# TIXhjq/ML_Function

Hardware: AMD Instinct MI355X
Metric: samples/sec fwd+bwd xDeepFM-CIN B=4096,F=39,K=16 (higher is better)
Workload: dtype f32

## Files before the change

ml_function_amd/csrc/cin.hip:

```cpp
#include "cin_kernels.h"
#include "cin_tail.h"
#include "cin_launch.h"
#include "cin_qtail.h"
#include "cin_qsplit.h"
#include "cin_qmerge.h"

#include <stdlib.h>

namespace fil {

struct CinShape {
  int B, F, K, L;
  int H[kCinMaxL];
  int Hp(int l) const { return l == 0 ? F : H[l - 1]; }
  int HS(int l) const { return 128 * cdiv(H[l], 128); }
  int xps(int l) const { return l == 0 ? F : HS(l - 1); }
  long M() const { return (long)B * K; }
  int JT() const { return cin_jt_of(F); }
  int HSmax() const {
    int h = 0;
    for (int l = 0; l < L; ++l) h = std::max(h, HS(l));
    return h;
  }
};
// ... 4 lines not shown
  if (F > kCinMaxFields) return fail(FIL_ERR_UNSUPPORTED, "%s: F=%d > %d fields", fn, F, kCinMaxFields);
  if ((long)B * K > (1L << 28)) return fail(FIL_ERR_UNSUPPORTED, "%s: B*K = %ld rows > 2^28 (row-split byte offsets of the dW kernel are 32-bit)", fn, (long)B * K);
  s.B = B; s.F = F; s.K = K; s.L = L;
  for (int l = 0; l < L; ++l) {
    if (H[l] < 1) return fail(FIL_ERR_ARG, "%s: H[%d]=%d", fn, l, H[l]);
    if (H[l] > kCinMaxH) return fail(FIL_ERR_UNSUPPORTED, "%s: H[%d]=%d > %d feature maps", fn, l, H[l], kCinMaxH);
    s.H[l] = H[l];
  }
  return FIL_OK;
}

static int chunks_of(int H) { return cdiv(H, 128); }
static int env_int(const char* name, int dflt) {
  const char* v = getenv(name);
  return v != nullptr && *v != 0 ? atoi(v) : dflt;
}
struct Knobs {
  int mb, sym, dw_mb, dw_splits, dz_mb, tail_splits, tail_settle, tail_dz_mode, ksplit, dzs_mb, qtail, qmerge, dz2, fwdq, headfold, packfold, dwfold4;
};
static const Knobs& knobs() {
  static const Knobs k = {env_int("FIL_CIN_MB", 0), env_int("FIL_CIN_SYM", 1), env_int("FIL_CIN_DW_MB", 1), env_int("FIL_CIN_DW_SPLITS", 0),
                          env_int("FIL_CIN_DZ_MB", 1), env_int("FIL_CIN_TAIL_SPLITS", 0), env_int("FIL_CIN_TAIL_SETTLE", 0), env_int("FIL_CIN_TAIL_DZ_MODE", 0), env_int("FIL_CIN_KSPLIT", -1), env_int("FIL_CIN_DZS_MB", 0), env_int("FIL_CIN_QTAIL", 1), env_int("FIL_CIN_QMERGE", 1), env_int("FIL_CIN_DZ2", 1), env_int("FIL_CIN_FWDQ", 1), env_int("FIL_CIN_HEADFOLD", 1), env_int("FIL_CIN_PACKFOLD", 1), env_int("FIL_CIN_DWFOLD4", 1)};
  return k;
}
struct CinTune {
  int mb_forced;
  bool sym, no_ksplit;
  explicit CinTune(int mode)
      : mb_forced((mode & FIL_CIN_MB2) ? 2 : knobs().mb), sym(knobs().sym != 0 && !(mode & FIL_CIN_NOSYM)), no_ksplit((mode & FIL_CIN_NOKSPLIT) != 0) {}
  int mb_rows(long M) const {
    if (mb_forced == 1 || mb_forced == 2) return mb_forced;
    return cdiv((int)std::min<long>(M, 1L << 30), 64) >= 768 ? 2 : 1;
  }
  int ksplit(long M) const {
    if (knobs().ksplit == 0 || no_ksplit) return 1;
    if (mb_rows(M) != 1) return 1;
    if (knobs().ksplit == 4) return 4;
    return cdiv((int)std::min<long>(M, 1L << 30), 32) <= 512 ? 4 : 1;
  }
};

static const char* kFwdNames[kCinMaxL] = {"cin_fwd_l1", "cin_fwd_l2", "cin_fwd_l3", "cin_fwd_l4", "cin_fwd_l5", "cin_fwd_l6", "cin_fwd_l7", "cin_fwd_l8"};
static const char* kDwNames[kCinMaxL] = {"cin_bwd_dw_l1", "cin_bwd_dw_l2", "cin_bwd_dw_l3", "cin_bwd_dw_l4", "cin_bwd_dw_l5", "cin_bwd_dw_l6", "cin_bwd_dw_l7", "cin_bwd_dw_l8"};
static const char* kDzNames[kCinMaxL] = {"cin_bwd_dz_l1", "cin_bwd_dz_l2", "cin_bwd_dz_l3", "cin_bwd_dz_l4", "cin_bwd_dz_l5", "cin_bwd_dz_l6", "cin_bwd_dz_l7", "cin_bwd_dz_l8"};
static double gemm_flops(long M, int Hp, int F, int H) { return 2.0 * (double)M * Hp * F * H; }

struct DwPlan {
  int MB, blocks_x, splits, rows_per_split, chunks;
};
static int cu_count() {
  static const int n = [] {
    int dev = 0, v = 0;
    if (hipGetDevice(&dev) != hipSuccess || hipDeviceGetAttribute(&v, hipDeviceAttributeMultiprocessorCount, dev) != hipSuccess || v <= 0) v = 256;
    return v;
  }();
  return n;
}

static DwPlan dw_plan(long M, int C, int H) {
  DwPlan p;
  p.chunks = chunks_of(H);
  p.MB = knobs().dw_mb == 2 ? 2 : 1;
  const int waves_c = cdiv(C, 32 * p.MB);
  p.blocks_x = cdiv(waves_c, 4);
  const long tiles = (long)p.blocks_x * p.chunks;
  const long ncu = cu_count();
  const long unit = 2 * kDwDepth;
  auto rows_of = [&](int splits) { return std::max<long>(unit, ((M + splits - 1) / splits + unit - 1) / unit * unit); };
  int best = knobs().dw_splits;
  if (best <= 0) {
    static const double t_of[4] = {0.0, 1.05e-4, 1.39e-4, 1.96e-4};
    double best_ms = -1.0;
    for (int sp = (int)std::max<long>(1, (M + (1L << 20) - 1) >> 20); sp <= 256; ++sp) {
      const long rps = rows_of(sp);
      const long real = (M + rps - 1) / rps;
      if (real != sp && sp > 1) continue;
      long wgs = tiles * real;
      double per_row = 0.0;
      while (wgs > 0) {
        const long round = std::min(wgs, 3 * ncu);
        per_row += t_of[std::min<long>(3, (round + ncu - 1) / ncu)];
        wgs -= round;
      }
      const double ms = (double)rps * per_row * p.MB + (double)real * C * H * 4.0 / 6e9;
      if (best_ms < 0 || ms < best_ms) best = sp, best_ms = ms;
      if (rps == unit) break;
    }
  }
  best = std::min(std::max(best, 1), 256);
  const long rps = rows_of(best);
  p.rows_per_split = (int)rps;
  p.splits = (int)std::max<long>(1, (M + rps - 1) / rps);
  return p;
}

static int launch_dw3(hipStream_t st, const DwPlan& p, const float* gT, int HS, const float* xT, const float* xpT, int xps, float* part,
                      long M, int F, int Hp, int H, int symD = 0, int xtra = 0) {
  const int items = p.blocks_x * p.splits * p.chunks;
  const dim3 grid((items + 7) / 8 * 8);
#define FIL_DW3(MBV, ONES) \
  hipLaunchKernelGGL((cin_dw3_kernel<MBV, ONES>), grid, dim3(kCinThreads), 0, st, gT, HS, xT, xpT, xps, part, (int)M, F, Hp, H, p.rows_per_split, \
                     p.blocks_x, p.chunks, items, symD, xtra)
  if (xT == nullptr) {
    if (p.MB == 2) FIL_DW3(2, true); else FIL_DW3(1, true);
  } else {
    if (p.MB == 2) FIL_DW3(2, false); else FIL_DW3(1, false);
  }
#undef FIL_DW3
  return p.splits;
}

struct TailGeom {
  bool on = false;
  int p = 0;
  int NCB = 0, JP = 0, JT4 = 0, NQ = 0, JHp = 0;
  int Hpp = 0, Hq = 0, HL = 0, Cp = 0, C1 = 0;
  int periods = 0, tiles = 0;
  size_t uf_floats = 0, uz_floats = 0;
};
static TailGeom tail_geom(const CinShape& s) {
  TailGeom g;
  if (s.L < 3 || !cin_tail_supported(s.F)) return g;
  g.on = true;
  g.p = s.L - 2;
  g.NCB = cin_tail_ncb(s.F);
  g.JP = 16 * g.NCB;
  g.JT4 = cin_tail_jt4(s.F);
  g.NQ = cin_tail_nq(s.F);
  g.JHp = 4 * g.NQ;
  g.Hpp = s.H[g.p - 1];
  g.Hq = s.H[g.p];
  g.HL = s.H[s.L - 1];
  g.Cp = g.Hpp * s.F;
  g.C1 = g.Cp + 1;
  const int JT = s.JT();
  g.periods = cdiv(g.Hpp, cin_dz_h_per_period(JT));
  g.tiles = g.periods * cin_dz_tiles_per_period(JT) + 1;
  g.uf_floats = (size_t)g.Hpp * g.JT4 * 64 * g.NCB + (size_t)align_up(g.JP + 1, 64);
  g.uz_floats = (size_t)g.tiles * 64 * g.JHp;
  return g;
}
constexpr int kCinRetiredBits = 0;
static bool tail_used(const CinShape& s, int mode) {
  if ((mode & (FIL_CIN_GENERAL | FIL_CIN_NOTAIL)) != 0) return false;
  const TailGeom g = tail_geom(s);
  if (!g.on) return false;
  return (mode & FIL_CIN_TAIL_ALWAYS) != 0 || 4 * g.JP <= 3 * g.Hq;
}
static bool qtail_used(const CinShape& s, int mode, const CinTune& tune) {
  if (s.M() <= 16384 && (mode & FIL_CIN_TAIL_ALWAYS) == 0) return false;
  return tail_used(s, mode) && s.L == 3 && tune.sym && s.F >= 2 && s.F + 2 <= kQtConst && s.H[0] <= 128 && 3 * s.F + 1 <= s.HSmax() && (mode & FIL_CIN_NOQTAIL) == 0 &&
         knobs().qtail != 0;
}
static bool qmerge_used(const CinShape& s, int mode, const CinTune& tune) {
  return qtail_used(s, mode, tune) && 3 * s.F + 3 <= s.HSmax() && (mode & FIL_CIN_NOQMERGE) == 0 && knobs().qmerge != 0;
}
constexpr int kCinPrecBf16 = 1 << 20;
static int qsplit_planes(int mode) { return (mode & kCinPrecBf16) != 0 ? 1 : 3; }
static bool qsplit_fwd_menu(int JT) { return JT >= 2 && JT <= 12 && JT % 2 == 0; }
static bool qsplit_used(const CinShape& s, int mode, const CinTune& tune) {
  return (mode & (FIL_CIN_BF16X3 | kCinPrecBf16)) != 0 && qmerge_used(s, mode, tune) && knobs().fwdq != 0 && knobs().dz2 != 0 && s.HS(0) == 128 &&
         qsplit_fwd_menu(cin_jt_sym(s.F));
}
static size_t qsplit_wb_bytes(const CinShape& s) { return (size_t)cin_qs_steps(s.F, cin_jt_sym(s.F)) * kQsStageBytes; }
static size_t qsplit_wzb_bytes(const CinShape& s) {
  const int jts = cin_jt_sym(s.F);
  return ((size_t)cdiv(s.F, cin_dz_h_per_period(jts)) * cin_dz_tiles_per_period(jts) + 1) * 8 * 3072;
}
static size_t qtail_wz_floats(const CinShape& s) {
  const int jts = cin_jt_sym(s.F);
  return ((size_t)cdiv(s.F, cin_dz_h_per_period(jts)) * cin_dz_tiles_per_period(jts) + 1) * 32 * s.HS(0);
}
static size_t qtail_wsn_floats(const CinShape& s) { return (size_t)chunks_of(s.H[0]) * 2 * s.JT() * 128; }
static size_t qtail_saved_floats(const CinShape& s) {
  return (size_t)s.M() * s.HS(0) + (size_t)s.F * s.F * s.H[0] + (size_t)s.H[1] * s.F + 128 + (size_t)s.H[0] * s.F + qtail_wsn_floats(s) +
         qtail_wz_floats(s);
}
struct TailDwPlan {
  int blocks_x, splits, rows_per_split;
};
static TailDwPlan tail_dw_plan(long M, int C1) {
  TailDwPlan p;
  p.blocks_x = cdiv(C1, 16 * kTailCbw);
  const long unit = 4L * 4 * kTailDwDepth;
  long want = knobs().tail_splits > 0 ? knobs().tail_splits : std::max<long>(1, 2L * cu_count() / p.blocks_x);
  want = std::max<long>(want, (M + (1L << 22) - 1) >> 22);
  const long rows = std::max(unit, ((M + want - 1) / want + unit - 1) / unit * unit);
  p.rows_per_split = (int)rows;
  p.splits = (int)std::max<long>(1, (M + rows - 1) / rows);
  return p;
}

constexpr int kHeadChunk = 16;
constexpr int kColRows = 128;

static size_t saved_bytes(const CinShape& s) {
  size_t t = align_up((size_t)s.M() * s.F * sizeof(float), 256);
  for (int l = 0; l + 1 < s.L; ++l) t += align_up((size_t)s.M() * s.HS(l) * sizeof(float), 256);
  const TailGeom g = tail_geom(s);
  if (g.on) {
    size_t u = align_up((size_t)s.M() * s.F * sizeof(float), 256);
    for (int l = 0; l < g.p; ++l) u += align_up((size_t)s.M() * s.HS(l) * sizeof(float), 256);
    u += align_up((size_t)s.M() * g.JP * sizeof(float), 256) + align_up((g.uz_floats + g.uf_floats) * sizeof(float), 256) +
         align_up((size_t)g.Hq * s.F * sizeof(float), 256);
    t = std::max(t, u);
  }
  if (g.on && s.L == 3) {
    const size_t u = align_up((size_t)s.M() * s.F * sizeof(float), 256) + align_up((size_t)s.M() * s.HS(0) * sizeof(float), 256) +
                     align_up(qtail_saved_floats(s) * sizeof(float), 256);
    t = std::max(t, u);
  }
  return t;
}
static size_t wf_floats(const CinShape& s) {
  size_t w = 0;
  for (int l = 0; l < s.L; ++l) {
    w = std::max(w, (size_t)chunks_of(s.H[l]) * s.Hp(l) * 2 * s.JT() * 128);
  }
  w = std::max(w, (size_t)chunks_of(s.H[0]) * s.F * 2 * cin_jt_sym(s.F) * 128);
  w += (size_t)2 * 2 * s.JT() * 128;
  return w;
}
static int dz_periods(const CinShape& s, int l) { return cdiv(s.Hp(l), cin_dz_h_per_period(s.JT())); }
static size_t wz_floats(const CinShape& s) {
  const int jts = cin_jt_sym(s.F);
  size_t w = ((size_t)cdiv(s.F, cin_dz_h_per_period(jts)) * cin_dz_tiles_per_period(jts) + 1) * 32 * s.HS(0);
  w = std::max(w, (size_t)s.F * (s.F / 2 + 1) * s.H[0]);
  for (int l = 0; l < s.L; ++l) w = std::max(w, ((size_t)dz_periods(s, l) * cin_dz_tiles_per_period(s.JT()) + 1) * 32 * s.HS(l));
  return w;
}
static int pool_chunks(const CinShape& s, int l) { return std::max(chunks_of(s.H[l]), l > 0 ? chunks_of(s.H[l - 1]) : 1); }
static size_t fwd_ws_bytes(const CinShape& s) {
  size_t t = 0;
  for (int l = 0; l < s.L; ++l) t += align_up((size_t)pool_chunks(s, l) * s.M() * sizeof(float), 256);
  t += align_up((size_t)s.Hp(s.L - 1) * s.F * sizeof(float), 256);
  t += align_up(wf_floats(s) * sizeof(float), 256);
  t += align_up((size_t)kCinMaxH * sizeof(float), 256);
  t += align_up(cin_x2_floats(s.M(), cin_x2_len(s.F)) * sizeof(float), 256);
  t += align_up((size_t)chunks_of(s.H[0]) * s.F * 2 * cin_jt_sym(s.F) * 128 * sizeof(float), 256);
  t += align_up(qsplit_wb_bytes(s), 256);
  return t;
}
static size_t dw_part_floats(const CinShape& s) {
  size_t pmax = 0;
  for (int l = 0; l < s.L; ++l) pmax = std::max(pmax, (size_t)dw_plan(s.M(), s.Hp(l) * s.F, s.H[l]).splits * s.Hp(l) * s.F * s.H[l]);
  const int csym = s.F * (s.F / 2 + 1);
  pmax = std::max(pmax, (size_t)dw_plan(s.M(), csym, s.H[0]).splits * csym * s.H[0]);
  pmax = std::max(pmax, (size_t)dw_plan(s.M(), csym + s.F, s.H[0]).splits * (csym + s.F) * s.H[0]);
  if (s.L == 3) pmax = std::max(pmax, (size_t)cin_dwq_plan(s.M(), csym + s.F, cu_count()).pairs * (csym + s.F) * 256);
  if (s.L == 3) pmax = std::max(pmax, (size_t)cin_dwqb_plan(s.M(), csym + s.F, cu_count()).splits * (csym + s.F) * 256);
  pmax = std::max(pmax, (size_t)dw_plan(s.M(), s.Hp(s.L - 1), s.F).splits * s.Hp(s.L - 1) * s.F);
  pmax = std::max(pmax, (size_t)dw_plan(s.M(), s.F, s.Hp(s.L - 1)).splits * s.Hp(s.L - 1) * s.F);
  const TailGeom g = tail_geom(s);
  if (g.on) {
    pmax = std::max(pmax, (size_t)tail_dw_plan(s.M(), g.C1).splits * g.C1 * g.JP + (size_t)cdiv(g.Cp, kTailPc) * g.Hq * s.F);
  }
  return pmax;
}
static size_t bwd_ws_bytes(const CinShape& s) {
  const size_t LK = (size_t)s.L * s.K;
  const size_t M = (size_t)s.M();
  size_t t = 0;
  t += align_up((size_t)s.B * LK * sizeof(float), 256);
  t += 2 * align_up(M * s.HSmax() * sizeof(float), 256);
  t += align_up(dw_part_floats(s) * sizeof(float), 256);
  const size_t nblk = (size_t)cdiv(std::max(1, s.B), kHeadChunk);
  const size_t ncol = (M + kColRows - 1) / kColRows;
  t += align_up(std::max(ncol * s.HSmax(), nblk * (LK + 1)) * sizeof(float), 256);
  const size_t cl = (size_t)std::max(s.Hp(s.L - 1), s.L == 3 ? s.H[0] : 0) * s.F;
  t += 2 * align_up(cl * sizeof(float), 256);
  t += align_up(wz_floats(s) * sizeof(float), 256);
  t += 2 * align_up(M * s.F * sizeof(float), 256);
  t += align_up((size_t)s.F * s.F * kCinMaxH * sizeof(float), 256);
  t += align_up(((M + 255) / 256 + 1) * kQtConst * sizeof(float), 256);
  t += align_up(((M + 255) / 256) * (LK + 1) * sizeof(float), 256);
  t += 2 * align_up(qsplit_wzb_bytes(s), 256);
  return t;
}

template <typename KernelT>
static void allow_lds(KernelT kernel, size_t sh) {
  if (sh > 48 * 1024) (void)hipFuncSetAttribute(reinterpret_cast<const void*>(kernel), hipFuncAttributeMaxDynamicSharedMemorySize, (int)sh);
}

}

using namespace fil;

extern "C" size_t fil_cin_saved_bytes(int B, int F, int K, int L, const int* H) {
  CinShape s;
  if (check_shape("fil_cin_saved_bytes", B, F, K, L, H, s) != FIL_OK || B == 0) return 0;
  return saved_bytes(s);
}

extern "C" size_t fil_cin_fwd_workspace_bytes(int B, int F, int K, int L, const int* H) {
  CinShape s;
  if (check_shape("fil_cin_fwd_workspace_bytes", B, F, K, L, H, s) != FIL_OK || B == 0) return 0;
  return fwd_ws_bytes(s);
}

extern "C" size_t fil_cin_bwd_workspace_bytes(int B, int F, int K, int L, const int* H) {
  CinShape s;
  if (check_shape("fil_cin_bwd_workspace_bytes", B, F, K, L, H, s) != FIL_OK || B == 0) return 0;
  return bwd_ws_bytes(s);
}

extern "C" int fil_cin_grad_ready_points(int B, int F, int K, int L, const int* H, int mode, int* point) {
  CinShape s;
  if (int rc = check_shape("fil_cin_grad_ready_points", B, F, K, L, H, s)) return rc;
  if (point == nullptr || mode < 0 || mode > 1023) return fail(FIL_ERR_ARG, "fil_cin_grad_ready_points: point == NULL or mode %d out of range", mode);
  if ((mode & kCinRetiredBits) != 0) return fail(FIL_ERR_UNSUPPORTED, "fil_cin_grad_ready_points: mode %d holds a retired bit (2: the split-bf16 experiment)", mode);
  if (B == 0) {
    for (int i = 0; i <= L; ++i) point[i] = 0;
    return 1;
  }
  int pt = 0, l = L - 1;
  point[L] = pt++;
  if (qmerge_used(s, mode, CinTune(mode))) {
    point[0] = point[L] = 0;
    pt = 1;
    point[1] = point[2] = pt++;
    return pt;
  }
  if (tail_used(s, mode)) {
    point[L - 1] = point[L - 2] = pt++;
    l = L - 3;
  }
  for (; l >= 0; --l) point[l] = pt++;
  return pt;
}

#define FIL_CIN_CHECK_ARG(cond)                                                        \
  do {                                                                                 \
    if (!(cond)) return ::fil::fail(FIL_ERR_ARG, "%s: bad argument: %s", who, #cond); \
  } while (0)

static int cin_precision_bits(const char* who, int mode, int precision, int* bits) {
  if (precision != FIL_CIN_PREC_DEFAULT && precision != FIL_CIN_PREC_BF16)
    return fail(FIL_ERR_ARG, "%s: precision %d (0 DEFAULT, 1 BF16)", who, precision);
  if (precision == FIL_CIN_PREC_BF16 && (mode & FIL_CIN_BF16X3) != 0)
    return fail(FIL_ERR_ARG, "%s: precision BF16 with mode bit BF16X3 (mode %d): two operand precisions", who, mode);
  *bits = precision == FIL_CIN_PREC_BF16 ? kCinPrecBf16 : 0;
  return FIL_OK;
}

extern "C" int fil_cin_precision_used(int B, int F, int K, int L, const int* H, int mode, int precision) {
  CinShape s;
  if (int rc = check_shape("fil_cin_precision_used", B, F, K, L, H, s)) return rc;
  if (mode < 0 || mode > 1023 || (mode & kCinRetiredBits) != 0) return fail(FIL_ERR_UNSUPPORTED, "fil_cin_precision_used: mode %d", mode);
  int bits = 0;
  if (int rc = cin_precision_bits("fil_cin_precision_used", mode, precision, &bits)) return rc;
  if (bits == 0 || B == 0) return FIL_CIN_PREC_DEFAULT;
  return qsplit_used(s, mode | bits, CinTune(mode)) ? FIL_CIN_PREC_BF16 : FIL_CIN_PREC_DEFAULT;
}

static int cin_fwd_impl(const char* who, const float* x, const float* const* W, const float* const* bias, const float* dense_w,
                        const float* dense_b, float* out, float* pooled, float* saved, int B, int F, int K, int L,
                        const int* H, int output_dim, int mode, int precision, void* workspace, size_t workspace_bytes, void* stream) {
  CinShape s;
  int rc = check_shape(who, B, F, K, L, H, s);
  if (rc != FIL_OK) return rc;
  if (mode < 0 || mode > 1023 || (mode & kCinRetiredBits) != 0)
    return fail(FIL_ERR_UNSUPPORTED, "%s: mode %d (bits: 1 general kernels, 2 BF16X3, 4 MB2, 8 NOSYM, 16 X_TRANSPOSED, 32 NOTAIL, 64 TAIL_ALWAYS, 128 NOKSPLIT, 256 NOQTAIL, 512 NOQMERGE)", who, mode);
  {
    int bits = 0;
    if ((rc = cin_precision_bits(who, mode, precision, &bits)) != FIL_OK) return rc;
    mode |= bits;
  }
  const bool xt_in = (mode & FIL_CIN_X_TRANSPOSED) != 0;
  const CinTune tune(mode);
  const bool tail = tail_used(s, mode);
  const bool qtail = qtail_used(s, mode, tune);
  const bool qmerge = qmerge_used(s, mode, tune);
  const bool qsplit = qsplit_used(s, mode, tune);
  const int qnp = qsplit_planes(mode);
  const TailGeom tg = tail_geom(s);
  mode &= 1;
  if (B == 0) return FIL_OK;
  FIL_CIN_CHECK_ARG(x && W && bias && pooled && saved);
  FIL_CIN_CHECK_ARG(output_dim != 1 || (dense_w && dense_b && out));
  if (workspace == nullptr || workspace_bytes < fwd_ws_bytes(s))
    return fail(FIL_ERR_WORKSPACE, "fil_cin_fwd: workspace %zu < %zu bytes", workspace_bytes, fwd_ws_bytes(s));
  hipStream_t st = (hipStream_t)stream;
  const long M = s.M();
  const int JT = s.JT(), MB = tune.mb_rows(M);
  Carver ws(workspace);
  PoolArgs pa;
  for (int l = 0; l < L; ++l) {
    pa.part[l] = ws.take<float>((size_t)pool_chunks(s, l) * M);
    pa.chunks[l] = chunks_of(H[l]);
  }
  float* wsum = ws.take<float>((size_t)s.Hp(L - 1) * F);
  float* Wf = ws.take<float>(wf_floats(s));
  float* qt_zbias = ws.take<float>((size_t)kCinMaxH);
  const int XL = cin_x2_len(F);
  float* x2T = ws.take<float>(cin_x2_floats(M, XL));
  const bool need_x2 = tune.sym;
  float* WfT = ws.take<float>((size_t)chunks_of(H[0]) * F * 2 * cin_jt_sym(F) * 128);
  u32x4* Wb = reinterpret_cast<u32x4*>(ws.take<unsigned char>(qsplit_wb_bytes(s)));
  Carver sv(saved);
  float* xT_own = sv.take<float>((size_t)M * F);
  const float* xT = xt_in ? x : xT_own;
  float *tailY = nullptr, *tailUz = nullptr, *tailBmT = nullptr;
  float *qtR = nullptr, *qtT = nullptr, *qtWsumL = nullptr, *qtCvec = nullptr, *qtWsumP = nullptr, *qtWsnP = nullptr, *qtWzT = nullptr;
  if (qtail) {
    Carver pv(saved);
    (void)pv.take<float>((size_t)M * F);
    (void)pv.take<float>((size_t)M * s.HS(0));
    float* q = pv.take<float>(qtail_saved_floats(s));
    qtR = q;
    qtT = qtR + (size_t)M * s.HS(0);
    qtWsumL = qtT + (size_t)F * F * H[0];
    qtCvec = qtWsumL + (size_t)H[1] * F;
    qtWsumP = qtCvec + 128;
    qtWsnP = qtWsumP + (size_t)H[0] * F;
    qtWzT = qtWsnP + qtail_wsn_floats(s);
  } else if (tail) {
    Carver pv(saved);
    (void)pv.take<float>((size_t)M * F);
    for (int l = 0; l < tg.p; ++l) (void)pv.take<float>((size_t)M * s.HS(l));
    tailY = pv.take<float>((size_t)M * tg.JP);
    tailUz = pv.take<float>(tg.uz_floats + tg.uf_floats);
    tailBmT = pv.take<float>((size_t)tg.Hq * F);
  }
  const bool prep_fused = tail && tune.sym;
  if (qtail) {
    FIL_CIN_CHECK_ARG(W[0] && W[L - 1] && W[L - 2]);
    ProfScope ps("cin_fwd_prep", st, 2.0 * M * F * sizeof(float));
    const int JTs = cin_jt_sym(F), chunks0 = chunks_of(H[0]);
    const long npack = (long)chunks0 * F * 2 * JTs * 128;
    const bool fq = qmerge && knobs().fwdq != 0 && s.HS(0) == 128;
    const int nt = fq ? 0 : B, npk = (int)std::min<long>((npack + 255) / 256, 1024), nwl = cdiv(tg.Hq * F, 8), nwp = cdiv(tg.Hpp * F, 8);
    const size_t sh = (xt_in || fq) ? 0 : (size_t)F * (K + 1) * sizeof(float);
    allow_lds(cin_qtail_prep_kernel, sh);
    hipLaunchKernelGGL(cin_qtail_prep_kernel, dim3(nt + npk + nwl + nwp), dim3(256), sh, st, x, xT_own, F, K, nt, W[0], Wf, H[0], 2 * JTs, chunks0, npk,
                       W[L - 1], qtWsumL, tg.Hq, tg.HL, nwl, W[L - 2], qtWsumP, qtWsnP, tg.Hpp, 2 * JT, chunks_of(tg.Hpp), x2T, XL, xt_in ? 1 : 0);
  } else if (prep_fused) {
    FIL_CIN_CHECK_ARG(W[0] && W[L - 1]);
    ProfScope ps("cin_fwd_prep", st, 2.0 * M * F * sizeof(float));
    const int JTs = cin_jt_sym(F), chunks0 = chunks_of(H[0]);
    const long npack = (long)chunks0 * F * 2 * JTs * 128;
    const int nt = B, npk = (int)std::min<long>((npack + 255) / 256, 1024), nws = cdiv(tg.Hq * F, 8), nz = 64;
    const size_t sh = xt_in ? 0 : (size_t)F * (K + 1) * sizeof(float);
    allow_lds(cin_fwd_prep_kernel, sh);
    hipLaunchKernelGGL(cin_fwd_prep_kernel, dim3(nt + npk + nws + nz), dim3(256), sh, st, x, xT_own, F, K, nt, W[0], Wf, H[0], 2 * JTs, chunks0,
                       npk, W[L - 1], tailBmT, tg.Hq, tg.HL, nws, reinterpret_cast<float4*>(tailUz), (long)((tg.uz_floats + tg.uf_floats) / 4), x2T, XL,
                       xt_in ? 1 : 0);
  } else if (!xt_in || need_x2) {
    ProfScope ps("cin_transpose_in", st, 2.0 * M * F * sizeof(float));
    hipLaunchKernelGGL(cin_transpose_in_kernel, dim3(B), dim3(256), xt_in ? 0 : (size_t)F * (K + 1) * sizeof(float), st, x, xT_own, F, K,
                       need_x2 ? x2T : nullptr, XL, xt_in ? 1 : 0);
  }
  FIL_CHECK_LAUNCH();
  const float* xpT = xT;
  bool fused_last = false;
  bool head_done = false;
  for (int l = 0; l < L; ++l) {
    FIL_CIN_CHECK_ARG(W[l] && bias[l]);
    if (qtail && qmerge && l == 0 && knobs().fwdq != 0 && s.HS(0) == 128) {
      const int p = tg.p, lL = L - 1, Hpp = tg.Hpp, Hq = tg.Hq, HS0 = s.HS(0);
      FIL_CIN_CHECK_ARG(W[p] && W[lL] && bias[p] && bias[lL]);
      const int JTs = cin_jt_sym(F), chunks = chunks_of(Hpp);
      float* x1T = sv.take<float>((size_t)M * HS0);
      {
        ProfScope ps("cin_tail_prep", st);
        int ks = -1;
        if (!xt_in && K <= 64 && (K & (K - 1)) == 0 && (reinterpret_cast<uintptr_t>(x) & 15) == 0)
          for (ks = 0; (1 << ks) < K;) ++ks;
        const size_t sh_x = ks >= 0 ? (size_t)(64 >> ks) * F * (K + 1) : (xt_in ? (size_t)64 * (F | 1) : (size_t)F * (K + 1));
        const int tiles = cdiv(F, cin_dz_h_per_period(JTs)) * cin_dz_tiles_per_period(JTs) + 1;
        const bool fold = !qsplit && knobs().packfold != 0;
        const QtPackFold pf = fold ? QtPackFold{WfT, qtWzT, JTs, chunks, HS0, tiles} : QtPackFold{nullptr, nullptr, 0, 0, 0, 0};
        const size_t sh = std::max(cin_qtail_t_lds_floats(F, Hq, fold), sh_x) * sizeof(float);
        allow_lds(cin_qtail_t_x_kernel, sh);
        const int nx = (ks >= 0 || xt_in) ? (int)((M + 63) / 64) : B, nT = cin_qtail_t_wgs(Hpp);
        hipLaunchKernelGGL(cin_qtail_t_x_kernel, dim3(nT + nx), dim3(256), sh, st, W[p], qtWsumL, bias[p], bias[lL], tg.HL, qtT, qtCvec, qt_zbias, Hpp, F, Hq,
                           nT, x, xT_own, K, x2T, XL, xt_in ? 1 : 0, ks, (ks >= 0 || xt_in) ? (long)M : 0L, pf);
        if (!fold) {
          const long npack = (long)chunks * F * 2 * JTs * 128;
          const int nbf = (int)std::min<long>((npack + 255) / 256, 1024), nbz = (int)std::min<long>(((long)tiles * 32 * HS0 + 255) / 256, 1024);
          const int NTq = qsplit ? cin_qs_steps(F, JTs) : 0, nbq = qsplit ? std::min(cdiv(NTq * 512, 256), 512) : 0;
          if (qnp == 1)
            hipLaunchKernelGGL(cin_qtail_pack_kernel<1>, dim3(nbf + nbz + nbq), dim3(256), 0, st, qtT, WfT, qtWzT, F, Hpp, JTs, chunks, nbf, HS0, tiles, nbz,
                               W[0], H[0], Wb, NTq);
          else
            hipLaunchKernelGGL(cin_qtail_pack_kernel<3>, dim3(nbf + nbz + nbq), dim3(256), 0, st, qtT, WfT, qtWzT, F, Hpp, JTs, chunks, nbf, HS0, tiles, nbz,
                               W[0], H[0], Wb, NTq);
        }
      }
      FIL_CHECK_LAUNCH();
      {
        const double algo = gemm_flops(M, F, F, H[0]) + gemm_flops(M, Hpp, F, Hq) + gemm_flops(M, Hq, F, tg.HL);
        ProfScope ps("cin_fwd_q", st, algo, gemm_flops(M, 1, F * (F / 2 + 1), H[0]) + gemm_flops(M, 1, F * (F / 2 + 1), Hpp));
        CinHeadFold hf{};
        if (K <= 32 && (K & (K - 1)) == 0 && knobs().headfold != 0) {
          int ks = 0;
          while ((1 << ks) < K) ++ks;
          hf = CinHeadFold{pooled, output_dim == 1 ? out : nullptr, dense_w, dense_b, ks, (int)(L * K), p * K, lL * K};
          head_done = true;
        }
        if (qsplit) {
          const int NT = cin_qs_steps(F, JTs);
          if (!cin_launch_fwdq_b(st, qnp, JTs, x2T, XL, Wb, NT, bias[0], qtWsnP, JT, qtCvec, x1T, qtR, HS0, const_cast<float*>(pa.part[0]),
                                 const_cast<float*>(pa.part[p]), const_cast<float*>(pa.part[lL]), (int)M, F, H[0], hf))
            return fail(FIL_ERR_UNSUPPORTED, "fil_cin_fwd: no split-bf16 forward kernel for JT=%d (F=%d)", JTs, F);
        } else if (!cin_launch_fwdq(st, JTs, x2T, XL, Wf, WfT, bias[0], qtWsnP, JT, qtCvec, x1T, qtR, HS0, const_cast<float*>(pa.part[0]),
                                    const_cast<float*>(pa.part[p]), const_cast<float*>(pa.part[lL]), (int)M, F, H[0], hf))
          return fail(FIL_ERR_UNSUPPORTED, "fil_cin_fwd: no merged forward kernel for JT=%d (F=%d)", JTs, F);
        pa.chunks[0] = pa.chunks[p] = pa.chunks[lL] = 1;
      }
      FIL_CHECK_LAUNCH();
      break;
    }
    if (qtail && l == tg.p) {
      const int lL = L - 1, Hpp = tg.Hpp, Hq = tg.Hq, HS0 = s.HS(0);
      FIL_CIN_CHECK_ARG(W[lL] && bias[lL]);
      const int JTs = cin_jt_sym(F), chunks = chunks_of(Hpp);
      {
        ProfScope ps("cin_tail_prep", st);
        const size_t sh = cin_qtail_t_lds_floats(F, Hq, false) * sizeof(float);
        allow_lds(cin_qtail_t_kernel, sh);
        hipLaunchKernelGGL(cin_qtail_t_kernel, dim3(cin_qtail_t_wgs(Hpp)), dim3(256), sh, st, W[l], qtWsumL, bias[l], bias[lL], tg.HL, qtT, qtCvec, qt_zbias, Hpp, F, Hq);
        const long npack = (long)chunks * F * 2 * JTs * 128;
        const int tiles = cdiv(F, cin_dz_h_per_period(JTs)) * cin_dz_tiles_per_period(JTs) + 1;
        const int nbf = (int)std::min<long>((npack + 255) / 256, 1024), nbz = (int)std::min<long>(((long)tiles * 32 * HS0 + 255) / 256, 1024);
        hipLaunchKernelGGL(cin_qtail_pack_kernel<3>, dim3(nbf + nbz), dim3(256), 0, st, qtT, Wf, qtWzT, F, Hpp, JTs, chunks, nbf, HS0, tiles);
      }
      FIL_CHECK_LAUNCH();
      {
        const double algo = gemm_flops(M, Hpp, F, Hq) + gemm_flops(M, Hq, F, tg.HL);
        ProfScope ps("cin_fwd_tail", st, algo, gemm_flops(M, 1, F * (F / 2 + 1), Hpp));
        const int ks = tune.ksplit(M);
        cin_launch_fwd3_sym(st, MB, JTs, dim3(ks == 4 ? cdiv((int)M, 32) : cdiv((int)M, 128 * MB), chunks), xT, x2T, XL, Wf, qt_zbias, qtR, HS0,
                            const_cast<float*>(pa.part[lL]), (int)M, F, Hpp, ks);
      }
      FIL_CHECK_LAUNCH();
      {
        ProfScope ps("cin_tail_pool", st);
        const float* wsn = qtWsnP;
        float* pp = const_cast<float*>(pa.part[l]);
        float* pL = const_cast<float*>(pa.part[lL]);
        const dim3 grid((int)((M + 127) / 128));
#define FIL_QP(JTV) \
  case JTV: hipLaunchKernelGGL((cin_qtail_pool2_kernel<JTV>), grid, dim3(256), 0, st, xT, xpT, s.xps(l), wsn, qtR, HS0, qtCvec, pp, pL, (int)M, F, Hpp); break;
        switch (JT) { FIL_QP(4) FIL_QP(8) FIL_QP(12) FIL_QP(16) FIL_QP(20) FIL_QP(24) FIL_QP(28) FIL_QP(32) }
#undef FIL_QP
        pa.chunks[l] = pa.chunks[lL] = 1;
      }
      FIL_CHECK_LAUNCH();
      break;
    }
    if (tail && l == tg.p) {
      const int lL = L - 1;
      FIL_CIN_CHECK_ARG(W[lL] && bias[lL]);
      float* Y = tailY;
      float* Uz = tailUz;
      float* bmT = tailBmT;
      float* Uf = Uz + tg.uz_floats;
      float* consts = Uf + (size_t)tg.Hpp * tg.JT4 * 64 * tg.NCB;
      {
        ProfScope ps("cin_tail_prep", st);
        if (!prep_fused) {
          hipLaunchKernelGGL(cin_tail_wsum_kernel, dim3(cdiv(tg.Hq * F, 8)), dim3(256), 0, st, W[lL], bmT, tg.Hq, F, tg.HL);
          (void)hipMemsetAsync(Uz, 0, (tg.uz_floats + tg.uf_floats) * sizeof(float), st);
        }
        const size_t sh = (size_t)(F + 1) * (((tg.Hq + 3) & ~3) + 4) * sizeof(float);
        allow_lds(cin_tail_ueff_kernel, sh);
        hipLaunchKernelGGL(cin_tail_ueff_kernel, dim3(cdiv(tg.C1, kTailUc)), dim3(256), sh, st, W[l], bias[l], bmT, bias[lL], tg.HL, Uf, Uz, consts,
                           tg.Hpp, F, tg.Hq, tg.JT4, tg.JP, JT, tg.JHp);
      }
      FIL_CHECK_LAUNCH();
      {
        const double algo = gemm_flops(M, tg.Hpp, F, tg.Hq) + gemm_flops(M, tg.Hq, F, tg.HL);
        ProfScope ps("cin_fwd_tail", st, algo, 2.0 * (double)M * tg.Cp * (F + 1));
        const int RB = tune.mb_rows(M) == 2 ? 4 : 2;
        TailFwdArgs a{xT, xpT, s.xps(l), Uf, consts, Y, tg.JP, const_cast<float*>(pa.part[l]), const_cast<float*>(pa.part[lL]), (int)M, F, tg.Hpp,
                      tune.ksplit(M)};
        cin_launch_tail_fwd(st, RB, tg.JT4, tg.NCB, a);
        pa.chunks[l] = pa.chunks[lL] = 1;
      }
      FIL_CHECK_LAUNCH();
      break;
    }
    const int Hp = s.Hp(l), Hl = H[l], xps = s.xps(l);
    float* xoutT = l + 1 < L ? sv.take<float>((size_t)M * s.HS(l)) : nullptr;
    float* part = const_cast<float*>(pa.part[l]);
    const bool fuse_next = mode == 0 && l == L - 2 && !(l == 0 && tune.sym);
    if (l == L - 1 && mode == 0) {
      if (!fused_last) {
        const size_t sh = (size_t)Hp * ((F + 3) & ~3) * sizeof(float);
        ProfScope ps("cin_last_fwd", st, 2.0 * (double)M * Hp * F);
        hipLaunchKernelGGL(cin_wsum_kernel, dim3(cdiv(Hp * F, 8)), dim3(256), 0, st, W[l], wsum, Hp * F, Hl);
        allow_lds(cin_last_fwd_kernel, sh);
        hipLaunchKernelGGL(cin_last_fwd_kernel, dim3(cdiv((int)M, kLastRows)), dim3(256), sh, st, xT, xpT, xps, wsum, bias[l], part, (int)M, F, Hp, Hl);
        pa.chunks[l] = 1;
      }
    } else {
      const int chunks = chunks_of(Hl);
      if (l == 0 && tune.sym) {
        const int JTs = cin_jt_sym(F);
        const long npack = (long)chunks * F * 2 * JTs * 128;
        if (!prep_fused)
          hipLaunchKernelGGL(cin_pack_wf_sym_kernel, dim3((int)std::min<long>((npack + 255) / 256, 2048)), dim3(256), 0, st, W[l], Wf, F, Hl, 2 * JTs, chunks);
        ProfScope ps(kFwdNames[l], st, gemm_flops(M, Hp, F, Hl), gemm_flops(M, 1, F * (F / 2 + 1), Hl));
        const int ks = tune.ksplit(M);
        cin_launch_fwd3_sym(st, MB, JTs, dim3(ks == 4 ? cdiv((int)M, 32) : cdiv((int)M, 128 * MB), chunks), xT, x2T, XL, Wf, bias[l], xoutT, s.HS(l), part,
                            (int)M, F, Hl, ks);
      } else {
        const long npack = (long)chunks * Hp * 2 * JT * 128;
        hipLaunchKernelGGL(cin_pack_wf_kernel, dim3((int)std::min<long>((npack + 255) / 256, 2048)), dim3(256), 0, st, W[l], Wf, Hp, F, Hl, 2 * JT, chunks);
        const float* wsn = nullptr;
        if (fuse_next) {
          FIL_CIN_CHECK_ARG(W[l + 1] && bias[l + 1]);
          float* wsn_buf = Wf + (size_t)npack;
          hipLaunchKernelGGL(cin_wsum_wsn_kernel, dim3(cdiv(Hl * F, 8)), dim3(256), 0, st, W[l + 1], wsum, Hl * F, H[l + 1], wsn_buf, Hl, F, 2 * JT,
                             chunks);
          wsn = wsn_buf;
          pa.chunks[l + 1] = chunks;
          fused_last = true;
        }
        ProfScope ps(kFwdNames[l], st, gemm_flops(M, Hp, F, Hl) + (fuse_next ? 2.0 * (double)M * Hl * F : 0.0));
        cin_launch_fwd3(st, MB, JT, dim3(cdiv((int)M, 128 * MB), chunks), xT, xpT, xps, Wf, bias[l], xoutT, s.HS(l), part, (int)M, F, Hp, Hl,
                        wsn, fuse_next ? bias[l + 1] : nullptr, fuse_next ? H[l + 1] : 0, fuse_next ? const_cast<float*>(pa.part[l + 1]) : nullptr);
      }
    }
    FIL_CHECK_LAUNCH();
    xpT = xoutT;
  }
  if (!head_done) {
    ProfScope ps("cin_head_fwd", st);
    hipLaunchKernelGGL(cin_head_fwd_kernel, dim3(cdiv(B, kHeadSamples)), dim3(256), (size_t)kHeadSamples * L * K * sizeof(float), st, pa, dense_w, dense_b, pooled,
                       output_dim == 1 ? out : nullptr, B, K, L);
  }
  FIL_CHECK_LAUNCH();
  return FIL_OK;
}

extern "C" int fil_cin_fwd(const float* x, const float* const* W, const float* const* bias, const float* dense_w,
                           const float* dense_b, float* out, float* pooled, float* saved, int B, int F, int K, int L,
                           const int* H, int output_dim, int mode, void* workspace, size_t workspace_bytes, void* stream) {
  return cin_fwd_impl("fil_cin_fwd", x, W, bias, dense_w, dense_b, out, pooled, saved, B, F, K, L, H, output_dim, mode, FIL_CIN_PREC_DEFAULT, workspace,
                      workspace_bytes, stream);
}

extern "C" int fil_cin_fwd_p(const float* x, const float* const* W, const float* const* bias, const float* dense_w,
                             const float* dense_b, float* out, float* pooled, float* saved, int B, int F, int K, int L,
                             const int* H, int output_dim, int mode, int precision, void* workspace, size_t workspace_bytes, void* stream) {
  return cin_fwd_impl("fil_cin_fwd_p", x, W, bias, dense_w, dense_b, out, pooled, saved, B, F, K, L, H, output_dim, mode, precision, workspace,
                      workspace_bytes, stream);
}

static int cin_bwd_impl(const char* who, const float* x, const float* const* W, const float* const* bias, const float* dense_w,
                        const float* pooled, const float* saved, const float* g, float* dx, float* const* dW,
                        float* const* dbias, float* ddense_w, float* ddense_b, int B, int F, int K, int L, const int* H,
                        int output_dim, int mode, int precision, void* const* grad_ready_events, void* workspace, size_t workspace_bytes,
                        void* stream) {
  CinShape s;
  int rc = check_shape(who, B, F, K, L, H, s);
  if (rc != FIL_OK) return rc;
  if (mode < 0 || mode > 1023 || (mode & kCinRetiredBits) != 0)
    return fail(FIL_ERR_UNSUPPORTED, "%s: mode %d (bits: 1 general kernels, 2 BF16X3, 4 MB2, 8 NOSYM, 16 X_TRANSPOSED, 32 NOTAIL, 64 TAIL_ALWAYS, 128 NOKSPLIT, 256 NOQTAIL, 512 NOQMERGE)", who, mode);
  {
    int bits = 0;
    if ((rc = cin_precision_bits(who, mode, precision, &bits)) != FIL_OK) return rc;
    mode |= bits;
  }
  const bool xt_in = (mode & FIL_CIN_X_TRANSPOSED) != 0;
  const CinTune tune(mode);
  const bool tail = tail_used(s, mode);
  const bool qtail = qtail_used(s, mode, tune);
  const bool qmerge = qmerge_used(s, mode, tune);
  const bool qsplit = qsplit_used(s, mode, tune);
  const int qnp = qsplit_planes(mode);
  const TailGeom tg = tail_geom(s);
  mode &= 1;
  FIL_CIN_CHECK_ARG(W && dW && dbias);
  hipStream_t st = (hipStream_t)stream;
  const size_t LK = (size_t)L * K;
  auto ready = [&](int slot) {
    if (grad_ready_events != nullptr && grad_ready_events[slot] != nullptr) (void)hipEventRecord((hipEvent_t)grad_ready_events[slot], st);
  };
  if (B == 0) {
    for (int l = 0; l < L; ++l) {
      (void)hipMemsetAsync(dW[l], 0, (size_t)s.Hp(l) * F * H[l] * sizeof(float), st);
      (void)hipMemsetAsync(dbias[l], 0, (size_t)H[l] * sizeof(float), st);
    }
    if (output_dim == 1) {
      (void)hipMemsetAsync(ddense_w, 0, LK * sizeof(float), st);
      (void)hipMemsetAsync(ddense_b, 0, sizeof(float), st);
    }
    for (int l = 0; l <= L; ++l) ready(l);
    return FIL_OK;
  }
  FIL_CIN_CHECK_ARG(g && dx && saved && (x || !xt_in));
  FIL_CIN_CHECK_ARG(output_dim != 1 || (dense_w && pooled && ddense_w && ddense_b));
  if (workspace == nullptr || workspace_bytes < bwd_ws_bytes(s))
    return fail(FIL_ERR_WORKSPACE, "fil_cin_bwd: workspace %zu < %zu bytes", workspace_bytes, bwd_ws_bytes(s));
  const long M = s.M();
  const int JT = s.JT();
  Carver ws(workspace);
  float* dP = ws.take<float>((size_t)B * LK);
  float* Gbuf[2];
  Gbuf[0] = ws.take<float>((size_t)M * s.HSmax());
  Gbuf[1] = ws.take<float>((size_t)M * s.HSmax());
  float* part = ws.take<float>(dw_part_floats(s));
  const int nblk = cdiv(B, kHeadChunk);
  const int ncol = (int)((M + kColRows - 1) / kColRows);
  float* small = ws.take<float>(std::max((size_t)ncol * s.HSmax(), (size_t)nblk * (LK + 1)));
  const size_t cl = (size_t)s.Hp(L - 1) * F;
  const size_t cl_buf = (size_t)std::max(s.Hp(L - 1), L == 3 ? H[0] : 0) * F;
  float* wsum = ws.take<float>(cl_buf);
  float* vlast = ws.take<float>(cl_buf);
  float* Wz = ws.take<float>(wz_floats(s));
  float* dxT = ws.take<float>((size_t)M * F);
  float* gx0T = ws.take<float>((size_t)M * F);
  float* qt_dT = ws.take<float>((size_t)F * F * kCinMaxH);
  const int qt_ndc = (int)((M + 255) / 256);
  float* qt_dcpart = ws.take<float>((size_t)(qt_ndc + 1) * kQtConst);
  float* qt_hpart = ws.take<float>((size_t)qt_ndc * (LK + 1));
  u32x4* Wzb1 = reinterpret_cast<u32x4*>(ws.take<unsigned char>(qsplit_wzb_bytes(s)));
  u32x4* Wzb2 = reinterpret_cast<u32x4*>(ws.take<unsigned char>(qsplit_wzb_bytes(s)));

  Carver sv(const_cast<float*>(saved));
  const float* xT_own = sv.take<float>((size_t)M * F);
  const float* xT = xt_in ? x : xT_own;
  const float* maps[kCinMaxL];
  const float *tailY = nullptr, *tailUz = nullptr, *tailWsum = nullptr;
  const float *qtR = nullptr, *qtT = nullptr, *qtWsumL = nullptr, *qtCvec = nullptr, *qtWsumP = nullptr, *qtWsnP = nullptr, *qtWzT = nullptr;
  if (qtail) {
    maps[0] = sv.take<float>((size_t)M * s.HS(0));
    const float* q = sv.take<float>(qtail_saved_floats(s));
    qtR = q;
    qtT = qtR + (size_t)M * s.HS(0);
    qtWsumL = qtT + (size_t)F * F * H[0];
    qtCvec = qtWsumL + (size_t)H[1] * F;
    qtWsumP = qtCvec + 128;
    qtWsnP = qtWsumP + (size_t)H[0] * F;
    qtWzT = qtWsnP + qtail_wsn_floats(s);
  } else if (tail) {
    for (int l = 0; l < tg.p; ++l) maps[l] = sv.take<float>((size_t)M * s.HS(l));
    tailY = sv.take<float>((size_t)M * tg.JP);
    tailUz = sv.take<float>(tg.uz_floats + tg.uf_floats);
    tailWsum = sv.take<float>((size_t)tg.Hq * F);
  } else {
    for (int l = 0; l + 1 < L; ++l) maps[l] = sv.take<float>((size_t)M * s.HS(l));
  }

  const float* dPsrc = g;
  if (output_dim == 1 && qmerge) {
    dPsrc = dP;
  } else if (output_dim == 1) {
    ProfScope ps("cin_head_bwd", st);
    hipLaunchKernelGGL(cin_head_bwd_kernel, dim3(nblk), dim3(256), 0, st, g, dense_w, pooled, dP, small, B, (int)LK, kHeadChunk);
    if (!tail) hipLaunchKernelGGL(cin_reduce_kernel, dim3(cdiv((int)LK + 1, 64)), dim3(256), 0, st, small, ddense_w, (long)(LK + 1), nblk, ddense_b, (long)LK);
    FIL_CHECK_LAUNCH();
    dPsrc = dP;
  }
  if (!tail) ready(L);

  int cur = 0;
  int ltop = L - 1;
  bool dx_started = false;
  bool have_gx0 = false;
  bool wz_prepacked = false;
  bool qm_joined = false;
  if (qmerge) {
    const int p = tg.p, lL = L - 1, Hpp = tg.Hpp, Hq = tg.Hq, HS0 = s.HS(0);
    FIL_CIN_CHECK_ARG(bias && W[0] && W[p] && W[lL] && bias[p] && dW[0] && dW[p] && dW[lL] && dbias[0] && dbias[p] && dbias[lL]);
    const float* xpT = maps[p - 1];
    const int xps = s.xps(p);
    const float* dPp = dPsrc + (size_t)p * K;
    const float* dPL = dPsrc + (size_t)lL * K;
    const float* dPprev = dPsrc + (size_t)(p - 1) * K;
    const double algo_tail = gemm_flops(M, Hpp, F, Hq) + gemm_flops(M, Hq, F, tg.HL);
    const double algo1 = gemm_flops(M, F, F, H[0]);
    const int symD = F / 2 + 1, Cl = F * symD;
    const int JTs = cin_jt_sym(F);
    const int periods = cdiv(F, cin_dz_h_per_period(JTs));
    const int tiles0 = periods * cin_dz_tiles_per_period(JTs) + 1;
    const int XE = F + 3;
    float* xe = Gbuf[1];
    float* gxR = xe + (size_t)M * XE;
    float* dxR = gxR + (size_t)M * F;
    {
      ProfScope ps("cin_tail_a", st, (double)M * (2 * F + 3) * sizeof(float));
      const size_t sh = (size_t)256 * (F + 3 + (output_dim == 1 ? L : 0)) * sizeof(float);
      allow_lds(cin_qtail_xe_kernel<3>, sh);
      allow_lds(cin_qtail_xe_kernel<1>, sh);
      const int np = (int)std::min<long>(((long)tiles0 * 32 * HS0 + 255) / 256, 1024);
      const int nq2 = qsplit ? 2 * std::min(cdiv(tiles0 * 512, 256), 256) : 0;
      if (qnp == 1)
        hipLaunchKernelGGL(cin_qtail_xe_kernel<1>, dim3(qt_ndc + np + nq2), dim3(kXeThreads), sh, st, xT, dPL, dPp, (int)LK, K, xe, qt_dcpart, (int)M, F,
                           qt_ndc, output_dim == 1 ? g : nullptr, dense_w, pooled, dP, qt_hpart, (int)LK, lL, p, W[0], Wz, H[0], JTs, HS0, tiles0, np, qtT,
                           Hpp, Wzb1, Wzb2);
      else
        hipLaunchKernelGGL(cin_qtail_xe_kernel<3>, dim3(qt_ndc + np + nq2), dim3(kXeThreads), sh, st, xT, dPL, dPp, (int)LK, K, xe, qt_dcpart, (int)M, F,
                           qt_ndc, output_dim == 1 ? g : nullptr, dense_w, pooled, dP, qt_hpart, (int)LK, lL, p, W[0], Wz, H[0], JTs, HS0, tiles0, np, qtT,
                           Hpp, Wzb1, Wzb2);
    }
    FIL_CHECK_LAUNCH();
    {
      ProfScope ps("cin_last_bwd", st, 6.0 * (double)M * Hpp * F);
      cin_launch_last_bwd2(st, JT, xT, xpT, xps, qtWsumP, qtWsnP, dPp, (int)LK, dPprev, Gbuf[cur], HS0, dxT, (int)M, F, K, Hpp, qtR, HS0, dPL, small);
    }
    FIL_CHECK_LAUNCH();
    int dw_parts = 0;
    {
      ProfScope ps("cin_bwd_dw_q", st, algo1 + algo_tail, gemm_flops(M, 1, Cl, H[0]) + gemm_flops(M, 1, Cl, Hpp));
      if (qsplit) {
        const DwqbPlan bp = cin_dwqb_plan(M, Cl + F, cu_count());
        cin_launch_dwq_b(st, qnp, bp, Gbuf[cur], xpT, HS0, xe, XE, part, (int)M, F, symD);
        dw_parts = bp.splits;
      } else {
        const bool f4 = knobs().dwfold4 != 0;
        const DwqPlan dp = f4 ? cin_dwq_plan4(M, Cl + F, cu_count()) : cin_dwq_plan(M, Cl + F, cu_count());
        if (f4)
          hipLaunchKernelGGL((cin_dwq_kernel<kDwqDepth, 4>), dim3((dp.wgs + 7) / 8 * 8), dim3(kDwqThreads), 0, st, Gbuf[cur], xpT, HS0, xe, XE, part, (int)M, F,
                             symD, dp.rows_per_split, dp.splits, dp.ncol_full, dp.rem, dp.wgs_full, dp.wgs);
        else
          hipLaunchKernelGGL((cin_dwq_kernel<kDwqDepth, 2>), dim3((dp.wgs + 7) / 8 * 8), dim3(kDwqThreads), 0, st, Gbuf[cur], xpT, HS0, xe, XE, part, (int)M, F,
                             symD, dp.rows_per_split, dp.splits, dp.ncol_full, dp.rem, dp.wgs_full, dp.wgs);
        dw_parts = dp.pairs;
      }
    }
    FIL_CHECK_LAUNCH();
    {
      ProfScope ps("cin_reduce_dw", st);
      const int nb1 = cdiv(H[0], 64);
      const int nh = output_dim == 1 ? cdiv((int)LK + 1, 64) : 0;
      hipLaunchKernelGGL(cin_reduce_expand_q_kernel, dim3((Cl + F + 3) / 4 + nb1 + nh), dim3(256), 0, st, part, dw_parts, F, symD, H[0], Hpp, dW[0], qt_dT,
                         vlast, small, ncol, dbias[0], nb1, qt_hpart, qt_ndc, (int)LK, ddense_w, ddense_b);
    }
    FIL_CHECK_LAUNCH();
    ready(L);
    ready(0);
    {
      ProfScope ps("cin_tail_params", st);
      const size_t sh = cin_qtail_params_lds(F, Hq);
      allow_lds(cin_qtail_params_kernel, sh);
      float* dcfin = qt_dcpart + (size_t)qt_ndc * kQtConst;
      hipLaunchKernelGGL(cin_qtail_params_kernel, dim3(2 * Hpp + 1), dim3(256), sh, st, W[p], qtWsumL, qt_dT, vlast, dW[p], part, Hpp, F, Hq, qt_dcpart, qt_ndc,
                         dcfin);
      hipLaunchKernelGGL(cin_qtail_fill_kernel, dim3(cdiv(Hq * F, kQtFillCols)), dim3(kQtFillThreads), 0, st, part, Hpp, dcfin, bias[p], qtWsumL, dW[lL], dbias[p], dbias[lL], F, Hq,
                         tg.HL);
    }
    FIL_CHECK_LAUNCH();
    ready(lL);
    ready(p);
    const int NHMAX = HS0 / 2;
    if (NHMAX == 64 && knobs().dz2 != 0) {
      ProfScope ps("cin_bwd_dz_q", st, algo1 + algo_tail, gemm_flops(M, 1, Cl, H[0]) + gemm_flops(M, 1, Cl, Hpp));
      bool split_done = false;
      if (qsplit) {
        split_done = cin_launch_dz2_b(st, qnp, JTs, Gbuf[cur], xpT, HS0, dPL, (int)LK, K, Wzb1, Wzb2, xT, dxT, 1, (int)M, F, H[0], Hpp, periods, dx, qtCvec);
      }
      if (!split_done &&
          !cin_launch_dz2(st, JTs, Gbuf[cur], xpT, HS0, dPL, (int)LK, K, Wz, qtWzT, xT, dxT, 1, (int)M, F, H[0], Hpp, periods, dx, qtCvec))
        return fail(FIL_ERR_UNSUPPORTED, "fil_cin_bwd: no two-pass data-gradient kernel for JT=%d (F=%d)", JTs, F);
      qm_joined = true;
    } else {
      const bool two_waves = NHMAX == 64 && cin_dzs_two_waves(JTs) && tune.mb_forced != 2 && knobs().dzs_mb != 2;
      const int MBs = two_waves ? 1 : tune.mb_rows(M);
      const int ks = MBs != 1 ? 1 : tune.ksplit(M);
      const dim3 zgrid(ks == 4 ? cdiv((int)M, 32) : cdiv((int)M, 128 * MBs));
      {
        ProfScope ps("cin_bwd_dz_tail", st, algo_tail, gemm_flops(M, 1, Cl, Hpp));
        cin_launch_dz3_sym(st, MBs, JTs, NHMAX, zgrid, xpT, HS0, qtWzT, xT, gxR, dxR, 0, (int)M, F, Hpp, periods, ks);
      }
      FIL_CHECK_LAUNCH();
      {
        ProfScope ps("cin_bwd_dz_l1", st, algo1, gemm_flops(M, 1, Cl, H[0]));
        cin_launch_dz3_sym(st, MBs, JTs, NHMAX, zgrid, Gbuf[cur], HS0, Wz, xT, gx0T, dxT, 1, (int)M, F, H[0], periods, ks);
      }
      have_gx0 = true;
    }
    FIL_CHECK_LAUNCH();
    dx_started = true;
    ltop = -1;
  } else if (qtail) {
    const int p = tg.p, lL = L - 1, Hpp = tg.Hpp, Hq = tg.Hq, HS0 = s.HS(0);
    FIL_CIN_CHECK_ARG(bias && W[p] && W[lL] && bias[p] && dW[p] && dW[lL] && dbias[p] && dbias[lL]);
    const float* xpT = maps[p - 1];
    const int xps = s.xps(p);
    const float* dPp = dPsrc + (size_t)p * K;
    const float* dPL = dPsrc + (size_t)lL * K;
    const float* dPprev = dPsrc + (size_t)(p - 1) * K;
    const double algo = gemm_flops(M, Hpp, F, Hq) + gemm_flops(M, Hq, F, tg.HL);
    float* xs = Gbuf[1];
    float* gxR = xs + (size_t)M * (F + 1);
    float* dxR = gxR + (size_t)M * F;
    {
      ProfScope ps("cin_tail_a", st, (double)M * (F + 64) * sizeof(float));
      const size_t sh = (size_t)256 * (F + 3) * sizeof(float);
      allow_lds(cin_qtail_scale_kernel, sh);
      const int nh = output_dim == 1 ? cdiv((int)LK + 1, 64) : 0;
      FIL_CIN_CHECK_ARG(W[0]);
      const int JTs0 = cin_jt_sym(F);
      const int tiles0 = cdiv(F, cin_dz_h_per_period(JTs0)) * cin_dz_tiles_per_period(JTs0) + 1;
      const int np = (int)std::min<long>(((long)tiles0 * 32 * HS0 + 255) / 256, 1024);
      hipLaunchKernelGGL(cin_qtail_scale_kernel, dim3(qt_ndc + nh + np), dim3(256), sh, st, xT, dPL, dPp, (int)LK, K, xs, qt_dcpart, (int)M, F, qt_ndc, small,
                         ddense_w, ddense_b, (int)LK, nblk, nh, W[0], Wz, H[0], JTs0, HS0, tiles0);
      wz_prepacked = true;
    }
    FIL_CHECK_LAUNCH();
    ready(L);
    {
      ProfScope ps("cin_last_bwd", st, 6.0 * (double)M * Hpp * F);
      cin_launch_last_bwd2(st, JT, xT, xpT, xps, qtWsumP, qtWsnP, dPp, (int)LK, dPprev, Gbuf[cur], HS0, dxT, (int)M, F, K, Hpp, qtR, HS0, dPL, small);
    }
    FIL_CHECK_LAUNCH();
    const int symD = F / 2 + 1, Cl = F * symD;
    const int JTs = cin_jt_sym(F);
    {
      ProfScope ps("cin_bwd_dw_tail", st, algo, gemm_flops(M, 1, Cl, Hpp));
      const int parts = launch_dw3(st, dw_plan(M, Cl + F, Hpp), xpT, HS0, xT, xs, F + 1, part, M, F, F, Hpp, symD, F);
      const long nW = (long)Cl * Hpp, pstride = (long)(Cl + F) * Hpp;
      hipLaunchKernelGGL(cin_reduce_expand_sym_kernel, dim3((int)((nW + 63) / 64) + cdiv(F * Hpp, 64)), dim3(256), 0, st, part, qt_dT, F, symD, Hpp, parts,
                         pstride, vlast, (long)F * Hpp);
    }
    FIL_CHECK_LAUNCH();
    {
      ProfScope ps("cin_tail_params", st);
      const size_t sh = cin_qtail_params_lds(F, Hq);
      allow_lds(cin_qtail_params_kernel, sh);
      float* dcfin = qt_dcpart + (size_t)qt_ndc * kQtConst;
      hipLaunchKernelGGL(cin_qtail_params_kernel, dim3(2 * Hpp + 1), dim3(256), sh, st, W[p], qtWsumL, qt_dT, vlast, dW[p], part, Hpp, F, Hq, qt_dcpart, qt_ndc,
                         dcfin);
      hipLaunchKernelGGL(cin_qtail_fill_kernel, dim3(cdiv(Hq * F, kQtFillCols)), dim3(kQtFillThreads), 0, st, part, Hpp, dcfin, bias[p], qtWsumL, dW[lL], dbias[p], dbias[lL], F, Hq,
                         tg.HL);
    }
    FIL_CHECK_LAUNCH();
    ready(lL);
    ready(p);
    {
      const int periods = cdiv(F, cin_dz_h_per_period(JTs));
      ProfScope ps("cin_bwd_dz_tail", st, algo, gemm_flops(M, 1, Cl, Hpp));
      const int NHMAX = HS0 / 2;
      const bool two_waves = NHMAX == 64 && cin_dzs_two_waves(JTs) && tune.mb_forced != 2 && knobs().dzs_mb != 2;
      const int MBs = two_waves ? 1 : tune.mb_rows(M);
      const int ks = MBs != 1 ? 1 : tune.ksplit(M);
      cin_launch_dz3_sym(st, MBs, JTs, NHMAX, dim3(ks == 4 ? cdiv((int)M, 32) : cdiv((int)M, 128 * MBs)), xpT, HS0, qtWzT, xT, gxR, dxR, 0, (int)M, F, Hpp,
                         periods, ks);
    }
    FIL_CHECK_LAUNCH();
    dx_started = true;
    ltop = p - 1;
  } else if (tail) {
    const int p = tg.p, lL = L - 1;
    FIL_CIN_CHECK_ARG(bias && W[p] && W[lL] && bias[p] && dW[p] && dW[lL] && dbias[p] && dbias[lL]);
    const float* xpT = maps[p - 1];
    const int xps = s.xps(p);
    const double algo = gemm_flops(M, tg.Hpp, F, tg.Hq) + gemm_flops(M, tg.Hq, F, tg.HL);
    float* Apk = Gbuf[1];
    wz_prepacked = p == 1 && tune.sym && F >= 2;
    {
      ProfScope ps("cin_tail_a", st, (double)M * (F + 64) * sizeof(float));
      const int na = (int)std::min<long>((M * 16 * tg.NCB + 255) / 256, 4096);
      const int nh = output_dim == 1 ? cdiv((int)LK + 1, 64) : 0;
      int np = 0, JTs = 0, tiles0 = 0;
      if (wz_prepacked) {
        FIL_CIN_CHECK_ARG(W[0]);
        JTs = cin_jt_sym(F);
        tiles0 = cdiv(F, cin_dz_h_per_period(JTs)) * cin_dz_tiles_per_period(JTs) + 1;
        np = (int)std::min<long>(((long)tiles0 * 32 * s.HS(0) + 255) / 256, 1024);
      }
      hipLaunchKernelGGL(cin_tail_pre_kernel, dim3(na + nh + np), dim3(256), 0, st, xT, dPsrc, (int)LK, K, p, lL, Apk, (int)M, F, tg.NCB, na, small,
                         ddense_w, ddense_b, (int)LK, nblk, nh, W[0], Wz, H[0], JTs, s.HS(0), tiles0);
    }
    FIL_CHECK_LAUNCH();
    ready(L);
    const TailDwPlan tp = tail_dw_plan(M, tg.C1);
    {
      ProfScope ps("cin_bwd_dw_tail", st, algo, 2.0 * (double)M * tg.C1 * (F + 2));
      TailDwArgs a{Apk, xT, xpT, xps, part, (int)M, F, tg.Hpp, tg.JP, tp.rows_per_split, tp.blocks_x, tp.blocks_x * tp.splits, knobs().tail_settle != 0};
      cin_launch_tail_dw(st, tg.NCB, a);
    }
    FIL_CHECK_LAUNCH();
    {
      ProfScope ps("cin_tail_params", st);
      const int nblk_p = cdiv(tg.Cp, kTailPc);
      const int ldb = (tg.Hq + 3) & ~3;
      const size_t sh = ((size_t)(F + 1) * ldb + (size_t)tg.JP * (kTailPc + 4) + (size_t)kTailPc * ldb) * sizeof(float);
      allow_lds(cin_tail_params_kernel, sh);
      float* partB = part + (size_t)tp.splits * tg.C1 * tg.JP;
      float* qones = vlast;
      hipLaunchKernelGGL(cin_tail_params_kernel, dim3(2 * nblk_p), dim3(256), sh, st, part, tp.splits, W[p], tailWsum, dW[p], dbias[p], partB, qones,
                         tg.Cp, F, tg.Hq, tg.JP);
      hipLaunchKernelGGL(cin_tail_fill_kernel, dim3(cdiv(tg.Hq * F, 64)), dim3(256), 0, st, partB, nblk_p, qones, bias[p], dW[lL], dbias[lL], F,
                         tg.Hq, tg.HL);
    }
    FIL_CHECK_LAUNCH();
    ready(lL);
    ready(p);
    {
      ProfScope ps("cin_bwd_dz_tail", st, algo, 2.0 * (double)M * tg.Cp * (F + 1));
      TailDzArgs a{tailUz, xT, xpT, xps, tailY, tg.JP, dPsrc, (int)LK, K, p, lL, Gbuf[cur], s.HS(p - 1), dxT, (int)M, F, tg.Hpp, tg.periods, knobs().tail_dz_mode,
                   tune.ksplit(M)};
      cin_launch_tail_dz(st, JT, tg.NQ, a);
    }
    FIL_CHECK_LAUNCH();
    dx_started = true;
    ltop = p - 1;
  } else if (mode == 0) {
    const int l = L - 1;
    FIL_CIN_CHECK_ARG(W[l] && dW[l] && dbias[l]);
    const int Hp = s.Hp(l), Hl = H[l], xps = s.xps(l);
    const float* xpT = l == 0 ? xT : maps[l - 1];
    const float* dPl = dPsrc + (size_t)l * K;
    const float* dPprev = l > 0 ? dPsrc + (size_t)(l - 1) * K : nullptr;
    const size_t shw = (size_t)Hp * ((F + 3) & ~3) * sizeof(float);
    ProfScope ps("cin_last_bwd", st, 6.0 * (double)M * Hp * F);
    hipLaunchKernelGGL(cin_wsum_wsn_kernel, dim3(cdiv(Hp * F, 8)), dim3(256), 0, st, W[l], wsum, Hp * F, Hl, l > 0 ? Wz : nullptr, Hp, F, 2 * JT,
                       chunks_of(Hp));
    hipLaunchKernelGGL(cin_slice_sum_kernel, dim3(nblk), dim3(256), 0, st, dPl, (int)LK, small, B, K, kHeadChunk);
    {
      float* yT = Gbuf[1];
      const int YS = (F + 3) & ~3;
      const long tot = M * YS;
      hipLaunchKernelGGL(cin_scale_rows3_kernel, dim3((int)std::min<long>((tot + 255) / 256, 4096)), dim3(256), 0, st, xT, dPl, (int)LK, K, yT, (int)M, F, YS);
      const bool swap = l > 0;
      int nb;
      if (swap) nb = launch_dw3(st, dw_plan(M, F, Hp), xpT, xps, nullptr, yT, YS, part, M, 1, F, Hp);
      else nb = launch_dw3(st, dw_plan(M, Hp, F), yT, YS, nullptr, xpT, xps, part, M, 1, Hp, F);
      hipLaunchKernelGGL(cin_reduce_kernel, dim3(cdiv((int)cl, 64)), dim3(256), 0, st, part, vlast, (long)cl, nb);
      hipLaunchKernelGGL(cin_fill_rows_kernel, dim3((int)std::min<long>(((long)cl * Hl + 255) / 256, 2048)), dim3(256), 0, st, vlast, dW[l], (long)cl, Hl,
                         swap ? F : 0, Hp, small, nblk, dbias[l]);
    }
    ready(l);
    if (l > 0) {
      cin_launch_last_bwd2(st, JT, xT, xpT, xps, wsum, Wz, dPl, (int)LK, dPprev, Gbuf[cur], s.HS(l - 1), dxT, (int)M, F, K, Hp);
    } else {
      const size_t shb = shw + (size_t)kLastRows * (kLastFMax + 1) * sizeof(float);
      allow_lds(cin_last_bwd_kernel, shb);
      hipLaunchKernelGGL(cin_last_bwd_kernel, dim3(cdiv((int)M, kLastRows)), dim3(256), shb, st, xT, xpT, xps, wsum, dPl, (int)LK, dPprev,
                         nullptr, 0, dxT, 1, (int)M, F, K, Hp);
    }
    FIL_CHECK_LAUNCH();
    dx_started = true;
    ltop = L - 2;
  } else {
    const long total = M * s.HS(L - 1);
    ProfScope ps("cin_bcast_g", st, (double)total * sizeof(float));
    hipLaunchKernelGGL(cin_bcast3_kernel, dim3((int)std::min<long>((total + 255) / 256, 4096)), dim3(256), 0, st, dPsrc + (size_t)(L - 1) * K, (int)LK,
                       K, Gbuf[cur], s.HS(L - 1), (int)M, H[L - 1]);
    FIL_CHECK_LAUNCH();
  }
  for (int l = ltop; l >= 0; --l) {
    FIL_CIN_CHECK_ARG(W[l] && dW[l] && dbias[l]);
    const int Hp = s.Hp(l), Hl = H[l], HSl = s.HS(l), xps = s.xps(l);
    const float* xpT = l == 0 ? xT : maps[l - 1];
    const float* G = Gbuf[cur];
    {
      ProfScope ps("cin_dbias", st, (double)M * Hl * sizeof(float));
      if (!(qtail && l == ltop)) hipLaunchKernelGGL(cin_colsum3_kernel, dim3(ncol), dim3(256), 0, st, G, HSl, small, (int)M, Hl, kColRows);
      hipLaunchKernelGGL(cin_reduce_kernel, dim3(cdiv(Hl, 64)), dim3(256), 0, st, small, dbias[l], (long)Hl, ncol);
    }
    FIL_CHECK_LAUNCH();
    int parts;
    const int symD = (l == 0 && tune.sym) ? F / 2 + 1 : 0;
    const int Cl = symD > 0 ? F * symD : Hp * F;
    {
      ProfScope ps(kDwNames[l], st, gemm_flops(M, Hp, F, Hl), gemm_flops(M, 1, Cl, Hl));
      parts = launch_dw3(st, dw_plan(M, Cl, Hl), G, HSl, xT, xpT, xps, part, M, F, Hp, Hl, symD);
    }
    FIL_CHECK_LAUNCH();
    const long nW = (long)Cl * Hl;
    {
      ProfScope ps("cin_reduce_dw", st, (double)(parts + 1) * nW * sizeof(float));
      if (symD > 0) hipLaunchKernelGGL(cin_reduce_expand_sym_kernel, dim3((int)((nW + 63) / 64)), dim3(256), 0, st, part, dW[l], F, symD, Hl, parts);
      else hipLaunchKernelGGL(cin_reduce_kernel, dim3((int)((nW + 63) / 64)), dim3(256), 0, st, part, dW[l], nW, parts);
    }
    FIL_CHECK_LAUNCH();
    ready(l);
    {
      const int NHMAX = HSl / 2;
      const int MB = NHMAX == 128 ? 1 : tune.mb_rows(M);
      const int MBg = NHMAX == 128 ? 1 : ((knobs().dz_mb == 2 && JT <= 28) ? 2 : 1);
      const float* dPprev = l > 0 ? dPsrc + (size_t)(l - 1) * K : nullptr;
      if (l == 0 && tune.sym && F >= 2) {
        const int JTs = cin_jt_sym(F);
        const int periods = cdiv(F, cin_dz_h_per_period(JTs));
        const int tiles = periods * cin_dz_tiles_per_period(JTs) + 1;
        const long npack = (long)tiles * 32 * HSl;
        const bool two_waves = NHMAX == 64 && cin_dzs_two_waves(JTs) && tune.mb_forced != 2 && knobs().dzs_mb != 2;
        const int MBs = two_waves ? 1 : MB;
        if (!wz_prepacked) {
          hipLaunchKernelGGL(cin_pack_wz_sym_kernel, dim3((int)std::min<long>((npack + 255) / 256, 2048)), dim3(256), 0, st, W[l], Wz, F, Hl, JTs, HSl, tiles);
        }
        ProfScope ps(kDzNames[l], st, gemm_flops(M, Hp, F, Hl), gemm_flops(M, 1, F * (F / 2 + 1), Hl));
        const int ks = (NHMAX != 64 || MBs != 1) ? 1 : tune.ksplit(M);
        cin_launch_dz3_sym(st, MBs, JTs, NHMAX, dim3(ks == 4 ? cdiv((int)M, 32) : cdiv((int)M, 128 * MBs)), G, HSl, Wz, xT, gx0T, dxT,
                           dx_started ? 1 : 0, (int)M, F, Hl, periods, ks);
      } else {
        const int periods = dz_periods(s, l);
        const int tiles = periods * cin_dz_tiles_per_period(JT) + 1;
        const long npack = (long)tiles * 32 * HSl;
        hipLaunchKernelGGL(cin_pack_wz_kernel, dim3((int)std::min<long>((npack + 255) / 256, 2048)), dim3(256), 0, st, W[l], Wz, Hp, F, Hl, JT, HSl, tiles);
        ProfScope ps(kDzNames[l], st, gemm_flops(M, Hp, F, Hl));
        cin_launch_dz3(st, MBg, JT, NHMAX, dim3(cdiv((int)M, 128 * MBg)), G, HSl, Wz, xT, xpT, xps, dPprev, (int)LK, K,
                       l > 0 ? Gbuf[cur ^ 1] : nullptr, l > 0 ? s.HS(l - 1) : 0, l == 0 ? gx0T : nullptr, dxT, dx_started ? 1 : 0,
                       (int)M, F, Hp, Hl, periods);
      }
      dx_started = true;
      if (l == 0) have_gx0 = true;
    }
    FIL_CHECK_LAUNCH();
    cur ^= 1;
  }
  if (!qm_joined) {
    ProfScope ps("cin_transpose_out", st, 2.0 * M * F * sizeof(float));
    if (qmerge)
      hipLaunchKernelGGL(cin_transpose_out_kernel, dim3(B), dim3(256), (size_t)K * (F + 1) * sizeof(float), st, dxT, have_gx0 ? gx0T : nullptr, dx, F, K,
                         Gbuf[1] + (size_t)M * (F + 3), Gbuf[1] + (size_t)M * (F + 3) + (size_t)M * F, qtCvec, dPsrc + (size_t)(L - 1) * K, (int)LK);
    else if (qtail)
      hipLaunchKernelGGL(cin_transpose_out_kernel, dim3(B), dim3(256), (size_t)K * (F + 1) * sizeof(float), st, dxT, have_gx0 ? gx0T : nullptr, dx, F, K,
                         Gbuf[1] + (size_t)M * (F + 1), Gbuf[1] + (size_t)M * (F + 1) + (size_t)M * F, qtCvec, dPsrc + (size_t)(L - 1) * K, (int)LK);
    else
      hipLaunchKernelGGL(cin_transpose_out_kernel, dim3(B), dim3(256), (size_t)K * (F + 1) * sizeof(float), st, dxT, have_gx0 ? gx0T : nullptr, dx, F, K);
  }
  FIL_CHECK_LAUNCH();
  return FIL_OK;
}

extern "C" int fil_cin_bwd(const float* x, const float* const* W, const float* const* bias, const float* dense_w,
                           const float* pooled, const float* saved, const float* g, float* dx, float* const* dW,
                           float* const* dbias, float* ddense_w, float* ddense_b, int B, int F, int K, int L, const int* H,
                           int output_dim, int mode, void* const* grad_ready_events, void* workspace, size_t workspace_bytes,
                           void* stream) {
  return cin_bwd_impl("fil_cin_bwd", x, W, bias, dense_w, pooled, saved, g, dx, dW, dbias, ddense_w, ddense_b, B, F, K, L, H, output_dim, mode,
                      FIL_CIN_PREC_DEFAULT, grad_ready_events, workspace, workspace_bytes, stream);
}

extern "C" int fil_cin_bwd_p(const float* x, const float* const* W, const float* const* bias, const float* dense_w,
                             const float* pooled, const float* saved, const float* g, float* dx, float* const* dW,
                             float* const* dbias, float* ddense_w, float* ddense_b, int B, int F, int K, int L, const int* H,
                             int output_dim, int mode, int precision, void* const* grad_ready_events, void* workspace, size_t workspace_bytes,
                             void* stream) {
  return cin_bwd_impl("fil_cin_bwd_p", x, W, bias, dense_w, pooled, saved, g, dx, dW, dbias, ddense_w, ddense_b, B, F, K, L, H, output_dim, mode,
                      precision, grad_ready_events, workspace, workspace_bytes, stream);
}
```

ml_function_amd/csrc/cin_fwd.hip:

```cpp
#include "cin_kernels.h"
#include "cin_launch.h"

namespace fil {

template <int MB, int JT>
static void fwd3(hipStream_t st, dim3 grid, const float* xT, const float* xpT, int xps, const float* Wf, const float* bias,
                 float* xoutT, int HS, float* pool_part, int M, int F, int Hp, int H, const float* wsn, const float* bias_next,
                 int H_next, float* pool_next) {
  hipLaunchKernelGGL((cin_fwd3_kernel<MB, JT>), grid, dim3(kCinThreads), 0, st, xT, xpT, xps, Wf, bias, xoutT, HS, pool_part, M, F, Hp, H, wsn,
                     bias_next, H_next, pool_next);
}

void cin_launch_fwd3(hipStream_t st, int MB, int JT, dim3 grid, const float* xT, const float* xpT, int xps, const float* Wf,
                     const float* bias, float* xoutT, int HS, float* pool_part, int M, int F, int Hp, int H, const float* wsn,
                     const float* bias_next, int H_next, float* pool_next) {
#define FIL_F3(JTV)                                                                                                                      \
  case JTV:                                                                                                                              \
    if (MB == 2) fwd3<2, JTV>(st, grid, xT, xpT, xps, Wf, bias, xoutT, HS, pool_part, M, F, Hp, H, wsn, bias_next, H_next, pool_next);   \
    else fwd3<1, JTV>(st, grid, xT, xpT, xps, Wf, bias, xoutT, HS, pool_part, M, F, Hp, H, wsn, bias_next, H_next, pool_next);           \
    break;
  switch (JT) { FIL_F3(4) FIL_F3(8) FIL_F3(12) FIL_F3(16) FIL_F3(20) FIL_F3(24) FIL_F3(28) FIL_F3(32) }
#undef FIL_F3
}

template <int MB, int JT>
static void fwd3s(hipStream_t st, dim3 grid, const float* xT, const float* x2T, int XL, const float* Wf, const float* bias, float* xoutT, int HS,
                  float* pool_part, int M, int F, int H, int ks) {
  if constexpr (MB == 1) {
    if (ks == 4) {
      hipLaunchKernelGGL((cin_fwd3_kernel<1, JT, true, 4>), grid, dim3(kCinThreads), 0, st, xT, x2T, XL, Wf, bias, xoutT, HS, pool_part, M, F,
                         F, H, nullptr, nullptr, 0, nullptr);
      return;
    }
  }
  hipLaunchKernelGGL((cin_fwd3_kernel<MB, JT, true>), grid, dim3(kCinThreads), 0, st, xT, x2T, XL, Wf, bias, xoutT, HS, pool_part, M, F, F, H,
                     nullptr, nullptr, 0, nullptr);
}

void cin_launch_fwd3_sym(hipStream_t st, int MB, int JT, dim3 grid, const float* xT, const float* x2T, int XL, const float* Wf, const float* bias,
                         float* xoutT, int HS, float* pool_part, int M, int F, int H, int ks) {
#define FIL_F3S(JTV)                                                                             \
  case JTV:                                                                                      \
    if (MB == 2) fwd3s<2, JTV>(st, grid, xT, x2T, XL, Wf, bias, xoutT, HS, pool_part, M, F, H, 1);  \
    else fwd3s<1, JTV>(st, grid, xT, x2T, XL, Wf, bias, xoutT, HS, pool_part, M, F, H, ks);         \
    break;
  switch (JT) { FIL_F3S(2) FIL_F3S(4) FIL_F3S(6) FIL_F3S(8) FIL_F3S(10) FIL_F3S(12) FIL_F3S(14) FIL_F3S(16) FIL_F3S(18) }
#undef FIL_F3S
}

template <int JT>
static void last_bwd2(hipStream_t st, const float* xT, const float* xpT, int xps, const float* wsum, const float* wsn, const float* dP,
                      int ldp, const float* dPprev, float* GprevT, int HSp, float* dxT, int M, int F, int K, int Hp, const float* Radd, int HSr,
                      const float* dPadd, float* colpart) {
  const size_t sh = ((size_t)((Hp * F + 3) & ~3) + 4 * kLast2Stage) * sizeof(float);
  if (sh > 48 * 1024)
    (void)hipFuncSetAttribute(reinterpret_cast<const void*>(cin_last_bwd2_kernel<JT>), hipFuncAttributeMaxDynamicSharedMemorySize, (int)sh);
  hipLaunchKernelGGL((cin_last_bwd2_kernel<JT>), dim3((M + 127) / 128), dim3(kCinThreads), sh, st, xT, xpT, xps, wsum, wsn, dP, ldp, dPprev,
                     GprevT, HSp, dxT, M, F, K, Hp, Radd, HSr, dPadd, colpart);
}

void cin_launch_last_bwd2(hipStream_t st, int JT, const float* xT, const float* xpT, int xps, const float* wsum, const float* wsn,
                          const float* dP, int ldp, const float* dPprev, float* GprevT, int HSp, float* dxT, int M, int F, int K, int Hp,
                          const float* Radd, int HSr, const float* dPadd, float* colpart) {
#define FIL_LB(JTV) \
  case JTV: last_bwd2<JTV>(st, xT, xpT, xps, wsum, wsn, dP, ldp, dPprev, GprevT, HSp, dxT, M, F, K, Hp, Radd, HSr, dPadd, colpart); break;
  switch (JT) { FIL_LB(4) FIL_LB(8) FIL_LB(12) FIL_LB(16) FIL_LB(20) FIL_LB(24) FIL_LB(28) FIL_LB(32) }
#undef FIL_LB
}

}
```

ml_function_amd/csrc/cin_kernels.h:

```cpp
#pragma once
#include "common.h"

namespace fil {

constexpr int kCinThreads = 256;
constexpr int kCinMaxL = 8;
constexpr int kCinMaxH = 256;

__device__ __forceinline__ f32x16 mfma32(float a, float b, f32x16 c) {
  return __builtin_amdgcn_mfma_f32_32x32x2f32(a, b, c, 0, 0, 0);
}

__device__ __forceinline__ void settle(float& v) { asm volatile("" : "+v"(v)); }
typedef float f32x4s __attribute__((ext_vector_type(4)));
__device__ __forceinline__ void settle(f32x4s& v) { asm volatile("" : "+v"(v)); }

__device__ __forceinline__ __amdgpu_buffer_rsrc_t make_rsrc(const float* p, long bytes) {
  return __builtin_amdgcn_make_buffer_rsrc(const_cast<float*>(p), 0, (int)std::min<long>(bytes, 0x7fffffffL), 0x00020000);
}
__device__ __forceinline__ __amdgpu_buffer_rsrc_t make_rsrc_uniform(const float* p, long bytes) {
  const unsigned long a = reinterpret_cast<unsigned long>(p);
  const unsigned lo = __builtin_amdgcn_readfirstlane((unsigned)a), hi = __builtin_amdgcn_readfirstlane((unsigned)(a >> 32));
  const int n = __builtin_amdgcn_readfirstlane((int)std::min<long>(bytes, 0x7fffffffL));
  return __builtin_amdgcn_make_buffer_rsrc(reinterpret_cast<float*>(((unsigned long)hi << 32) | lo), 0, n, 0x00020000);
// ... 1088 lines not shown
static __global__ __launch_bounds__(256) void cin_wsum_wsn_kernel(const float* __restrict__ W, float* __restrict__ wsum, int C, int H,
                                                           float* __restrict__ wsn, int Hp, int F, int JT2, int chunks) {
  const int row = blockIdx.x * 8 + (threadIdx.x >> 5), l = threadIdx.x & 31;
  float t = 0.f;
  if (row < C)
    for (int n = l; n < H; n += 32) t += W[(long)row * H + n];
  t = half_wave_sum(t);
  if (row < C && l == 0) {
    wsum[row] = t;
    if (wsn != nullptr) {
      const int n = row / F, fp = row - n * F;
      wsn[(((n >> 7) * JT2) + fp) * 128 + (n & 127)] = t;
    }
  }
  if (wsn != nullptr) {
    const int total = chunks * JT2 * 128;
    for (int i = blockIdx.x * blockDim.x + threadIdx.x; i < total; i += gridDim.x * blockDim.x) {
      const int col = i & 127, fp = (i >> 7) % JT2, chunk = (i >> 7) / JT2;
      if (fp >= F || chunk * 128 + col >= Hp) wsn[i] = 0.f;
    }
  }
}

__device__ __forceinline__ void stage_wsum(const float* __restrict__ wsum, float* ws, int Hp, int F, int FP4) {
  for (int idx = threadIdx.x; idx < Hp * FP4; idx += blockDim.x) {
    const int h = idx / FP4, f = idx - h * FP4;
    ws[idx] = f < F ? wsum[h * F + f] : 0.f;
  }
}

constexpr int kLastRows = 64;

static __global__ __launch_bounds__(256) void cin_last_fwd_kernel(const float* __restrict__ xT, const float* __restrict__ xpT, int xps,
                                                           const float* __restrict__ wsum, const float* __restrict__ bias,
                                                           float* __restrict__ pool, int M, int F, int Hp, int H) {
  extern __shared__ __attribute__((aligned(16))) float smem[];
  const int FP4 = (F + 3) & ~3;
  stage_wsum(wsum, smem, Hp, F, FP4);
  float bsum = 0.f;
  for (int n = 0; n < H; ++n) bsum += bias[n];
  __syncthreads();
  const int lane = threadIdx.x & 63, wave = threadIdx.x >> 6;
  const int m = blockIdx.x * kLastRows + wave * 16 + (lane & 15), hq = lane >> 4;
  const bool valid = m < M;
  const long mm = valid ? m : 0;
  float xr[kLastFMax];
#pragma unroll
  for (int f = 0; f < kLastFMax; ++f) xr[f] = (valid && f < F) ? xT[mm * F + f] : 0.f;
  const float* xprow = xpT + mm * xps;
  float p = 0.f;
  for (int h = hq; h < Hp; h += 4) {
    const float4* wrow = reinterpret_cast<const float4*>(smem + h * FP4);
    float t = 0.f;
#pragma unroll
    for (int f4 = 0; f4 < kLastFMax / 4; ++f4) {
      if (4 * f4 < F) {
        const float4 w = wrow[f4];
        t = fmaf(xr[4 * f4], w.x, t);
        t = fmaf(xr[4 * f4 + 1], w.y, t);
        t = fmaf(xr[4 * f4 + 2], w.z, t);
        t = fmaf(xr[4 * f4 + 3], w.w, t);
      }
    }
    p = fmaf(valid ? xprow[h] : 0.f, t, p);
  }
  p += __shfl_xor(p, 16);
  p += __shfl_xor(p, 32);
  if (valid && hq == 0) pool[m] = p + bsum;
}

static __global__ __launch_bounds__(256) void cin_last_bwd_kernel(const float* __restrict__ xT, const float* __restrict__ xpT, int xps,
                                                           const float* __restrict__ wsum, const float* __restrict__ dP, int ldp,
                                                           const float* __restrict__ dPprev, float* __restrict__ GprevT, int HSp,
                                                           float* __restrict__ dxT, int layer1, int M, int F, int K, int Hp) {
  extern __shared__ __attribute__((aligned(16))) float smem[];
  const int FP4 = (F + 3) & ~3;
  float* ts = smem + Hp * FP4;
  stage_wsum(wsum, smem, Hp, F, FP4);
  __syncthreads();
  const int lane = threadIdx.x & 63, wave = threadIdx.x >> 6;
  const int rowl = wave * 16 + (lane & 15), hq = lane >> 4;
  const int m = blockIdx.x * kLastRows + rowl;
  const bool valid = m < M;
  const long mm = valid ? m : 0;
  const int b = (int)(mm / K), k = (int)(mm - (long)b * K);
  float xr[kLastFMax], u[kLastFMax];
#pragma unroll
  for (int f = 0; f < kLastFMax; ++f) {
    xr[f] = (valid && f < F) ? xT[mm * F + f] : 0.f;
    u[f] = 0.f;
  }
  const float dp = valid ? dP[(long)b * ldp + k] : 0.f;
  const float dpp = (valid && dPprev != nullptr) ? dPprev[(long)b * ldp + k] : 0.f;
  const float* xprow = xpT + mm * xps;
  for (int h = hq; h < Hp; h += 4) {
    const float4* wrow = reinterpret_cast<const float4*>(smem + h * FP4);
    const float xph = valid ? xprow[h] : 0.f;
    float t = 0.f;
#pragma unroll
    for (int f4 = 0; f4 < kLastFMax / 4; ++f4) {
      if (4 * f4 < F) {
        const float4 w = wrow[f4];
        t = fmaf(xr[4 * f4], w.x, t);
        t = fmaf(xr[4 * f4 + 1], w.y, t);
        t = fmaf(xr[4 * f4 + 2], w.z, t);
        t = fmaf(xr[4 * f4 + 3], w.w, t);
        u[4 * f4] = fmaf(xph, w.x, u[4 * f4]);
        u[4 * f4 + 1] = fmaf(xph, w.y, u[4 * f4 + 1]);
        u[4 * f4 + 2] = fmaf(xph, w.z, u[4 * f4 + 2]);
        u[4 * f4 + 3] = fmaf(xph, w.w, u[4 * f4 + 3]);
      }
    }
    if (layer1) ts[rowl * (kLastFMax + 1) + h] = t;
    else if (valid) GprevT[mm * HSp + h] = fmaf(dp, t, dpp);
  }
  if (layer1) __syncthreads();
#pragma unroll
  for (int f = 0; f < kLastFMax; ++f) {
    if (f < F) {
      float v = u[f];
      v += __shfl_xor(v, 16);
      v += __shfl_xor(v, 32);
      if (layer1) v += ts[rowl * (kLastFMax + 1) + f];
      if (valid && hq == 0) dxT[mm * F + f] = dp * v;
    }
  }
}

static __global__ __launch_bounds__(256) void cin_fill_rows_kernel(const float* __restrict__ v, float* __restrict__ dW, long C, int H, int Ft,
                                                            int Hp, const float* __restrict__ bpart = nullptr, int bparts = 0,
                                                            float* __restrict__ dbias = nullptr) {
  if (bpart != nullptr && blockIdx.x == 0) {
    __shared__ float red[256];
    float t = 0.f;
    for (int p = threadIdx.x; p < bparts; p += 256) t += bpart[p];
    red[threadIdx.x] = t;
    __syncthreads();
    for (int s = 128; s > 0; s >>= 1) {
      if (threadIdx.x < s) red[threadIdx.x] += red[threadIdx.x + s];
      __syncthreads();
    }
    const float tot = red[0];
    for (int n = threadIdx.x; n < H; n += 256) dbias[n] = tot;
  }
  const long total = C * H;
  for (long i = (long)blockIdx.x * blockDim.x + threadIdx.x; i < total; i += (long)gridDim.x * blockDim.x) {
    const long c = i / H;
    dW[i] = Ft > 0 ? v[(c % Ft) * Hp + c / Ft] : v[c];
  }
}

constexpr int kLast2Ld = 66;
constexpr int kLast2Stage = 32 * kLast2Ld;
template <int JT>
__global__ __launch_bounds__(256, 2) void cin_last_bwd2_kernel(const float* __restrict__ xT, const float* __restrict__ xpT, int xps,
                                                            const float* __restrict__ wsum, const float* __restrict__ wsn,
                                                            const float* __restrict__ dP, int ldp, const float* __restrict__ dPprev,
                                                            float* __restrict__ GprevT, int HSp, float* __restrict__ dxT, int M, int F,
                                                            int K, int Hp, const float* __restrict__ Radd = nullptr, int HSr = 0,
                                                            const float* __restrict__ dPadd = nullptr, float* __restrict__ colpart = nullptr) {
  __shared__ float colred[4][128];
  extern __shared__ __attribute__((aligned(16))) float smem[];
  for (int i = threadIdx.x; i < Hp * F; i += 256) smem[i] = wsum[i];
  __syncthreads();
  const int tid = threadIdx.x, lane = tid & 63, wave = tid >> 6;
  const int r = lane & 31, half = lane >> 5;
  const int wrow0 = (blockIdx.x * 4 + wave) * 32;
  if (wrow0 >= M && colpart == nullptr) return;
  const long mq = min(wrow0 + r, M - 1);
  float* stg = smem + ((Hp * F + 3) & ~3) + wave * kLast2Stage;
  const int nrow = min(32, M - wrow0);
  if (nrow > 0) {
    const float4* src = reinterpret_cast<const float4*>(xT + (long)wrow0 * F);
    const int n4 = nrow * F / 4, tail = nrow * F - 4 * n4;
    for (int i = lane; i < n4; i += 64) *reinterpret_cast<float4*>(stg + 4 * i) = src[i];
    if (lane < tail) stg[4 * n4 + lane] = xT[(long)wrow0 * F + 4 * n4 + lane];
  }
  __builtin_amdgcn_wave_barrier();
  float xr[JT];
  {
    const float* xrow = stg + min(r, max(nrow, 1) - 1) * F;
#pragma unroll
    for (int j = 0; j < JT; ++j) {
      const int f = 2 * j + half;
      xr[j] = (f < F && nrow > 0) ? xrow[min(f, F - 1)] : 0.f;
    }
  }
  __shared__ float dps[4][3][32];
  if (half == 0) {
    const int b = (int)(mq / K), k = (int)(mq - (long)b * K);
    dps[wave][0][r] = dP[(long)b * ldp + k];
    dps[wave][1][r] = dPprev != nullptr ? dPprev[(long)b * ldp + k] : 0.f;
    dps[wave][2][r] = Radd != nullptr ? dPadd[(long)b * ldp + k] : 0.f;
  }
  __builtin_amdgcn_wave_barrier();
  auto phase_t = [&]() {
  const int chunks = (Hp + 127) >> 7;
  for (int chunk = 0; chunk < chunks; ++chunk) {
    f32x16 t[4];
#pragma unroll
    for (int nb = 0; nb < 4; ++nb)
#pragma unroll
      for (int i = 0; i < 16; ++i) t[nb][i] = 0.f;
    const float4* wsb = reinterpret_cast<const float4*>(wsn + (long)chunk * (2 * JT) * 128) + (half * 32 + r);
    constexpr int QB = JT % 5 == 0 ? 5 : 4;
#pragma unroll
    for (int j0 = 0; j0 < JT; j0 += QB) {
      float4 wq[QB];
#pragma unroll
      for (int j = 0; j < QB; ++j) wq[j] = wsb[(long)(2 * (j0 + j)) * 32];
      __builtin_amdgcn_sched_barrier(0);
#pragma unroll
      for (int j = 0; j < QB; ++j) {
        const float4 w = wq[j];
        t[0] = mfma32(xr[j0 + j], w.x, t[0]);
        t[1] = mfma32(xr[j0 + j], w.y, t[1]);
        t[2] = mfma32(xr[j0 + j], w.z, t[2]);
        t[3] = mfma32(xr[j0 + j], w.w, t[3]);
      }
    }
    const int n0 = chunk * 128 + 4 * r;
    float c0 = 0.f, c1 = 0.f, c2 = 0.f, c3 = 0.f;
    float4 rq[8];
#pragma unroll
    for (int reg = 0; reg < 16; ++reg) {
      if (Radd != nullptr && (reg & 7) == 0) {
#pragma unroll
        for (int u = 0; u < 8; ++u) {
          const long mm = min(wrow0 + mfma32_row(reg + u, half), M - 1);
          rq[u] = *reinterpret_cast<const float4*>(Radd + mm * HSr + n0);
        }
      }
      const int row = mfma32_row(reg, half);
      const int m = wrow0 + row;
      const float dpr = dps[wave][0][row], dppr = dps[wave][1][row], dpa = dps[wave][2][row];
      if (m < M) {
        float* dst = GprevT + (long)m * HSp + n0;
        float v0 = fmaf(dpr, t[0][reg], dppr), v1 = fmaf(dpr, t[1][reg], dppr);
        float v2 = fmaf(dpr, t[2][reg], dppr), v3 = fmaf(dpr, t[3][reg], dppr);
        if (Radd != nullptr) {
          const float4 ra = rq[reg & 7];
          v0 = fmaf(dpa, ra.x, v0);
          v1 = fmaf(dpa, ra.y, v1);
          v2 = fmaf(dpa, ra.z, v2);
          v3 = fmaf(dpa, ra.w, v3);
        }
        c0 += v0;
        c1 += v1;
        c2 += v2;
        c3 += v3;
        if (n0 + 3 < Hp) {
          *reinterpret_cast<float4*>(dst) = make_float4(v0, v1, v2, v3);
        } else {
          if (n0 < Hp) dst[0] = v0;
          if (n0 + 1 < Hp) dst[1] = v1;
          if (n0 + 2 < Hp) dst[2] = v2;
        }
      }
    }
    if (colpart != nullptr) {
      c0 = lane_halves_sum(c0);
      c1 = lane_halves_sum(c1);
      c2 = lane_halves_sum(c2);
      c3 = lane_halves_sum(c3);
      if (half == 0) *reinterpret_cast<float4*>(&colred[wave][4 * r]) = make_float4(c0, c1, c2, c3);
      __syncthreads();
      for (int n = tid; n < 128; n += 256)
        if (chunk * 128 + n < Hp) colpart[(long)blockIdx.x * Hp + chunk * 128 + n] = (colred[0][n] + colred[1][n]) + (colred[2][n] + colred[3][n]);
      __syncthreads();
    }
  }
  };
  auto phase_u = [&]() {
  if (wrow0 >= M) return;
  f32x16 u0, u1;
#pragma unroll
  for (int i = 0; i < 16; ++i) u0[i] = u1[i] = 0.f;
  const bool two = F > 32;
  const int quads = (Hp + 3) >> 2;
#pragma unroll 1
  for (int q0 = 0; q0 < quads; q0 += 16) {
    __builtin_amdgcn_wave_barrier();
    {
      float4 v[8];
#pragma unroll
      for (int i = 0; i < 8; ++i) {
        const int row = (lane >> 4) + 4 * i, c4 = lane & 15;
        const long mm = min(wrow0 + row, M - 1);
        v[i] = 4 * q0 + 4 * c4 < xps ? *reinterpret_cast<const float4*>(xpT + mm * xps + 4 * q0 + 4 * c4) : make_float4(0.f, 0.f, 0.f, 0.f);
      }
#pragma unroll
      for (int i = 0; i < 8; ++i) {
        const int row = (lane >> 4) + 4 * i, c4 = lane & 15;
        float* d = stg + row * kLast2Ld + 4 * c4;
        *reinterpret_cast<float2*>(d) = make_float2(v[i].x, v[i].y);
        *reinterpret_cast<float2*>(d + 2) = make_float2(v[i].z, v[i].w);
      }
    }
    __builtin_amdgcn_wave_barrier();
    float2 av[16];
    const float* xprow = stg + r * kLast2Ld + 2 * half;
#pragma unroll
    for (int i = 0; i < 16; ++i) av[i] = q0 + i < quads ? *reinterpret_cast<const float2*>(xprow + 4 * i) : make_float2(0.f, 0.f);
#pragma unroll
    for (int i0 = 0; i0 < 16; i0 += 4) {
      float b0[4][2], b1[4][2];
#pragma unroll
      for (int ii = 0; ii < 4; ++ii) {
        const int h = 4 * (q0 + i0 + ii) + 2 * half;
        const float* w0 = smem + min(h, Hp - 1) * F;
        const float* w1 = smem + min(h + 1, Hp - 1) * F;
        const int k0 = (h < Hp && r < F) ? -1 : 0, k1 = (h + 1 < Hp && r < F) ? -1 : 0;
        b0[ii][0] = __builtin_bit_cast(float, __builtin_bit_cast(int, w0[min(r, F - 1)]) & k0);
        b0[ii][1] = __builtin_bit_cast(float, __builtin_bit_cast(int, w1[min(r, F - 1)]) & k1);
        b1[ii][0] = b1[ii][1] = 0.f;
        if (two) {
          const int k2 = (h < Hp && r + 32 < F) ? -1 : 0, k3 = (h + 1 < Hp && r + 32 < F) ? -1 : 0;
          b1[ii][0] = __builtin_bit_cast(float, __builtin_bit_cast(int, w0[min(r + 32, F - 1)]) & k2);
          b1[ii][1] = __builtin_bit_cast(float, __builtin_bit_cast(int, w1[min(r + 32, F - 1)]) & k3);
        }
      }
      __builtin_amdgcn_sched_barrier(0);
#pragma unroll
      for (int ii = 0; ii < 4; ++ii) {
        u0 = mfma32(av[i0 + ii].x, b0[ii][0], u0);
        u0 = mfma32(av[i0 + ii].y, b0[ii][1], u0);
        if (two) {
          u1 = mfma32(av[i0 + ii].x, b1[ii][0], u1);
          u1 = mfma32(av[i0 + ii].y, b1[ii][1], u1);
        }
      }
    }
  }
#pragma unroll
  for (int reg = 0; reg < 16; ++reg) {
    const int m = wrow0 + mfma32_row(reg, half);
    if (m < M) {
      const float dpr = dps[wave][0][mfma32_row(reg, half)];
      if (r < F) dxT[(long)m * F + r] = dpr * u0[reg];
      if (two && r + 32 < F) dxT[(long)m * F + 32 + r] = dpr * u1[reg];
    }
  }
  };
  if ((blockIdx.x >> 3) & 1) {
    phase_u();
    phase_t();
  } else {
    phase_t();
    phase_u();
  }
}

struct PoolArgs {
  const float* part[kCinMaxL];
  int chunks[kCinMaxL];
};

constexpr int kHeadSamples = 8;
static __global__ __launch_bounds__(256) void cin_head_fwd_kernel(PoolArgs pa, const float* __restrict__ dense_w,
                                                           const float* __restrict__ dense_b, float* __restrict__ pooled,
                                                           float* __restrict__ out, int B, int K, int L) {
  extern __shared__ float sh[];
  const int LK = L * K;
  const long M = (long)B * K;
  const int b0 = blockIdx.x * kHeadSamples;
  const int nb = min(kHeadSamples, B - b0);
  for (int e = threadIdx.x; e < nb * LK; e += 256) {
    const int bl = e / LK, j = e - bl * LK;
    const int l = j / K, k = j - l * K;
    const long b = b0 + bl;
    float v = 0.f;
    for (int ch = 0; ch < pa.chunks[l]; ++ch) v += pa.part[l][(long)ch * M + b * K + k];
    pooled[b * LK + j] = v;
    if (out != nullptr) sh[e] = v * dense_w[j];
  }
  if (out == nullptr) return;
  __syncthreads();
  if (threadIdx.x < nb) {
    float o = 0.f;
    for (int j = 0; j < LK; ++j) o += sh[threadIdx.x * LK + j];
    out[b0 + threadIdx.x] = o + dense_b[0];
  }
}

static __global__ __launch_bounds__(256) void cin_head_bwd_kernel(const float* __restrict__ g, const float* __restrict__ dense_w,
                                                           const float* __restrict__ pooled, float* __restrict__ dP,
                                                           float* __restrict__ part, int B, int LK, int bchunk) {
  __shared__ float red[4][256];
  const int b_lo = blockIdx.x * bchunk, b_hi = min(B, b_lo + bchunk);
  if (LK + 1 <= 64) {
    const int j = threadIdx.x & 63, w = threadIdx.x >> 6;
    float t = 0.f;
    if (j <= LK) {
      const float wj = j < LK ? dense_w[j] : 0.f;
      for (int b = b_lo + w; b < b_hi; b += 4) {
        const float gb = g[b];
        if (j < LK) {
          dP[(long)b * LK + j] = gb * wj;
          t = fmaf(gb, pooled[(long)b * LK + j], t);
        } else {
          t += gb;
        }
      }
    }
    red[w][j] = t;
    __syncthreads();
    if (w == 0 && j <= LK) part[(long)blockIdx.x * (LK + 1) + j] = ((red[0][j] + red[1][j]) + red[2][j]) + red[3][j];
  } else {
    for (int j = threadIdx.x; j <= LK; j += 256) {
      const float wj = j < LK ? dense_w[j] : 0.f;
      float t = 0.f;
      for (int b = b_lo; b < b_hi; ++b) {
        const float gb = g[b];
        if (j < LK) {
          dP[(long)b * LK + j] = gb * wj;
          t = fmaf(gb, pooled[(long)b * LK + j], t);
        } else {
          t += gb;
        }
      }
      part[(long)blockIdx.x * (LK + 1) + j] = t;
    }
  }
}


}
```

ml_function_amd/csrc/cin_launch.h:

```cpp
#pragma once
#include <hip/hip_runtime.h>

namespace fil {

inline int cin_jt_of(int F) { return ((F + 1) / 2 + 3) / 4 * 4; }

constexpr int kCinMaxFields = 64;
constexpr int cin_jt_sym(int F) { return ((F / 2 + 1 + 1) / 2 + 1) / 2 * 2; }
static_assert(cin_jt_sym(kCinMaxFields) <= 18, "the symmetric kernels' JT menu (2..18) must cover every legal field count");

inline int cin_x2_len(int F) { return F + 2 * cin_jt_sym(F); }
void cin_launch_fwd3_sym(hipStream_t st, int MB, int JT, dim3 grid, const float* xT, const float* x2T, int XL, const float* Wf, const float* bias,
                         float* xoutT, int HS, float* pool_part, int M, int F, int H, int ks = 1);

void cin_launch_fwd3(hipStream_t st, int MB, int JT, dim3 grid, const float* xT, const float* xpT, int xps, const float* Wf,
                     const float* bias, float* xoutT, int HS, float* pool_part, int M, int F, int Hp, int H,
                     const float* wsn = nullptr, const float* bias_next = nullptr, int H_next = 0, float* pool_next = nullptr);

void cin_launch_dz3(hipStream_t st, int MB, int JT, int NHMAX, dim3 grid, const float* gT, int HS, const float* Wz, const float* xT,
                    const float* xpT, int xps, const float* dPprev, int ldp, int K, float* GprevT, int HSp, float* gx0T, float* dxT,
                    int accumulate, int M, int F, int Hp, int H, int periods);

void cin_launch_last_bwd2(hipStream_t st, int JT, const float* xT, const float* xpT, int xps, const float* wsum, const float* wsn,
                          const float* dP, int ldp, const float* dPprev, float* GprevT, int HSp, float* dxT, int M, int F, int K, int Hp,
                          const float* Radd = nullptr, int HSr = 0, const float* dPadd = nullptr, float* colpart = nullptr);

void cin_launch_dz3_sym(hipStream_t st, int MB, int JT, int NHMAX, dim3 grid, const float* gT, int HS, const float* Wz, const float* xT,
                        float* gx0T, float* dxT, int accumulate, int M, int F, int H, int periods, int ks = 1);

inline int cin_gcd(int a, int b) { return b == 0 ? a : cin_gcd(b, a % b); }
inline int cin_dz_tiles_per_period(int JT) { return JT / cin_gcd(16, JT); }
inline int cin_dz_h_per_period(int JT) { return 16 * cin_dz_tiles_per_period(JT) / JT; }

inline int cin_dz_sym_rows(int F, int JT) { return F > cin_dz_h_per_period(JT) + 2 * JT ? F : cin_dz_h_per_period(JT) + 2 * JT; }

inline bool cin_tail_supported(int F) { return F >= 1 && F <= 62; }
inline int cin_tail_ncb(int F) { return (F + 2 + 15) / 16; }
inline int cin_tail_jt4(int F) {
  const int v = (F + 3) / 4;
  return v == 11 ? 12 : (v == 13 ? 14 : v);
}
inline int cin_tail_nq(int F) { return ((F + 2) / 2 + 3) / 4; }
struct TailFwdArgs {
  const float *xT, *xpT;
  int xps;
  const float *Uf, *consts;
  float* Y;
  int JP;
  float *pool_p, *pool_L;
  int M, F, Hp;
  int ks;
};
void cin_launch_tail_fwd(hipStream_t st, int RB, int JT4, int NCB, const TailFwdArgs& a);
struct TailDwArgs {
  const float *Apk, *xT, *xpT;
  int xps;
  float* part;
  int M, F, Hp, JP, rows_per_split, blocks_x, items;
  bool settle;
};
void cin_launch_tail_dw(hipStream_t st, int NCB, const TailDwArgs& a);
struct TailDzArgs {
  const float *Uz, *xT, *xpT;
  int xps;
  const float* Y;
  int JP;
  const float* dP;
  int ldp, K, lp, lL;
  float* GprevT;
  int HSp;
  float* dxT;
  int M, F, Hp, periods;
  int smode;
  int ks;
};
void cin_launch_tail_dz(hipStream_t st, int JT, int NQ, const TailDzArgs& a);

}
```

ml_function_amd/csrc/cin_qmerge.h:

```cpp
#pragma once
#include "cin_kernels.h"
#include "cin_launch.h"
#include "cin_qtail.h"

namespace fil {

constexpr int kDwqDepth = 6;
constexpr int kDwqThreads = 512;
struct DwqPlan {
  int tiles, ncol_full, rem, splits, pairs, rows_per_split, wgs_full, wgs;
};
inline int cin_dwq_rem_wgs(int rem, int pairs) { return rem == 0 ? 0 : (rem == 1 ? (pairs + 3) / 4 : (rem == 2 ? (pairs + 1) / 2 : pairs)); }
inline DwqPlan cin_dwq_plan(long M, int C, int cus) {
  DwqPlan p;
  p.tiles = (C + 31) / 32;
  p.ncol_full = p.tiles / 4;
  p.rem = p.tiles % 4;
  const long unit = 2 * kDwqDepth;
  const long slots = cus;
  int best = 1;
  for (int s = 1; s <= 512; ++s) {
    if ((long)p.ncol_full * s + cin_dwq_rem_wgs(p.rem, s) > slots) break;
    best = s;
  }
  long want = std::max<long>(2L * best, (M + (1L << 20) - 1) >> 20);
  long rows = std::max(unit, ((M + want - 1) / want + unit - 1) / unit * unit);
  p.rows_per_split = (int)rows;
  p.splits = (int)std::max<long>(1, (M + rows - 1) / rows);
  p.pairs = (p.splits + 1) / 2;
  p.wgs_full = p.ncol_full * p.pairs;
  p.wgs = p.wgs_full + cin_dwq_rem_wgs(p.rem, p.pairs);
  return p;
}

inline DwqPlan cin_dwq_plan4(long M, int C, int cus) {
  DwqPlan p;
  p.tiles = (C + 31) / 32;
  p.ncol_full = p.tiles / 2;
  p.rem = p.tiles % 2;
  const long unit = 2 * kDwqDepth;
  int best = 1;
  for (int q = 1; q <= 256; ++q) {
    if ((long)p.ncol_full * q + (p.rem ? (q + 1) / 2 : 0) > cus) break;
    best = q;
  }
  long want = std::max<long>(4L * best, (M + (1L << 20) - 1) >> 20);
  long rows = std::max(unit, ((M + want - 1) / want + unit - 1) / unit * unit);
  p.rows_per_split = (int)rows;
  p.splits = (int)std::max<long>(1, (M + rows - 1) / rows);
  p.pairs = (p.splits + 3) / 4;
  p.wgs_full = p.ncol_full * p.pairs;
  p.wgs = p.wgs_full + (p.rem ? (p.pairs + 1) / 2 : 0);
  return p;
}

template <int DEPTH = kDwqDepth, int FOLD = 2>
__global__ __launch_bounds__(kDwqThreads, 2) void cin_dwq_kernel(const float* __restrict__ gT, const float* __restrict__ x1T, int HS, const float* __restrict__ xe,
                                                                int XE, float* __restrict__ part, int M, int F, int symD, int rows_per_split, int splits,
                                                                int ncol_full, int rem, int wgs_full, int wgs) {
  __shared__ float fold[4][128][64];
  const int tid = threadIdx.x, lane = tid & 63, wave = tid >> 6;
  const int r = lane & 31, half = lane >> 5;
  const int Cp = F * symD, C = Cp + F;
  const int item = (blockIdx.x & 7) * (gridDim.x >> 3) + (blockIdx.x >> 3);
  if (item >= wgs) return;
  const int wl = FOLD == 4 ? (wave & 1) : (wave & 3), up = FOLD == 4 ? (wave >> 1) : (wave >> 2);
  int tile, pair;
  bool idle = false;
  if constexpr (FOLD == 4) {
    if (item < wgs_full) {
      tile = (item % ncol_full) * 2 + wl;
      pair = item / ncol_full;
    } else {
      tile = ncol_full * 2;
      pair = 2 * (item - wgs_full) + wl;
    }
  } else if (item < wgs_full) {
    tile = (item % ncol_full) * 4 + wl;
    pair = item / ncol_full;
  } else {
    const int j = item - wgs_full;
    if (rem == 1) {
      tile = ncol_full * 4;
      pair = 4 * j + wl;
    } else if (rem == 2) {
      tile = ncol_full * 4 + (wl & 1);
      pair = 2 * j + (wl >> 1);
    } else {
      tile = ncol_full * 4 + wl;
      pair = j;
      idle = wl == 3;
    }
  }
  tile = __builtin_amdgcn_readfirstlane(tile);
  pair = __builtin_amdgcn_readfirstlane(pair);
  const int split = FOLD * pair + up;
  const int npairs = (splits + FOLD - 1) / FOLD;
  const int c0 = tile * 32;
  const int m_lo = split * rows_per_split;
  const int m_hi = min(M, m_lo + rows_per_split);
  const bool work = !idle && pair < npairs && split < splits && m_lo < m_hi;
  const long mrem = work ? (long)m_hi - m_lo : 0;
  const long mbase = work ? m_lo : 0;
  const __amdgpu_buffer_rsrc_t rg = make_rsrc_uniform(gT + mbase * HS, mrem * HS * 4);
  const __amdgpu_buffer_rsrc_t r1 = make_rsrc_uniform(x1T + mbase * HS, mrem * HS * 4);
  const __amdgpu_buffer_rsrc_t rx = make_rsrc_uniform(xe + mbase * XE, mrem * XE * 4);
  const int c = c0 + r;
  const int cc = c < C ? c : C - 1;
  int hh, ff, sel;
  if (cc < Cp) {
    hh = cc / symD;
    ff = (hh + (cc - hh * symD)) % F;
    sel = 0;
  } else {
    hh = F;
    ff = cc - Cp;
    sel = 1;
  }
  const int ho = (half * XE + hh) * 4, fo = (half * XE + ff) * 4, so = (half * XE + F + 1 + sel) * 4;
  const int go = (half * HS + 4 * r) * 4;
  const int steps = work ? (m_hi - m_lo + 1) >> 1 : 0;
  const int groups = (steps + DEPTH - 1) / DEPTH;

  f32x16 acc[8];
#pragma unroll
  for (int nb = 0; nb < 8; ++nb)
#pragma unroll
    for (int i = 0; i < 16; ++i) acc[nb][i] = 0.f;
  f32x4s qg[DEPTH], q1[DEPTH];
  float qh[DEPTH], qf[DEPTH], qs[DEPTH];
  auto fetch = [&](int s, int d) {
    const int row = 2 * s;
    qg[d] = __builtin_bit_cast(f32x4s, __builtin_amdgcn_raw_buffer_load_b128(rg, go, row * HS * 4, 0));
    q1[d] = __builtin_bit_cast(f32x4s, __builtin_amdgcn_raw_buffer_load_b128(r1, go, row * HS * 4, 0));
    qh[d] = __builtin_bit_cast(float, __builtin_amdgcn_raw_buffer_load_b32(rx, ho, row * XE * 4, 0));
    qf[d] = __builtin_bit_cast(float, __builtin_amdgcn_raw_buffer_load_b32(rx, fo, row * XE * 4, 0));
    qs[d] = __builtin_bit_cast(float, __builtin_amdgcn_raw_buffer_load_b32(rx, so, row * XE * 4, 0));
  };
#pragma unroll
  for (int d = 0; d < DEPTH; ++d) fetch(d, d);
  float ac = qh[0] * qf[0], ac2 = ac * qs[0], an, an2;
#pragma unroll 1
  for (int g = 0; g < groups; ++g) {
#pragma unroll
    for (int d = 0; d < DEPTH; ++d) {
      const f32x4s g4 = qg[d], x4 = q1[d];
      an = qh[(d + 1) % DEPTH] * qf[(d + 1) % DEPTH];
      an2 = an * qs[(d + 1) % DEPTH];
      __builtin_amdgcn_sched_barrier(0);
      acc[0] = mfma32(ac, g4[0], acc[0]);
      acc[1] = mfma32(ac, g4[1], acc[1]);
      acc[2] = mfma32(ac, g4[2], acc[2]);
      acc[3] = mfma32(ac, g4[3], acc[3]);
      acc[4] = mfma32(ac2, x4[0], acc[4]);
      acc[5] = mfma32(ac2, x4[1], acc[5]);
      acc[6] = mfma32(ac2, x4[2], acc[6]);
      acc[7] = mfma32(ac2, x4[3], acc[7]);
      ac = an;
      ac2 = an2;
      __builtin_amdgcn_sched_barrier(0);
      fetch(g * DEPTH + d + DEPTH, d);
      __builtin_amdgcn_sched_barrier(0);
    }
  }
  if constexpr (FOLD == 4) {
    const int slot = (up >> 1) * 2 + wl;
    if (up & 1) {
#pragma unroll
      for (int nb = 0; nb < 8; ++nb)
#pragma unroll
        for (int i = 0; i < 16; ++i) fold[slot][nb * 16 + i][lane] = acc[nb][i];
    }
    __syncthreads();
    if (!(up & 1)) {
#pragma unroll
      for (int nb = 0; nb < 8; ++nb)
#pragma unroll
        for (int i = 0; i < 16; ++i) acc[nb][i] += fold[slot][nb * 16 + i][lane];
    }
    __syncthreads();
    if (up == 2) {
#pragma unroll
      for (int nb = 0; nb < 8; ++nb)
#pragma unroll
        for (int i = 0; i < 16; ++i) fold[wl][nb * 16 + i][lane] = acc[nb][i];
    }
    __syncthreads();
    if (up != 0 || pair >= npairs) return;
#pragma unroll
    for (int nb = 0; nb < 8; ++nb)
#pragma unroll
      for (int i = 0; i < 16; ++i) acc[nb][i] += fold[wl][nb * 16 + i][lane];
  } else {
    if (up == 1) {
#pragma unroll
      for (int nb = 0; nb < 8; ++nb)
#pragma unroll
        for (int i = 0; i < 16; ++i) fold[wl][nb * 16 + i][lane] = acc[nb][i];
    }
    __syncthreads();
    if (up == 1 || idle || pair >= npairs) return;
#pragma unroll
    for (int nb = 0; nb < 8; ++nb)
#pragma unroll
      for (int i = 0; i < 16; ++i) acc[nb][i] += fold[wl][nb * 16 + i][lane];
  }
  float* pout = part + (long)pair * C * 256;
#pragma unroll
  for (int reg = 0; reg < 16; ++reg) {
    const int cr = c0 + mfma32_row(reg, half);
    if (cr < C) {
      float* dst = pout + (long)cr * 256 + 4 * r;
      if (cr < Cp) *reinterpret_cast<float4*>(dst) = make_float4(acc[0][reg], acc[1][reg], acc[2][reg], acc[3][reg]);
      *reinterpret_cast<float4*>(dst + 128) = make_float4(acc[4][reg], acc[5][reg], acc[6][reg], acc[7][reg]);
    }
  }
}

static __global__ __launch_bounds__(256) void cin_reduce_expand_q_kernel(const float* __restrict__ part, int parts, int F, int D, int H1, int H2,
                                                                          float* __restrict__ dW1, float* __restrict__ dT, float* __restrict__ vT,
                                                                          const float* __restrict__ bpart, int nbp, float* __restrict__ dbias1,
                                                                          int nb1, const float* __restrict__ hpart, int nhp, int LK,
                                                                          float* __restrict__ ddw, float* __restrict__ ddb) {
  const int Cp = F * D, C = Cp + F;
  const int nbw = (C + 3) / 4;
  if ((int)blockIdx.x >= nbw + nb1) {
    cin_reduce_body(hpart, ddw, (long)LK + 1, nhp, ddb, (long)LK, (int)blockIdx.x - nbw - nb1);
    return;
  }
  if ((int)blockIdx.x >= nbw) {
    cin_reduce_body(bpart, dbias1, (long)H1, nbp, nullptr, 0, (int)blockIdx.x - nbw);
    return;
  }
  const int lane = threadIdx.x & 63, wave = threadIdx.x >> 6;
  const int c = blockIdx.x * 4 + wave;
  if (c >= C) return;
  const long ps = (long)C * 256;
  const float* p0 = part + (long)c * 256 + 4 * lane;
  f32x4 t[8];
#pragma unroll
  for (int u = 0; u < 8; ++u) t[u] = f32x4{0.f, 0.f, 0.f, 0.f};
  int p = 0;
  for (; p + 7 < parts; p += 8) {
#pragma unroll
    for (int u = 0; u < 8; ++u) t[u] += *reinterpret_cast<const f32x4*>(p0 + (long)(p + u) * ps);
  }
  for (; p < parts; ++p) t[0] += *reinterpret_cast<const f32x4*>(p0 + (long)p * ps);
  const f32x4 v = ((t[0] + t[1]) + (t[2] + t[3])) + ((t[4] + t[5]) + (t[6] + t[7]));
  const int col = 4 * lane, n0 = col & 127;
  const bool second = col >= 128;
  const int H = second ? H2 : H1;
  if (c >= Cp) {
    if (second) {
#pragma unroll
      for (int e = 0; e < 4; ++e)
        if (n0 + e < H2) vT[(long)(c - Cp) * H2 + n0 + e] = v[e];
    }
    return;
  }
  const int h = c / D, d = c - h * D;
  const int f = (h + d) % F;
  float* dst = second ? dT : dW1;
  const bool twin = d != 0 && 2 * d != F;
  float* r0 = dst + ((long)h * F + f) * H + n0;
  float* r1 = dst + ((long)f * F + h) * H + n0;
  if ((H & 3) == 0 && n0 + 3 < H) {
    *reinterpret_cast<f32x4*>(r0) = v;
    if (twin) *reinterpret_cast<f32x4*>(r1) = v;
  } else {
#pragma unroll
    for (int e = 0; e < 4; ++e)
      if (n0 + e < H) {
        r0[e] = v[e];
        if (twin) r1[e] = v[e];
      }
  }
}

constexpr int kXeThreads = 1024;
template <int NP = 3>
static __global__ __launch_bounds__(kXeThreads) void cin_qtail_xe_kernel(const float* __restrict__ xT, const float* __restrict__ dPL,
                                                                  const float* __restrict__ dPp, int ldp, int K, float* __restrict__ xe,
                                                                  float* __restrict__ dcpart, int M, int F, int nscale,
                                                                  const float* __restrict__ g, const float* __restrict__ dense_w,
                                                                  const float* __restrict__ pooled, float* __restrict__ dP, float* __restrict__ hpart,
                                                                  int LK, int lL, int lp, const float* __restrict__ W0, float* __restrict__ Wz,
                                                                  int H0, int JTs, int HS0, int tiles0, int npz = -1,
                                                                  const float* __restrict__ Tq = nullptr, int HT = 0, u32x4* __restrict__ Wzb1 = nullptr,
                                                                  u32x4* __restrict__ Wzb2 = nullptr) {
  extern __shared__ __attribute__((aligned(16))) float smem[];
  if ((int)blockIdx.x >= nscale) {
    if (threadIdx.x >= 256) return;
    if (npz < 0) npz = gridDim.x - nscale;
    const int b = blockIdx.x - nscale;
    if (b < npz) cin_pack_wz_sym_body(W0, Wz, F, H0, JTs, HS0, tiles0, b, npz);
    else {
      const int nq = ((int)gridDim.x - nscale - npz) >> 1, q = b - npz;
      if (q < nq) cin_qs_pack_wz_body<NP>(W0, H0, Wzb1, tiles0, F, JTs, q, nq);
      else if (q < 2 * nq) cin_qs_pack_wz_body<NP>(Tq, HT, Wzb2, tiles0, F, JTs, q - nq, nq);
    }
    return;
  }
  const int nl = g != nullptr ? LK / K : 0;
  const int hl = nl + 1, XE = F + 3;
  const int tid = threadIdx.x;
  const long m0 = (long)blockIdx.x * 256;
  const int nrows = (int)min((long)256, (long)M - m0);
  float* xs = smem;
  float* dls = xs + 256 * F;
  float* dps = dls + 256;
  float* hd = dps + 256;
  {
    const float* src = xT + m0 * F;
    const int n = nrows * F;
    if ((reinterpret_cast<uintptr_t>(xT) & 15) == 0) {
      const int n4 = n >> 2;
      for (int i0 = tid; i0 < n4; i0 += 4 * kXeThreads) {
        float4 v[4];
#pragma unroll
        for (int u = 0; u < 4; ++u) v[u] = i0 + u * kXeThreads < n4 ? reinterpret_cast<const float4*>(src)[i0 + u * kXeThreads] : make_float4(0.f, 0.f, 0.f, 0.f);
#pragma unroll
        for (int u = 0; u < 4; ++u)
          if (i0 + u * kXeThreads < n4) reinterpret_cast<float4*>(xs)[i0 + u * kXeThreads] = v[u];
      }
      for (int i = 4 * n4 + tid; i < n; i += kXeThreads) xs[i] = src[i];
    } else {
      for (int i = tid; i < n; i += kXeThreads) xs[i] = src[i];
    }
    for (int i = n + tid; i < 256 * F; i += kXeThreads) xs[i] = 0.f;
  }
  if (tid < 256) {
    const long m = m0 + tid;
    float dl = 0.f, dp = 0.f;
    if (m < M) {
      const long b = m / K;
      const int k = (int)(m - b * K);
      if (g != nullptr) {
        const float gb = g[b];
        for (int l = 0; l < nl; ++l) {
          const float d = gb * dense_w[l * K + k];
          dP[b * LK + l * K + k] = d;
          hd[tid * hl + l] = gb * pooled[b * LK + l * K + k];
        }
        hd[tid * hl + nl] = k == 0 ? gb : 0.f;
        dl = gb * dense_w[lL * K + k];
        dp = gb * dense_w[lp * K + k];
      } else {
        dl = dPL[b * ldp + k];
        dp = dPp[b * ldp + k];
      }
    } else if (g != nullptr) {
      for (int l = 0; l <= nl; ++l) hd[tid * hl + l] = 0.f;
    }
    dls[tid] = dl;
    dps[tid] = dp;
  }
  __syncthreads();
  __shared__ float cs[4][64];
  if (tid < kXeThreads - 256) {
    constexpr int NT = kXeThreads - 256;
    float* dst = xe + m0 * XE;
    const int n4 = nrows * XE >> 2;
    const float rxe = 1.f / (float)XE;
    for (int i4 = tid; i4 < n4; i4 += NT) {
      int rr = (int)(((float)(4 * i4) + 0.5f) * rxe);
      int c = 4 * i4 - rr * XE;
      float e[4];
#pragma unroll
      for (int u = 0; u < 4; ++u) {
        e[u] = c < F ? xs[rr * F + c] : c == F ? 1.f : c == F + 1 ? dls[rr] : dps[rr];
        if (++c == XE) {
          c = 0;
          ++rr;
        }
      }
      reinterpret_cast<float4*>(dst)[i4] = make_float4(e[0], e[1], e[2], e[3]);
    }
    for (int i = 4 * n4 + tid; i < nrows * XE; i += NT) {
      const int rr = i / XE, c = i - rr * XE;
      dst[i] = c < F ? xs[rr * F + c] : c == F ? 1.f : c == F + 1 ? dls[rr] : dps[rr];
    }
  } else {
    const int t2 = tid - (kXeThreads - 256);
    {
      const int f = t2 & 63, q = t2 >> 6;
      float t0 = 0.f, t1 = 0.f;
      if (f < F) {
        for (int rr = 64 * q; rr < 64 * q + 64; rr += 2) {
          t0 += xs[rr * F + f] * dls[rr];
          t1 += xs[(rr + 1) * F + f] * dls[rr + 1];
        }
      } else if (f < F + 2) {
        const float* dv = f == F ? dls : dps;
        for (int rr = 64 * q; rr < 64 * q + 64; rr += 2) {
          t0 += dv[rr];
          t1 += dv[rr + 1];
        }
      }
      cs[q][f] = t0 + t1;
    }
    if (g != nullptr) {
      const int k0 = (int)(m0 % K);
      for (int j = t2; j <= LK; j += 256) {
        float t = 0.f;
        if (j < LK) {
          const int l = j / K, k = j - l * K;
          for (int rr = (k - k0 + K) % K; rr < 256; rr += K) t += hd[rr * hl + l];
        } else {
          for (int rr = (K - k0) % K; rr < 256; rr += K) t += hd[rr * hl + nl];
        }
        hpart[(long)blockIdx.x * (LK + 1) + j] = t;
      }
    }
  }
  __syncthreads();
  if (tid < F + 2) dcpart[(long)blockIdx.x * kQtConst + tid] = (cs[0][tid] + cs[1][tid]) + (cs[2][tid] + cs[3][tid]);
}

constexpr int kDz2FieldStride = 128 * 2;
inline int cin_dz2_rows(int F, int JT) {
  const int hpp = cin_dz_h_per_period(JT);
  return std::max(cin_dz_sym_rows(F, JT), (F + hpp - 1) / hpp * hpp);
}

__device__ __forceinline__ void cin_dz2_finish(const float* smem, int wave, int lane, int wrow0, int M, int F, int K, const float* __restrict__ dsc, int ldp,
                                               float* __restrict__ dxT, int accumulate, float* __restrict__ dx, const float* __restrict__ cvec) {
  constexpr int FS = kDz2FieldStride;
  const float* img = smem + wave * 32 * 2 + 1;
  const int nrow = min(32, M - wrow0);
  if (dx != nullptr) {
    const int rr = lane & 31;
    const int mm = wrow0 + rr;
    const bool ok = rr < nrow;
    const long mc = ok ? mm : M - 1;
    const long bb = mc / K;
    const int kk = (int)(mc - bb * K);
    const float sc = dsc[bb * ldp + kk];
    float* dxb = dx + (bb * F) * K + kk;
    const float* add = dxT + mc * F;
    for (int f0 = lane >> 5; f0 < F; f0 += 16) {
      float a8[8];
#pragma unroll
      for (int u = 0; u < 8; ++u) a8[u] = accumulate ? add[min(f0 + 2 * u, F - 1)] : 0.f;
#pragma unroll
      for (int u = 0; u < 8; ++u) {
        const int f = f0 + 2 * u;
        if (f < F) {
          const float v = a8[u] + img[f * FS + rr * 2] + sc * cvec[f];
          if (ok) dxb[(long)f * K] = v;
        }
      }
    }
    return;
  }
  float* dst = dxT + (long)wrow0 * F;
  for (int idx = lane; idx < nrow * F; idx += 64) {
    const int rr = idx / F, f = idx - rr * F;
    const float v = img[f * FS + rr * 2];
    dst[idx] = accumulate ? dst[idx] + v : v;
  }
}

template <int JT, int G>
__global__ __launch_bounds__(256, 2) void cin_dz2_kernel(const float* __restrict__ g1T, const float* __restrict__ g2T, int HS,
                                                         const float* __restrict__ dsc, int ldp, int K, const float* __restrict__ Wz1,
                                                         const float* __restrict__ Wz2, const float* __restrict__ xT, float* __restrict__ dxT,
                                                         int accumulate, int M, int F, int H1, int H2, int periods, int FR,
                                                         float* __restrict__ dx, const float* __restrict__ cvec) {
  extern __shared__ __attribute__((aligned(16))) float smem[];
  constexpr int P = JT / gcd_c(16, JT);
  constexpr int HPP = 16 * P / JT;
  constexpr int NQ = 16;
  constexpr int FS = kDz2FieldStride;
  const int tid = threadIdx.x, lane = tid & 63, wave = tid >> 6;
  const int r = lane & 31, half = lane >> 5;
  const int wrow0 = (blockIdx.x * 4 + wave) * 32;
  if (wrow0 >= M) return;
  float* lrow = smem + (wave * 32 + r) * 2;
  const int m = wrow0 + r;
  const bool vq = m < M;
  const long mq = vq ? m : M - 1;
  f32x4s gq[16];
  {
    const f32x4s* grow4 = reinterpret_cast<const f32x4s*>(g1T + mq * HS + half * 64);
#pragma unroll
    for (int s4 = 0; s4 < 16; ++s4) gq[s4] = grow4[s4];
  }
  for (int f0 = half; f0 < FR; f0 += 16) {
    float xt[8];
#pragma unroll
    for (int u = 0; u < 8; ++u) xt[u] = xT[mq * F + min(f0 + 2 * u, F - 1)];
#pragma unroll
    for (int u = 0; u < 8; ++u) {
      const int f = f0 + 2 * u;
      if (f < FR) {
        const int keep = (vq && f < F) ? -1 : 0;
        *reinterpret_cast<float2*>(lrow + f * FS) = make_float2(__builtin_bit_cast(float, __builtin_bit_cast(int, xt[u]) & keep), 0.f);
      }
    }
  }
  float dpl;
  {
    const long bb = mq / K;
    dpl = dsc[bb * ldp + (mq - bb * K)];
  }
  __builtin_amdgcn_wave_barrier();
  const long wbytes = ((long)periods * P + 1) * 32 * 128 * 4;
  const int wo = (r * 128 + half * 64) * 4;
  float greg[64];
  auto to_greg = [&](const f32x4s (&gv4)[16], int Hk, float sc) {
#pragma unroll
    for (int s4 = 0; s4 < 16; ++s4)
#pragma unroll
      for (int e = 0; e < 4; ++e) {
        const int keep = (vq && half * 64 + 4 * s4 + e < Hk) ? -1 : 0;
        const float gv = gv4[s4][e];
        greg[4 * s4 + e] = __builtin_bit_cast(float, __builtin_bit_cast(int, gv) & keep) * sc;
      }
  };
  to_greg(gq, H1, 1.f);

#pragma unroll 1
  for (int pass = 0; pass < 2; ++pass) {
    const float* gT = pass == 0 ? g1T : g2T;
    const int Hk = pass == 0 ? H1 : H2;
    const float sc = pass == 0 ? 1.f : dpl;
    const __amdgpu_buffer_rsrc_t rw = make_rsrc(pass == 0 ? Wz1 : Wz2, wbytes);
    auto ldw = [&](int t, int s4) {
      return __builtin_bit_cast(f32x4s, __builtin_amdgcn_raw_buffer_load_b128(rw, wo + 16 * s4, t * (32 * 128 * 4), 0));
    };
    constexpr int QD = 8;
    f32x4s q[QD];
#pragma unroll
    for (int s4 = 0; s4 < QD; ++s4) q[s4] = ldw(0, s4);
    if (pass == 1) {
      const f32x4s* grow4 = reinterpret_cast<const f32x4s*>(gT + mq * HS + half * 64);
      f32x4s g2[16];
#pragma unroll
      for (int s4 = 0; s4 < 16; ++s4) g2[s4] = grow4[s4];
      to_greg(g2, Hk, sc);
    }
    float gx = 0.f;
    f32x16 dprev;
#pragma unroll
    for (int i = 0; i < 16; ++i) dprev[i] = 0.f;
    float xprev[HPP], xcur[HPP];
#pragma unroll
    for (int hl = 0; hl < HPP; ++hl) xprev[hl] = xcur[hl] = 0.f;
    int hprev = 0;
    float2 lv[G];
    float* la[G];
#pragma unroll
    for (int k = 0; k < G; ++k) {
      lv[k] = make_float2(0.f, 0.f);
      la[k] = lrow;
    }
    float *abase = lrow, *awrap = lrow;
    int symh = 0;
    auto sym_period = [&](int hb) {
      symh = hb + half;
      abase = lrow + symh * FS;
      awrap = abase - F * FS;
    };
    auto slot_fetch = [&](int tp, int rr, int k) {
      const int sp = 16 * tp + rr;
      const int off = sp / JT + 2 * (sp % JT);
      la[k] = (symh >= F - off ? awrap : abase) + off * FS;
      lv[k] = *reinterpret_cast<const float2*>(la[k]);
    };
    auto slot_apply = [&](const f32x16& d, const float (&xpv)[HPP], int hb, int tp, int rr, int k) {
      const int sp = 16 * tp + rr;
      const int hl = sp / JT, j = sp % JT;
      const float dz = d[rr];
      gx = fmaf(dz, lv[k].x, gx);
      la[k][1] = fmaf(dz, xpv[hl], lv[k].y);
      if (j == JT - 1) {
        const float t = lane_halves_sum(gx);
        gx = 0.f;
        if (half == 0) __hip_atomic_fetch_add(lrow + (hb + hl) * FS + 1, t, __ATOMIC_RELAXED, __HIP_MEMORY_SCOPE_WAVEFRONT);
      }
    };
    sym_period(hprev);
#pragma unroll
    for (int k = 0; k < G; ++k) slot_fetch(P - 1, k, k);
#pragma unroll 1
    for (int per = 0; per < periods; ++per) {
      const int hbase = per * HPP;
#pragma unroll
      for (int hl = 0; hl < HPP; ++hl) xcur[hl] = lrow[(hbase + hl) * FS];
#pragma unroll
      for (int tp = 0; tp < P; ++tp) {
        const int t = per * P + tp;
        f32x16 d;
#pragma unroll
        for (int i = 0; i < 16; ++i) d[i] = 0.f;
#pragma unroll
        for (int s4 = 0; s4 < NQ; ++s4) {
          const f32x4s w = q[s4 % QD];
          d = mfma32(w[0], greg[4 * s4 + 0], d);
          d = mfma32(w[1], greg[4 * s4 + 1], d);
          d = mfma32(w[2], greg[4 * s4 + 2], d);
          d = mfma32(w[3], greg[4 * s4 + 3], d);
          q[s4 % QD] = s4 + QD < NQ ? ldw(t, s4 + QD) : ldw(t + 1, s4 + QD - NQ);
          if (s4 % G == G - 1) {
#pragma unroll
            for (int k = 0; k < G; ++k) {
              const int rr = s4 - G + 1 + k;
              if (tp == 0) slot_apply(dprev, xprev, hprev, P - 1, rr, k);
              else slot_apply(dprev, xcur, hbase, tp - 1, rr, k);
            }
            if (s4 < 15) {
#pragma unroll
              for (int k = 0; k < G; ++k) slot_fetch(tp == 0 ? P - 1 : tp - 1, s4 + 1 + k, k);
            } else {
              if (tp == 0) sym_period(hbase);
#pragma unroll
              for (int k = 0; k < G; ++k) slot_fetch(tp, k, k);
            }
            __builtin_amdgcn_sched_barrier(0);
          }
        }
        dprev = d;
      }
#pragma unroll
      for (int hl = 0; hl < HPP; ++hl) xprev[hl] = xcur[hl];
      hprev = hbase;
    }
#pragma unroll
    for (int r0 = 0; r0 < 16; r0 += G) {
#pragma unroll
      for (int k = 0; k < G; ++k) slot_apply(dprev, xprev, hprev, P - 1, r0 + k, k);
      if (r0 + G < 16) {
#pragma unroll
        for (int k = 0; k < G; ++k) slot_fetch(P - 1, r0 + G + k, k);
      }
    }
  }
  __builtin_amdgcn_wave_barrier();
  cin_dz2_finish(smem, wave, lane, wrow0, M, F, K, dsc, ldp, dxT, accumulate, dx, cvec);
}

bool cin_launch_dz2(hipStream_t st, int JT, const float* g1T, const float* g2T, int HS, const float* dsc, int ldp, int K, const float* Wz1,
                    const float* Wz2, const float* xT, float* dxT, int accumulate, int M, int F, int H1, int H2, int periods,
                    float* dx = nullptr, const float* cvec = nullptr);

struct CinHeadFold {
  float* pooled;
  float* out;
  const float* dense_w;
  const float* dense_b;
  int kshift, LK, op, oL;
};

template <int NW>
__device__ __forceinline__ void cin_fwdq_epilogue(f32x16 (&acc)[8], const __amdgpu_buffer_rsrc_t& rx, int vhalf, int wo, int r, int half, int wave, int wrow0,
                                                  const float* __restrict__ bias1, const float* __restrict__ wsn, int JTG, const float* __restrict__ cvec,
                                                  float* __restrict__ x1T, float* __restrict__ RT, int HS, float* __restrict__ pool1,
                                                  float* __restrict__ pool_p, float* __restrict__ pool_L, int M, int F, int H, const CinHeadFold& hf,
                                                  float (&lin_s)[NW][32], float (&pv_s)[NW][3][32]) {
  const int lane = half * 32 + r;
  f32x16 t[4];
#pragma unroll
  for (int nb = 0; nb < 4; ++nb)
#pragma unroll
    for (int i = 0; i < 16; ++i) t[nb][i] = 0.f;
  const __amdgpu_buffer_rsrc_t rs = make_rsrc(wsn, (long)2 * JTG * 128 * 4);
  const __amdgpu_buffer_rsrc_t rc = make_rsrc(cvec, (long)kQtConst * 4);
  float xs4[2][4], cs4[2][4];
  f32x4s ws4[2][4];
  auto ldgroup = [&](int j0, int b) {
#pragma unroll
    for (int u = 0; u < 4; ++u) {
      const int j = __builtin_amdgcn_readfirstlane(j0) + u;
      xs4[b][u] = __builtin_bit_cast(float, __builtin_amdgcn_raw_buffer_load_b32(rx, vhalf, j * 512, 0));
      cs4[b][u] = __builtin_bit_cast(float, __builtin_amdgcn_raw_buffer_load_b32(rc, half * 4, j * 8, 0));
      ws4[b][u] = __builtin_bit_cast(f32x4s, __builtin_amdgcn_raw_buffer_load_b128(rs, wo, j * 1024, 0));
    }
  };
  float lin = 0.f;
  ldgroup(0, 0);
#pragma unroll 1
  for (int j0 = 0; j0 < JTG; j0 += 8) {
    ldgroup(j0 + 4, 1);
#pragma unroll
    for (int u = 0; u < 4; ++u) {
      const bool in = 2 * (j0 + u) + half < F;
      lin = fmaf(in ? xs4[0][u] : 0.f, in ? cs4[0][u] : 0.f, lin);
      const float a = xs4[0][u];
      t[0] = mfma32(a, ws4[0][u][0], t[0]);
      t[1] = mfma32(a, ws4[0][u][1], t[1]);
      t[2] = mfma32(a, ws4[0][u][2], t[2]);
      t[3] = mfma32(a, ws4[0][u][3], t[3]);
    }
    if (j0 + 4 < JTG) {
      ldgroup(j0 + 8, 0);
#pragma unroll
      for (int u = 0; u < 4; ++u) {
        const bool in = 2 * (j0 + 4 + u) + half < F;
        lin = fmaf(in ? xs4[1][u] : 0.f, in ? cs4[1][u] : 0.f, lin);
        const float a = xs4[1][u];
        t[0] = mfma32(a, ws4[1][u][0], t[0]);
        t[1] = mfma32(a, ws4[1][u][1], t[1]);
        t[2] = mfma32(a, ws4[1][u][2], t[2]);
        t[3] = mfma32(a, ws4[1][u][3], t[3]);
      }
    }
  }
  lin = lane_halves_sum(lin);
  if (half == 0) lin_s[wave][r] = lin;
  __builtin_amdgcn_wave_barrier();

  float bv[4];
#pragma unroll
  for (int nb = 0; nb < 4; ++nb) bv[nb] = 4 * r + nb < H ? bias1[4 * r + nb] : 0.f;
  const float cp = cvec[kQtConst + 1], cL = cvec[kQtConst];
#pragma unroll
  for (int reg = 0; reg < 16; ++reg) {
    const int row = mfma32_row(reg, half);
    const int m = wrow0 + row;
    const float a0 = acc[0][reg] + bv[0], a1 = acc[1][reg] + bv[1], a2 = acc[2][reg] + bv[2], a3 = acc[3][reg] + bv[3];
    const float b0 = acc[4][reg], b1 = acc[5][reg], b2 = acc[6][reg], b3 = acc[7][reg];
    if (m < M) {
      *reinterpret_cast<float4*>(x1T + (long)m * HS + 4 * r) = make_float4(a0, a1, a2, a3);
      *reinterpret_cast<float4*>(RT + (long)m * HS + 4 * r) = make_float4(b0, b1, b2, b3);
    }
    float p1 = (a0 + a1) + (a2 + a3);
    float eL = a0 * b0, ep = a0 * t[0][reg];
    eL = fmaf(a1, b1, eL);
    eL = fmaf(a2, b2, eL);
    eL = fmaf(a3, b3, eL);
    ep = fmaf(a1, t[1][reg], ep);
    ep = fmaf(a2, t[2][reg], ep);
    ep = fmaf(a3, t[3][reg], ep);
    p1 = half_wave_sum_hi(p1);
    eL = half_wave_sum_hi(eL);
    ep = half_wave_sum_hi(ep);
    if (r == 31 && m < M) {
      const float vp = ep + cp, vL = (eL + lin_s[wave][row]) + cL;
      if (hf.pooled != nullptr) {
        float* pr = hf.pooled + (long)(m >> hf.kshift) * hf.LK + (m & ((1 << hf.kshift) - 1));
        pr[0] = p1;
        pr[hf.op] = vp;
        pr[hf.oL] = vL;
        pv_s[wave][0][row] = p1;
        pv_s[wave][1][row] = vp;
        pv_s[wave][2][row] = vL;
      } else {
        pool1[m] = p1;
        pool_p[m] = vp;
        pool_L[m] = vL;
      }
    }
  }
  if (hf.out == nullptr) return;
  __builtin_amdgcn_wave_barrier();
  {
    const int k = (wrow0 + r) & ((1 << hf.kshift) - 1);
    const int o0 = half == 0 ? 0 : hf.op;
    pv_s[wave][half][r] *= hf.dense_w[o0 + k];
    if (half == 0) pv_s[wave][2][r] *= hf.dense_w[hf.oL + k];
  }
  __builtin_amdgcn_wave_barrier();
  const int K = 1 << hf.kshift;
  if (lane < (32 >> hf.kshift) && wrow0 + lane * K < M) {
    float o = 0.f;
    for (int l = 0; l < 3; ++l)
      for (int k = 0; k < K; ++k) o += pv_s[wave][l][lane * K + k];
    hf.out[(wrow0 >> hf.kshift) + lane] = o + hf.dense_b[0];
  }
}

template <int JT>
__global__ __launch_bounds__(256, 2) void cin_fwdq_kernel(const float* __restrict__ x2T, int XL, const float* __restrict__ W1f, const float* __restrict__ WTf,
                                                          const float* __restrict__ bias1, const float* __restrict__ wsn, int JTG,
                                                          const float* __restrict__ cvec, float* __restrict__ x1T, float* __restrict__ RT, int HS,
                                                          float* __restrict__ pool1, float* __restrict__ pool_p, float* __restrict__ pool_L, int M, int F,
                                                          int H, CinHeadFold hf) {
  constexpr int DEPTH = JT % 5 == 0 ? 5 : (JT % 4 == 0 ? 4 : (JT % 7 == 0 ? 7 : (JT % 3 == 0 ? 3 : 2)));
  static_assert(JT % DEPTH == 0, "queue depth must divide the steps per h");
  __shared__ float lin_s[4][32];
  __shared__ float pv_s[4][3][32];
  const int tid = threadIdx.x, lane = tid & 63, wave = tid >> 6;
  const int r = lane & 31, half = lane >> 5;
  const int wrow0 = (blockIdx.x * 4 + wave) * 32;
  if (wrow0 >= M) return;
  const int wrow_u = __builtin_amdgcn_readfirstlane(wrow0);
  const __amdgpu_buffer_rsrc_t rx = make_rsrc_uniform(x2T + (long)(wrow_u >> 6) * XL * 64, (long)XL * 256);
  const long wbytes = (long)F * (2 * JT) * 128 * 4;
  const __amdgpu_buffer_rsrc_t rw1 = make_rsrc(W1f, wbytes), rwt = make_rsrc(WTf, wbytes);
  const int wo = (half * 32 + r) * 16;
  const int vrow = ((wrow_u & 63) + r) * 4, vhalf = vrow + half * 256;
  auto ldw = [&](const __amdgpu_buffer_rsrc_t& rw, int s) {
    return __builtin_bit_cast(f32x4s, __builtin_amdgcn_raw_buffer_load_b128(rw, wo, s * 1024, 0));
  };
  auto ldfrag = [&](int h, float (&xf)[JT], float& xp) {
    const int hb = __builtin_amdgcn_readfirstlane(h) * 256;
    xp = __builtin_bit_cast(float, __builtin_amdgcn_raw_buffer_load_b32(rx, vrow, hb, 0));
#pragma unroll
    for (int j = 0; j < JT; ++j) xf[j] = __builtin_bit_cast(float, __builtin_amdgcn_raw_buffer_load_b32(rx, vhalf + 512 * j, hb, 0));
  };
  f32x16 acc[8];
#pragma unroll
  for (int nb = 0; nb < 8; ++nb)
#pragma unroll
    for (int i = 0; i < 16; ++i) acc[nb][i] = 0.f;
  f32x4s q1[DEPTH], qt[DEPTH];
#pragma unroll
  for (int d = 0; d < DEPTH; ++d) {
    q1[d] = ldw(rw1, d);
    qt[d] = ldw(rwt, d);
  }
  float xa[JT], xb[JT], pa, pb;
  ldfrag(0, xa, pa);
#pragma unroll
  for (int d = 0; d < DEPTH; ++d) {
    settle(q1[d]);
    settle(qt[d]);
  }
  settle(pa);
  float ac = pa * xa[0], an;
  auto run_h = [&](int h, float (&xc)[JT], float& pc, float (&xn_)[JT], float& pn) {
    ldfrag(min(h + 1, F - 1), xn_, pn);
    const int sb = h * JT;
#pragma unroll
    for (int j = 0; j < JT; ++j) {
      const f32x4s w1 = q1[j % DEPTH], wt = qt[j % DEPTH];
      an = j + 1 < JT ? pc * xc[j + 1 < JT ? j + 1 : 0] : pn * xn_[0];
      __builtin_amdgcn_sched_barrier(0);
      acc[0] = mfma32(ac, w1[0], acc[0]);
      acc[1] = mfma32(ac, w1[1], acc[1]);
      acc[2] = mfma32(ac, w1[2], acc[2]);
      acc[3] = mfma32(ac, w1[3], acc[3]);
      acc[4] = mfma32(ac, wt[0], acc[4]);
      acc[5] = mfma32(ac, wt[1], acc[5]);
      acc[6] = mfma32(ac, wt[2], acc[6]);
      acc[7] = mfma32(ac, wt[3], acc[7]);
      ac = an;
      __builtin_amdgcn_sched_barrier(0);
      q1[j % DEPTH] = ldw(rw1, sb + j + DEPTH);
      qt[j % DEPTH] = ldw(rwt, sb + j + DEPTH);
      __builtin_amdgcn_sched_barrier(0);
    }
  };
  int h = 0;
#pragma unroll 1
  for (; h + 1 < F; h += 2) {
    run_h(h, xa, pa, xb, pb);
    run_h(h + 1, xb, pb, xa, pa);
  }
  if (h < F) run_h(h, xa, pa, xb, pb);

  cin_fwdq_epilogue<4>(acc, rx, vhalf, wo, r, half, wave, wrow0, bias1, wsn, JTG, cvec, x1T, RT, HS, pool1, pool_p, pool_L, M, F, H, hf, lin_s, pv_s);
}

bool cin_launch_fwdq(hipStream_t st, int JT, const float* x2T, int XL, const float* W1f, const float* WTf, const float* bias1, const float* wsn, int JTG,
                     const float* cvec, float* x1T, float* RT, int HS, float* pool1, float* pool_p, float* pool_L, int M, int F, int H, CinHeadFold hf);

}
```

ml_function_amd/csrc/cin_qmerge.hip:

```cpp
#include "cin_qmerge.h"

namespace fil {

template <int JT, int G>
static void dz2g(hipStream_t st, const float* g1T, const float* g2T, int HS, const float* dsc, int ldp, int K, const float* Wz1, const float* Wz2,
                 const float* xT, float* dxT, int accumulate, int M, int F, int H1, int H2, int periods, float* dx, const float* cvec) {
  const int FR = cin_dz2_rows(F, JT);
  const size_t sh = (size_t)FR * kDz2FieldStride * sizeof(float);
  if (sh > 48 * 1024)
    (void)hipFuncSetAttribute(reinterpret_cast<const void*>(cin_dz2_kernel<JT, G>), hipFuncAttributeMaxDynamicSharedMemorySize, (int)sh);
  hipLaunchKernelGGL((cin_dz2_kernel<JT, G>), dim3(cdiv(M, 128)), dim3(kCinThreads), sh, st, g1T, g2T, HS, dsc, ldp, K, Wz1, Wz2, xT, dxT, accumulate, M, F, H1,
                     H2, periods, FR, dx, cvec);
}
template <int JT>
static void dz2(hipStream_t st, const float* g1T, const float* g2T, int HS, const float* dsc, int ldp, int K, const float* Wz1, const float* Wz2,
                const float* xT, float* dxT, int accumulate, int M, int F, int H1, int H2, int periods, float* dx, const float* cvec) {
  if (JT >= 4 && F >= cin_dz_h_per_period(JT) + 2 * JT) dz2g<JT, (JT >= 4 ? 4 : 1)>(st, g1T, g2T, HS, dsc, ldp, K, Wz1, Wz2, xT, dxT, accumulate, M, F, H1, H2, periods, dx, cvec);
  else dz2g<JT, 1>(st, g1T, g2T, HS, dsc, ldp, K, Wz1, Wz2, xT, dxT, accumulate, M, F, H1, H2, periods, dx, cvec);
}

bool cin_launch_dz2(hipStream_t st, int JT, const float* g1T, const float* g2T, int HS, const float* dsc, int ldp, int K, const float* Wz1,
                    const float* Wz2, const float* xT, float* dxT, int accumulate, int M, int F, int H1, int H2, int periods, float* dx, const float* cvec) {
#define FIL_Z2(JTV) \
  case JTV: dz2<JTV>(st, g1T, g2T, HS, dsc, ldp, K, Wz1, Wz2, xT, dxT, accumulate, M, F, H1, H2, periods, dx, cvec); break;
  switch (JT) { FIL_Z2(2) FIL_Z2(4) FIL_Z2(6) FIL_Z2(8) FIL_Z2(10) FIL_Z2(12) FIL_Z2(14) FIL_Z2(16) FIL_Z2(18) default: return false; }
#undef FIL_Z2
  return true;
}

bool cin_launch_fwdq(hipStream_t st, int JT, const float* x2T, int XL, const float* W1f, const float* WTf, const float* bias1, const float* wsn, int JTG,
                     const float* cvec, float* x1T, float* RT, int HS, float* pool1, float* pool_p, float* pool_L, int M, int F, int H, CinHeadFold hf) {
#define FIL_FQ(JTV)                                                                                                                             \
  case JTV:                                                                                                                                     \
    hipLaunchKernelGGL((cin_fwdq_kernel<JTV>), dim3(cdiv(M, 128)), dim3(kCinThreads), 0, st, x2T, XL, W1f, WTf, bias1, wsn, JTG, cvec, x1T, RT, HS, \
                       pool1, pool_p, pool_L, M, F, H, hf);                                                                                       \
    break;
  switch (JT) { FIL_FQ(2) FIL_FQ(4) FIL_FQ(6) FIL_FQ(8) FIL_FQ(10) FIL_FQ(12) FIL_FQ(14) FIL_FQ(16) FIL_FQ(18) default: return false; }
#undef FIL_FQ
  return true;
}

}
```

ml_function_amd/csrc/cin_qtail.h:

```cpp
#pragma once
#include "cin_kernels.h"
#include "cin_split.h"

namespace fil {

__device__ __forceinline__ void qt_stage(const float* __restrict__ src, float* dst, int n) {
  for (int i0 = threadIdx.x; i0 < n; i0 += 8 * 256) {
    float v[8];
#pragma unroll
    for (int u = 0; u < 8; ++u) v[u] = i0 + u * 256 < n ? src[i0 + u * 256] : 0.f;
#pragma unroll
    for (int u = 0; u < 8; ++u)
      if (i0 + u * 256 < n) dst[i0 + u * 256] = v[u];
  }
}
__device__ __forceinline__ void qt_stage_rows(const float* __restrict__ src, float* dst, int rows, int cols, int ld) {
  const int n = rows * cols;
  for (int i0 = threadIdx.x; i0 < n; i0 += 8 * 256) {
    float v[8];
#pragma unroll
    for (int u = 0; u < 8; ++u) v[u] = i0 + u * 256 < n ? src[i0 + u * 256] : 0.f;
#pragma unroll
    for (int u = 0; u < 8; ++u) {
      const int i = i0 + u * 256;
// ... 92 lines not shown
      }
    }
    float* wl = smem;
    float* bp = wl + Hq * F;
    qt_stage(wsumL, wl, Hq * F);
    qt_stage(bias_p, bp, Hq);
    __syncthreads();
    for (int f = threadIdx.x; f < F; f += 256) {
      float t = 0.f;
      for (int n = 0; n < Hq; ++n) t = fmaf(bp[n], wl[n * F + f], t);
      cvec[f] = t;
    }
    if (threadIdx.x >= 64 && threadIdx.x < 192) {
      const int lane = threadIdx.x & 63, which = (threadIdx.x >> 6) - 1;
      const float* b = which == 0 ? bias_L : bias_p;
      const int nb = which == 0 ? HL : Hq;
      float t = 0.f;
      for (int n = lane; n < nb; n += 64) t += b[n];
      float tot = 0.f;
      for (int i = 0; i < 64; ++i) tot += __shfl(t, i);
      if (lane == 0) cvec[kQtConst + which] = tot;
    }
    for (int i = threadIdx.x; i < Hpp; i += 256) zbias[i] = 0.f;
    return;
  }
  const int FT = (F + 31) & ~31, K16 = (Hq + 15) & ~15, ldn = K16 + 1, on = F * Hq;
  float* wp = smem;
  float* wlT = smem + FT * ldn;
  float* tn = wlT + FT * ldn;
  const float* wsrc = Wp + (long)h * F * Hq;
  const float rH = 1.f / (float)Hq, rF = 1.f / (float)F;
  constexpr int NO = 20;
  float av[NO], bv[NO];
#pragma unroll
  for (int u = 0; u < NO; ++u) {
    const int i = threadIdx.x + u * 256;
    av[u] = i < on ? wsrc[i] : 0.f;
    bv[u] = i < on ? wsumL[i] : 0.f;
  }
  for (int i = threadIdx.x; i < 2 * FT * ldn; i += 256) smem[i] = 0.f;
  __syncthreads();
  auto put_a = [&](int i, float v) {
    const int fp = (int)(((float)i + 0.5f) * rH);
    wp[fp * ldn + (i - fp * Hq)] = v;
  };
  auto put_b = [&](int i, float v) {
    const int n = (int)(((float)i + 0.5f) * rF);
    wlT[(i - n * F) * ldn + n] = v;
  };
#pragma unroll
  for (int u = 0; u < NO; ++u) {
    const int i = threadIdx.x + u * 256;
    if (i < on) {
      put_a(i, av[u]);
      put_b(i, bv[u]);
    }
  }
  for (int i = threadIdx.x + NO * 256; i < on; i += 256) {
    put_a(i, wsrc[i]);
    put_b(i, wsumL[i]);
  }
  __syncthreads();
  {
    const int lane = threadIdx.x & 63, wave = threadIdx.x >> 6, r = lane & 31, half = lane >> 5;
    const int ntile = FT >> 5;
    if (wave < ntile * ntile) {
      const int mt = wave / ntile, nt = wave - mt * ntile;
      f32x16 acc;
#pragma unroll
      for (int i = 0; i < 16; ++i) acc[i] = 0.f;
      const float* ar = wp + (mt * 32 + r) * ldn + half;
      const float* br = wlT + (nt * 32 + r) * ldn + half;
      for (int k0 = 0; k0 < K16; k0 += 16) {
        float fa[8], fb[8];
#pragma unroll
        for (int u = 0; u < 8; ++u) {
          fa[u] = ar[k0 + 2 * u];
          fb[u] = br[k0 + 2 * u];
        }
#pragma unroll
        for (int u = 0; u < 8; ++u) acc = mfma32(fa[u], fb[u], acc);
      }
      const int f = nt * 32 + r;
#pragma unroll
      for (int reg = 0; reg < 16; ++reg) {
        const int fp = mt * 32 + mfma32_row(reg, half);
        if (fp < F && f < F) {
          T[(long)(fp * F + f) * Hpp + h] = acc[reg];
          if (fold) tn[fp * F + f] = acc[reg];
        }
      }
    }
  }
  if (!fold) return;
  __syncthreads();
  auto sym = [&](int hh, int d) -> float {
    if (hh >= F || d > F / 2) return 0.f;
    int f = hh + d;
    if (f >= F) f -= F;
    if (d == 0) return tn[hh * F + hh];
    const float v = tn[hh * F + f] + tn[f * F + hh];
    return 2 * d == F ? 0.5f * v : v;
  };
  {
    const int JT2 = 2 * pf.JTs;
    const float rj = 1.f / (float)JT2;
    float* dst = pf.Wf + (long)(h >> 7) * F * JT2 * 128 + (h & 127);
    for (int e = threadIdx.x; e < F * JT2; e += 256) {
      const int hh = (int)(((float)e + 0.5f) * rj), d = e - hh * JT2;
      dst[(long)e * 128] = sym(hh, d);
    }
  }
  {
    const float rj = 1.f / (float)pf.JTs;
    for (int row = threadIdx.x; row < pf.tiles * 32; row += 256) {
      const int i = row & 31, t = row >> 5;
      const int rr = (i & 3) + 4 * (i >> 3), hf = (i >> 2) & 1;
      const int slot = 16 * t + rr;
      const int hh = (int)(((float)slot + 0.5f) * rj), j = slot - hh * pf.JTs;
      pf.Wz[(long)row * pf.NCOL + h] = sym(hh, 2 * j + hf);
    }
  }
}

static __global__ __launch_bounds__(256) void cin_qtail_t_kernel(const float* __restrict__ Wp, const float* __restrict__ wsumL,
                                                                 const float* __restrict__ bias_p, const float* __restrict__ bias_L, int HL,
                                                                 float* __restrict__ T, float* __restrict__ cvec, float* __restrict__ zbias,
                                                                 int Hpp, int F, int Hq) {
  extern __shared__ __attribute__((aligned(16))) float smem[];
  cin_qtail_t_body(Wp, wsumL, bias_p, bias_L, HL, T, cvec, zbias, Hpp, F, Hq, blockIdx.x, smem);
}

static __global__ __launch_bounds__(256) void cin_qtail_t_x_kernel(const float* __restrict__ Wp, const float* __restrict__ wsumL,
                                                                   const float* __restrict__ bias_p, const float* __restrict__ bias_L, int HL,
                                                                   float* __restrict__ T, float* __restrict__ cvec, float* __restrict__ zbias,
                                                                   int Hpp, int F, int Hq, int nT, const float* __restrict__ x, float* __restrict__ xT,
                                                                   int K, float* __restrict__ x2T, int XL, int xt_in, int ks = -1, long M = 0,
                                                                   QtPackFold pf = QtPackFold{nullptr, nullptr, 0, 0, 0, 0}) {
  extern __shared__ __attribute__((aligned(16))) float smem[];
  const int b = blockIdx.x;
  if (b < nT) {
    cin_qtail_t_body(Wp, wsumL, bias_p, bias_L, HL, T, cvec, zbias, Hpp, F, Hq, b, smem, pf);
  } else if (ks >= 0) {
    cin_transpose_block_body(x, xT, x2T, F, ks, b - nT, M, XL, smem);
  } else if (xt_in && M > 0) {
    cin_wrap_block_body(x, x2T, F, b - nT, M, XL, smem);
  } else if (xt_in) {
    cin_wrap_rows_body(x, x2T, F, K, b - nT, XL);
  } else {
    cin_transpose_in_body(x, xT, F, K, b - nT, smem, x2T, XL);
  }
}

template <int JT>
__global__ __launch_bounds__(256, 2) void cin_qtail_pool2_kernel(const float* __restrict__ xT, const float* __restrict__ xpT, int xps,
                                                                 const float* __restrict__ wsn, const float* __restrict__ R, int HSr,
                                                                 const float* __restrict__ cvec, float* __restrict__ pool_p,
                                                                 float* __restrict__ pool_L, int M, int F, int Hp) {
  __shared__ float lin_s[4][32];
  const int tid = threadIdx.x, lane = tid & 63, wave = tid >> 6;
  const int r = lane & 31, half = lane >> 5;
  const int wrow0 = (blockIdx.x * 4 + wave) * 32;
  if (wrow0 >= M) return;
  const long mq = min(wrow0 + r, M - 1);
  float xr[JT];
  float lin = 0.f;
#pragma unroll
  for (int j = 0; j < JT; ++j) {
    const int f = 2 * j + half;
    xr[j] = f < F ? xT[mq * F + f] : 0.f;
    lin = fmaf(xr[j], f < F ? cvec[f] : 0.f, lin);
  }
  lin = lane_halves_sum(lin);
  if (half == 0) lin_s[wave][r] = lin;
  f32x16 t[4];
#pragma unroll
  for (int nb = 0; nb < 4; ++nb)
#pragma unroll
    for (int i = 0; i < 16; ++i) t[nb][i] = 0.f;
  const float4* wsb = reinterpret_cast<const float4*>(wsn) + (half * 32 + r);
  constexpr int QB = JT % 5 == 0 ? 5 : 4;
#pragma unroll
  for (int j0 = 0; j0 < JT; j0 += QB) {
    float4 wq[QB];
#pragma unroll
    for (int j = 0; j < QB; ++j) wq[j] = wsb[(long)(2 * (j0 + j)) * 32];
    __builtin_amdgcn_sched_barrier(0);
#pragma unroll
    for (int j = 0; j < QB; ++j) {
      const float4 w = wq[j];
      t[0] = mfma32(xr[j0 + j], w.x, t[0]);
      t[1] = mfma32(xr[j0 + j], w.y, t[1]);
      t[2] = mfma32(xr[j0 + j], w.z, t[2]);
      t[3] = mfma32(xr[j0 + j], w.w, t[3]);
    }
  }
  __builtin_amdgcn_wave_barrier();
  const float cp = cvec[kQtConst + 1], cL = cvec[kQtConst];
  const int n0 = 4 * r;
#pragma unroll
  for (int reg = 0; reg < 16; ++reg) {
    const int row = mfma32_row(reg, half);
    const int m = wrow0 + row;
    const long mc = min(m, M - 1);
    float4 a = make_float4(0.f, 0.f, 0.f, 0.f), b = make_float4(0.f, 0.f, 0.f, 0.f);
    if (n0 < Hp) {
      a = *reinterpret_cast<const float4*>(xpT + mc * xps + n0);
      b = *reinterpret_cast<const float4*>(R + mc * HSr + n0);
    }
    float ep = a.x * t[0][reg], eL = a.x * b.x;
    ep = fmaf(a.y, t[1][reg], ep);
    ep = fmaf(a.z, t[2][reg], ep);
    ep = fmaf(a.w, t[3][reg], ep);
    eL = fmaf(a.y, b.y, eL);
    eL = fmaf(a.z, b.z, eL);
    eL = fmaf(a.w, b.w, eL);
    ep = half_wave_sum_hi(ep);
    eL = half_wave_sum_hi(eL);
    if (r == 31 && m < M) {
      pool_p[m] = ep + cp;
      pool_L[m] = (eL + lin_s[wave][row]) + cL;
    }
  }
}

static __global__ __launch_bounds__(256) void cin_qtail_scale_kernel(const float* __restrict__ xT, const float* __restrict__ dPL,
                                                                     const float* __restrict__ dPp, int ldp, int K, float* __restrict__ xs,
                                                                     float* __restrict__ dcpart, int M, int F, int nscale,
                                                                     const float* __restrict__ hpart, float* __restrict__ ddw, float* __restrict__ ddb,
                                                                     int LK, int nhp, int nhead, const float* __restrict__ W0, float* __restrict__ Wz,
                                                                     int H0, int JTs, int HS0, int tiles0) {
  extern __shared__ __attribute__((aligned(16))) float smem[];
  if ((int)blockIdx.x >= nscale + nhead) {
    cin_pack_wz_sym_body(W0, Wz, F, H0, JTs, HS0, tiles0, blockIdx.x - nscale - nhead, gridDim.x - nscale - nhead);
    return;
  }
  if ((int)blockIdx.x >= nscale) {
    cin_reduce_body(hpart, ddw, (long)LK + 1, nhp, ddb, (long)LK, blockIdx.x - nscale);
    return;
  }
  const int ld = F + 3;
  const long m = (long)blockIdx.x * 256 + threadIdx.x;
  float* row = smem + threadIdx.x * ld;
  if (m < M) {
    const long b = m / K;
    const float dl = dPL[b * ldp + (m - b * K)], dp = dPp[b * ldp + (m - b * K)];
    for (int f = 0; f < F; ++f) {
      const float v = xT[m * F + f] * dl;
      xs[m * (F + 1) + f] = v;
      row[f] = v;
    }
    xs[m * (F + 1) + F] = dp;
    row[F] = dl;
    row[F + 1] = dp;
  } else {
    for (int f = 0; f < F + 2; ++f) row[f] = 0.f;
  }
  __syncthreads();
  __shared__ float cs[4][64];
  {
    const int f = threadIdx.x & 63, q = threadIdx.x >> 6;
    float t0 = 0.f, t1 = 0.f;
    if (f < F + 2) {
      for (int rr = 64 * q; rr < 64 * q + 64; rr += 2) {
        t0 += smem[rr * ld + f];
        t1 += smem[(rr + 1) * ld + f];
      }
    }
    cs[q][f] = t0 + t1;
  }
  __syncthreads();
  if (threadIdx.x < F + 2) dcpart[(long)blockIdx.x * kQtConst + threadIdx.x] = (cs[0][threadIdx.x] + cs[1][threadIdx.x]) + (cs[2][threadIdx.x] + cs[3][threadIdx.x]);
}

static __global__ __launch_bounds__(256) void cin_qtail_params_kernel(const float* __restrict__ Wp, const float* __restrict__ wsumL,
                                                                      const float* __restrict__ dT, const float* __restrict__ vT,
                                                                      float* __restrict__ dWp, float* __restrict__ partL, int Hpp, int F, int Hq,
                                                                      const float* __restrict__ dcpart, int ndc, float* __restrict__ dcfin) {
  extern __shared__ __attribute__((aligned(16))) float smem[];
  if ((int)blockIdx.x == 2 * Hpp) {
    float* red = smem;
    const int lane = threadIdx.x & 63, wave = threadIdx.x >> 6;
    float a0 = 0.f, a1 = 0.f, a2 = 0.f, a3 = 0.f;
    if (lane < F + 2) {
      int p = wave;
      for (; p + 60 < ndc; p += 64) {
        float u[16];
#pragma unroll
        for (int e = 0; e < 16; ++e) u[e] = dcpart[(long)(p + 4 * e) * kQtConst + lane];
#pragma unroll
        for (int e = 0; e < 16; e += 4) {
          a0 += u[e];
          a1 += u[e + 1];
          a2 += u[e + 2];
          a3 += u[e + 3];
        }
      }
      for (; p < ndc; p += 4) a0 += dcpart[(long)p * kQtConst + lane];
    }
    red[wave * 64 + lane] = (a0 + a1) + (a2 + a3);
    __syncthreads();
    if (wave == 0) dcfin[lane] = (red[lane] + red[64 + lane]) + (red[128 + lane] + red[192 + lane]);
    return;
  }
  const int h = blockIdx.x >> 1, phase = blockIdx.x & 1;
  const int FT = (F + 31) & ~31, HT = (Hq + 31) & ~31, FK16 = (F + 15) & ~15, ldd = FT + 1;
// ... 157 lines not shown
```

Before: 5.768 million.

## Save scaled output gradient from forward to shrink last-layer backward work

When the dense head has output_dim 1, the merged forward kernel writes an extra per-row quantity (ghat) into the saved R buffer, and a flag records whether it was produced. The backward pass then uses a cheaper last-layer kernel variant that scales by the saved per-sample gradient instead of recomputing three dP terms. The dW kernels gain one extra column, and the bias reduction is dropped. When the flag is off, a fallback kernel recomputes R from T and x. This adds template variants, a runtime flag read on the device, and reuse of the R buffer, so correctness depends on the flag and the buffer aliasing being right.

Result: faster. 5.827 million, median of 6 (+1.0%).

```diff
diff --git a/ml_function_amd/csrc/cin.hip b/ml_function_amd/csrc/cin.hip
--- a/ml_function_amd/csrc/cin.hip
+++ b/ml_function_amd/csrc/cin.hip
@@ -180,8 +180,10 @@
   return tail_used(s, mode) && s.L == 3 && tune.sym && s.F >= 2 && s.F + 2 <= kQtConst && s.H[0] <= 128 && 3 * s.F + 1 <= s.HSmax() && (mode & FIL_CIN_NOQTAIL) == 0 &&
          knobs().qtail != 0;
 }
+static int qmerge_xe(int F, bool gh) { return F + 3 + (gh ? 1 : 0); }
 static bool qmerge_used(const CinShape& s, int mode, const CinTune& tune) {
-  return qtail_used(s, mode, tune) && 3 * s.F + 3 <= s.HSmax() && (mode & FIL_CIN_NOQMERGE) == 0 && knobs().qmerge != 0;
+  return qtail_used(s, mode, tune) && qmerge_xe(s.F, true) + 2 * s.F <= s.HSmax() && (mode & FIL_CIN_NOQMERGE) == 0 &&
+         knobs().qmerge != 0;
 }
 constexpr int kCinPrecBf16 = 1 << 20;
 static int qsplit_planes(int mode) { return (mode & kCinPrecBf16) != 0 ? 1 : 3; }
@@ -203,6 +205,10 @@
 static size_t qtail_saved_floats(const CinShape& s) {
   return (size_t)s.M() * s.HS(0) + (size_t)s.F * s.F * s.H[0] + (size_t)s.H[1] * s.F + 128 + (size_t)s.H[0] * s.F + qtail_wsn_floats(s) +
          qtail_wz_floats(s);
+}
+constexpr int kQtGhatFlag = kQtConst + 2;
+static bool ghat_used(const CinShape& s, bool qmerge, bool qsplit, int output_dim) {
+  return qmerge && !qsplit && output_dim == 1 && knobs().fwdq != 0 && knobs().dz2 != 0 && s.HS(0) == 128;
 }
 struct TailDwPlan {
   int blocks_x, splits, rows_per_split;
@@ -275,7 +281,7 @@
   const int csym = s.F * (s.F / 2 + 1);
   pmax = std::max(pmax, (size_t)dw_plan(s.M(), csym, s.H[0]).splits * csym * s.H[0]);
   pmax = std::max(pmax, (size_t)dw_plan(s.M(), csym + s.F, s.H[0]).splits * (csym + s.F) * s.H[0]);
-  if (s.L == 3) pmax = std::max(pmax, (size_t)cin_dwq_plan(s.M(), csym + s.F, cu_count()).pairs * (csym + s.F) * 256);
+  if (s.L == 3) pmax = std::max(pmax, (size_t)cin_dwq_plan(s.M(), csym + s.F + 1, cu_count()).pairs * (csym + s.F + 1) * 256);
   if (s.L == 3) pmax = std::max(pmax, (size_t)cin_dwqb_plan(s.M(), csym + s.F, cu_count()).splits * (csym + s.F) * 256);
   pmax = std::max(pmax, (size_t)dw_plan(s.M(), s.Hp(s.L - 1), s.F).splits * s.Hp(s.L - 1) * s.F);
   pmax = std::max(pmax, (size_t)dw_plan(s.M(), s.F, s.Hp(s.L - 1)).splits * s.Hp(s.L - 1) * s.F);
@@ -430,7 +436,7 @@
   float* xT_own = sv.take<float>((size_t)M * F);
   const float* xT = xt_in ? x : xT_own;
   float *tailY = nullptr, *tailUz = nullptr, *tailBmT = nullptr;
-  float *qtR = nullptr, *qtT = nullptr, *qtWsumL = nullptr, *qtCvec = nullptr, *qtWsumP = nullptr, *qtWsnP = nullptr, *qtWzT = nullptr;
+  float *qtR = nullptr, *qtT = nullptr, *qtWsumL = nullptr, *qtCvec = nullptr, *qtWsumP = nullptr, *qtWsnP = nullptr, *qtWzT = nullptr, *qtGhat = nullptr;
   if (qtail) {
     Carver pv(saved);
     (void)pv.take<float>((size_t)M * F);
@@ -443,6 +449,7 @@
     qtWsumP = qtCvec + 128;
     qtWsnP = qtWsumP + (size_t)H[0] * F;
     qtWzT = qtWsnP + qtail_wsn_floats(s);
+    qtGhat = qtR;
   } else if (tail) {
     Carver pv(saved);
     (void)pv.take<float>((size_t)M * F);
@@ -533,7 +540,9 @@
                                  const_cast<float*>(pa.part[p]), const_cast<float*>(pa.part[lL]), (int)M, F, H[0], hf))
             return fail(FIL_ERR_UNSUPPORTED, "fil_cin_fwd: no split-bf16 forward kernel for JT=%d (F=%d)", JTs, F);
         } else if (!cin_launch_fwdq(st, JTs, x2T, XL, Wf, WfT, bias[0], qtWsnP, JT, qtCvec, x1T, qtR, HS0, const_cast<float*>(pa.part[0]),
-                                    const_cast<float*>(pa.part[p]), const_cast<float*>(pa.part[lL]), (int)M, F, H[0], hf))
+                                    const_cast<float*>(pa.part[p]), const_cast<float*>(pa.part[lL]), (int)M, F, H[0], hf,
+                                    hf.out != nullptr && ghat_used(s, qmerge, qsplit, output_dim) ? qtGhat : nullptr,
+                                    qtCvec + kQtGhatFlag))
           return fail(FIL_ERR_UNSUPPORTED, "fil_cin_fwd: no merged forward kernel for JT=%d (F=%d)", JTs, F);
         pa.chunks[0] = pa.chunks[p] = pa.chunks[lL] = 1;
       }
@@ -754,7 +763,7 @@
   const float* xT = xt_in ? x : xT_own;
   const float* maps[kCinMaxL];
   const float *tailY = nullptr, *tailUz = nullptr, *tailWsum = nullptr;
-  const float *qtR = nullptr, *qtT = nullptr, *qtWsumL = nullptr, *qtCvec = nullptr, *qtWsumP = nullptr, *qtWsnP = nullptr, *qtWzT = nullptr;
+  const float *qtR = nullptr, *qtT = nullptr, *qtWsumL = nullptr, *qtCvec = nullptr, *qtWsumP = nullptr, *qtWsnP = nullptr, *qtWzT = nullptr, *qtGhat = nullptr;
   if (qtail) {
     maps[0] = sv.take<float>((size_t)M * s.HS(0));
     const float* q = sv.take<float>(qtail_saved_floats(s));
@@ -765,6 +774,7 @@
     qtWsumP = qtCvec + 128;
     qtWsnP = qtWsumP + (size_t)H[0] * F;
     qtWzT = qtWsnP + qtail_wsn_floats(s);
+    qtGhat = qtR;
   } else if (tail) {
     for (int l = 0; l < tg.p; ++l) maps[l] = sv.take<float>((size_t)M * s.HS(l));
     tailY = sv.take<float>((size_t)M * tg.JP);
@@ -806,13 +816,16 @@
     const int JTs = cin_jt_sym(F);
     const int periods = cdiv(F, cin_dz_h_per_period(JTs));
     const int tiles0 = periods * cin_dz_tiles_per_period(JTs) + 1;
-    const int XE = F + 3;
+    const bool gh = ghat_used(s, qmerge, qsplit, output_dim);
+    const float* ghflag = qtCvec + kQtGhatFlag;
+    const bool rsel = !gh && ghat_used(s, qmerge, qsplit, 1);
+    const int XE = qmerge_xe(F, gh);
     float* xe = Gbuf[1];
     float* gxR = xe + (size_t)M * XE;
     float* dxR = gxR + (size_t)M * F;
     {
       ProfScope ps("cin_tail_a", st, (double)M * (2 * F + 3) * sizeof(float));
-      const size_t sh = (size_t)256 * (F + 3 + (output_dim == 1 ? L : 0)) * sizeof(float);
+      const size_t sh = (size_t)256 * (F + 3 + (output_dim == 1 ? L : 0) + (gh ? 1 : 0)) * sizeof(float);
       allow_lds(cin_qtail_xe_kernel<3>, sh);
       allow_lds(cin_qtail_xe_kernel<1>, sh);
       const int np = (int)std::min<long>(((long)tiles0 * 32 * HS0 + 255) / 256, 1024);
@@ -824,12 +837,20 @@
       else
         hipLaunchKernelGGL(cin_qtail_xe_kernel<3>, dim3(qt_ndc + np + nq2), dim3(kXeThreads), sh, st, xT, dPL, dPp, (int)LK, K, xe, qt_dcpart, (int)M, F,
                            qt_ndc, output_dim == 1 ? g : nullptr, dense_w, pooled, dP, qt_hpart, (int)LK, lL, p, W[0], Wz, H[0], JTs, HS0, tiles0, np, qtT,
-                           Hpp, Wzb1, Wzb2);
-    }
-    FIL_CHECK_LAUNCH();
-    {
-      ProfScope ps("cin_last_bwd", st, 6.0 * (double)M * Hpp * F);
-      cin_launch_last_bwd2(st, JT, xT, xpT, xps, qtWsumP, qtWsnP, dPp, (int)LK, dPprev, Gbuf[cur], HS0, dxT, (int)M, F, K, Hpp, qtR, HS0, dPL, small);
+                           Hpp, Wzb1, Wzb2, gh ? 1 : 0);
+    }
+    FIL_CHECK_LAUNCH();
+    {
+      ProfScope ps("cin_last_bwd", st, (gh ? 2.0 : 6.0) * (double)M * Hpp * F);
+      if (gh)
+        cin_launch_last_bwd2_gh(st, JT, xT, xpT, xps, qtWsumP, qtWsnP, dense_w + (size_t)p * K, dense_w + (size_t)(p - 1) * K, dense_w + (size_t)lL * K, g,
+                                ghflag, Gbuf[cur], HS0, dxT, (int)M, F, K, Hpp, qtR, HS0);
+      else if (rsel) {
+        hipLaunchKernelGGL(cin_qtail_r_kernel, dim3(cdiv((int)M, kQtRRows)), dim3(128), 0, st, xT, qtT, Gbuf[cur], HS0, (int)M, F, Hpp, ghflag);
+        cin_launch_last_bwd2_rsel(st, JT, xT, xpT, xps, qtWsumP, qtWsnP, dPp, (int)LK, dPprev, Gbuf[cur], HS0, dxT, (int)M, F, K, Hpp, qtR, HS0, dPL, small,
+                                  ghflag);
+      } else
+        cin_launch_last_bwd2(st, JT, xT, xpT, xps, qtWsumP, qtWsnP, dPp, (int)LK, dPprev, Gbuf[cur], HS0, dxT, (int)M, F, K, Hpp, qtR, HS0, dPL, small);
     }
     FIL_CHECK_LAUNCH();
     int dw_parts = 0;
@@ -841,8 +862,15 @@
         dw_parts = bp.splits;
       } else {
         const bool f4 = knobs().dwfold4 != 0;
-        const DwqPlan dp = f4 ? cin_dwq_plan4(M, Cl + F, cu_count()) : cin_dwq_plan(M, Cl + F, cu_count());
-        if (f4)
+        const int Cq = Cl + F + (gh ? 1 : 0);
+        const DwqPlan dp = f4 ? cin_dwq_plan4(M, Cq, cu_count()) : cin_dwq_plan(M, Cq, cu_count());
+        if (gh && f4)
+          hipLaunchKernelGGL((cin_dwq_kernel<kDwqDepth, 4, true>), dim3((dp.wgs + 7) / 8 * 8), dim3(kDwqThreads), 0, st, Gbuf[cur], xpT, HS0, xe, XE, part, (int)M, F,
+                             symD, dp.rows_per_split, dp.splits, dp.ncol_full, dp.rem, dp.wgs_full, dp.wgs, qtGhat, ghflag);
+        else if (gh)
+          hipLaunchKernelGGL((cin_dwq_kernel<kDwqDepth, 2, true>), dim3((dp.wgs + 7) / 8 * 8), dim3(kDwqThreads), 0, st, Gbuf[cur], xpT, HS0, xe, XE, part, (int)M, F,
+                             symD, dp.rows_per_split, dp.splits, dp.ncol_full, dp.rem, dp.wgs_full, dp.wgs, qtGhat, ghflag);
+        else if (f4)
           hipLaunchKernelGGL((cin_dwq_kernel<kDwqDepth, 4>), dim3((dp.wgs + 7) / 8 * 8), dim3(kDwqThreads), 0, st, Gbuf[cur], xpT, HS0, xe, XE, part, (int)M, F,
                              symD, dp.rows_per_split, dp.splits, dp.ncol_full, dp.rem, dp.wgs_full, dp.wgs);
         else
@@ -854,10 +882,10 @@
     FIL_CHECK_LAUNCH();
     {
       ProfScope ps("cin_reduce_dw", st);
-      const int nb1 = cdiv(H[0], 64);
+      const int nb1 = gh ? 0 : cdiv(H[0], 64);
       const int nh = output_dim == 1 ? cdiv((int)LK + 1, 64) : 0;
-      hipLaunchKernelGGL(cin_reduce_expand_q_kernel, dim3((Cl + F + 3) / 4 + nb1 + nh), dim3(256), 0, st, part, dw_parts, F, symD, H[0], Hpp, dW[0], qt_dT,
-                         vlast, small, ncol, dbias[0], nb1, qt_hpart, qt_ndc, (int)LK, ddense_w, ddense_b);
+      hipLaunchKernelGGL(cin_reduce_expand_q_kernel, dim3((Cl + F + (gh ? 1 : 0) + 3) / 4 + nb1 + nh), dim3(256), 0, st, part, dw_parts, F, symD, H[0], Hpp, dW[0], qt_dT,
+                         vlast, small, ncol, dbias[0], nb1, qt_hpart, qt_ndc, (int)LK, ddense_w, ddense_b, gh ? 1 : 0);
     }
     FIL_CHECK_LAUNCH();
     ready(L);
@@ -883,7 +911,8 @@
         split_done = cin_launch_dz2_b(st, qnp, JTs, Gbuf[cur], xpT, HS0, dPL, (int)LK, K, Wzb1, Wzb2, xT, dxT, 1, (int)M, F, H[0], Hpp, periods, dx, qtCvec);
       }
       if (!split_done &&
-          !cin_launch_dz2(st, JTs, Gbuf[cur], xpT, HS0, dPL, (int)LK, K, Wz, qtWzT, xT, dxT, 1, (int)M, F, H[0], Hpp, periods, dx, qtCvec))
+          !cin_launch_dz2(st, JTs, Gbuf[cur], xpT, HS0, dPL, (int)LK, K, Wz, qtWzT, xT, dxT, 1, (int)M, F, H[0], Hpp, periods, dx, qtCvec,
+                          gh ? g : nullptr, qtGhat, ghflag))
         return fail(FIL_ERR_UNSUPPORTED, "fil_cin_bwd: no two-pass data-gradient kernel for JT=%d (F=%d)", JTs, F);
       qm_joined = true;
     } else {
@@ -1139,7 +1168,8 @@
     ProfScope ps("cin_transpose_out", st, 2.0 * M * F * sizeof(float));
     if (qmerge)
       hipLaunchKernelGGL(cin_transpose_out_kernel, dim3(B), dim3(256), (size_t)K * (F + 1) * sizeof(float), st, dxT, have_gx0 ? gx0T : nullptr, dx, F, K,
-                         Gbuf[1] + (size_t)M * (F + 3), Gbuf[1] + (size_t)M * (F + 3) + (size_t)M * F, qtCvec, dPsrc + (size_t)(L - 1) * K, (int)LK);
+                         Gbuf[1] + (size_t)M * qmerge_xe(F, false), Gbuf[1] + (size_t)M * qmerge_xe(F, false) + (size_t)M * F, qtCvec,
+                         dPsrc + (size_t)(L - 1) * K, (int)LK);
     else if (qtail)
       hipLaunchKernelGGL(cin_transpose_out_kernel, dim3(B), dim3(256), (size_t)K * (F + 1) * sizeof(float), st, dxT, have_gx0 ? gx0T : nullptr, dx, F, K,
                          Gbuf[1] + (size_t)M * (F + 1), Gbuf[1] + (size_t)M * (F + 1) + (size_t)M * F, qtCvec, dPsrc + (size_t)(L - 1) * K, (int)LK);
diff --git a/ml_function_amd/csrc/cin_fwd.hip b/ml_function_amd/csrc/cin_fwd.hip
--- a/ml_function_amd/csrc/cin_fwd.hip
+++ b/ml_function_amd/csrc/cin_fwd.hip
@@ -48,15 +48,15 @@
 #undef FIL_F3S
 }
 
-template <int JT>
+template <int JT, bool GH = false, bool RSEL = false>
 static void last_bwd2(hipStream_t st, const float* xT, const float* xpT, int xps, const float* wsum, const float* wsn, const float* dP,
                       int ldp, const float* dPprev, float* GprevT, int HSp, float* dxT, int M, int F, int K, int Hp, const float* Radd, int HSr,
-                      const float* dPadd, float* colpart) {
+                      const float* dPadd, float* colpart, const float* gs = nullptr, const float* gflag = nullptr) {
   const size_t sh = ((size_t)((Hp * F + 3) & ~3) + 4 * kLast2Stage) * sizeof(float);
   if (sh > 48 * 1024)
-    (void)hipFuncSetAttribute(reinterpret_cast<const void*>(cin_last_bwd2_kernel<JT>), hipFuncAttributeMaxDynamicSharedMemorySize, (int)sh);
-  hipLaunchKernelGGL((cin_last_bwd2_kernel<JT>), dim3((M + 127) / 128), dim3(kCinThreads), sh, st, xT, xpT, xps, wsum, wsn, dP, ldp, dPprev,
-                     GprevT, HSp, dxT, M, F, K, Hp, Radd, HSr, dPadd, colpart);
+    (void)hipFuncSetAttribute(reinterpret_cast<const void*>(cin_last_bwd2_kernel<JT, GH, RSEL>), hipFuncAttributeMaxDynamicSharedMemorySize, (int)sh);
+  hipLaunchKernelGGL((cin_last_bwd2_kernel<JT, GH, RSEL>), dim3((M + 127) / 128), dim3(kCinThreads), sh, st, xT, xpT, xps, wsum, wsn, dP, ldp, dPprev,
+                     GprevT, HSp, dxT, M, F, K, Hp, Radd, HSr, dPadd, colpart, gs, gflag);
 }
 
 void cin_launch_last_bwd2(hipStream_t st, int JT, const float* xT, const float* xpT, int xps, const float* wsum, const float* wsn,
@@ -68,4 +68,26 @@
 #undef FIL_LB
 }
 
+void cin_launch_last_bwd2_rsel(hipStream_t st, int JT, const float* xT, const float* xpT, int xps, const float* wsum, const float* wsn,
+                               const float* dP, int ldp, const float* dPprev, float* GprevT, int HSp, float* dxT, int M, int F, int K, int Hp,
+                               const float* Radd, int HSr, const float* dPadd, float* colpart, const float* gflag) {
+#define FIL_LB(JTV) \
+  case JTV: last_bwd2<JTV, false, true>(st, xT, xpT, xps, wsum, wsn, dP, ldp, dPprev, GprevT, HSp, dxT, M, F, K, Hp, Radd, HSr, dPadd, colpart, nullptr, gflag); break;
+  switch (JT) { FIL_LB(4) FIL_LB(8) FIL_LB(12) FIL_LB(16) FIL_LB(20) FIL_LB(24) FIL_LB(28) FIL_LB(32) }
+#undef FIL_LB
 }
+
+}
+
+namespace fil {
+
+void cin_launch_last_bwd2_gh(hipStream_t st, int JT, const float* xT, const float* xpT, int xps, const float* wsum, const float* wsn,
+                             const float* w_p, const float* w_1, const float* w_L, const float* gs, const float* gflag, float* GhatT, int HSp,
+                             float* dxT, int M, int F, int K, int Hp, const float* R, int HSr) {
+#define FIL_LB(JTV) \
+  case JTV: last_bwd2<JTV, true>(st, xT, xpT, xps, wsum, wsn, w_p, 0, w_1, GhatT, HSp, dxT, M, F, K, Hp, R, HSr, w_L, nullptr, gs, gflag); break;
+  switch (JT) { FIL_LB(4) FIL_LB(8) FIL_LB(12) FIL_LB(16) FIL_LB(20) FIL_LB(24) FIL_LB(28) FIL_LB(32) }
+#undef FIL_LB
+}
+
+}
diff --git a/ml_function_amd/csrc/cin_kernels.h b/ml_function_amd/csrc/cin_kernels.h
--- a/ml_function_amd/csrc/cin_kernels.h
+++ b/ml_function_amd/csrc/cin_kernels.h
@@ -1264,14 +1264,18 @@
 
 constexpr int kLast2Ld = 66;
 constexpr int kLast2Stage = 32 * kLast2Ld;
-template <int JT>
+template <int JT, bool GH = false, bool RSEL = false>
 __global__ __launch_bounds__(256, 2) void cin_last_bwd2_kernel(const float* __restrict__ xT, const float* __restrict__ xpT, int xps,
                                                             const float* __restrict__ wsum, const float* __restrict__ wsn,
                                                             const float* __restrict__ dP, int ldp, const float* __restrict__ dPprev,
                                                             float* __restrict__ GprevT, int HSp, float* __restrict__ dxT, int M, int F,
                                                             int K, int Hp, const float* __restrict__ Radd = nullptr, int HSr = 0,
-                                                            const float* __restrict__ dPadd = nullptr, float* __restrict__ colpart = nullptr) {
+                                                            const float* __restrict__ dPadd = nullptr, float* __restrict__ colpart = nullptr,
+                                                            const float* __restrict__ gs = nullptr, const float* __restrict__ gflag = nullptr) {
   __shared__ float colred[4][128];
+  if constexpr (RSEL) {
+    if (*gflag != 0.f) Radd = GprevT;
+  }
   extern __shared__ __attribute__((aligned(16))) float smem[];
   for (int i = threadIdx.x; i < Hp * F; i += 256) smem[i] = wsum[i];
   __syncthreads();
@@ -1298,9 +1302,10 @@
       xr[j] = (f < F && nrow > 0) ? xrow[min(f, F - 1)] : 0.f;
     }
   }
-  __shared__ float dps[4][3][32];
+  __shared__ float dps[4][GH ? 4 : 3][32];
   if (half == 0) {
     const int b = (int)(mq / K), k = (int)(mq - (long)b * K);
+    if constexpr (GH) dps[wave][3][r] = gs[b];
     dps[wave][0][r] = dP[(long)b * ldp + k];
     dps[wave][1][r] = dPprev != nullptr ? dPprev[(long)b * ldp + k] : 0.f;
     dps[wave][2][r] = Radd != nullptr ? dPadd[(long)b * ldp + k] : 0.f;
@@ -1448,12 +1453,19 @@
   for (int reg = 0; reg < 16; ++reg) {
     const int m = wrow0 + mfma32_row(reg, half);
     if (m < M) {
-      const float dpr = dps[wave][0][mfma32_row(reg, half)];
+      float dpr = dps[wave][0][mfma32_row(reg, half)];
+      if constexpr (GH) dpr = dps[wave][3][mfma32_row(reg, half)] * dpr;
       if (r < F) dxT[(long)m * F + r] = dpr * u0[reg];
       if (two && r + 32 < F) dxT[(long)m * F + 32 + r] = dpr * u1[reg];
     }
   }
   };
+  if constexpr (GH) {
+    if (*gflag != 0.f) {
+      phase_u();
+      return;
+    }
+  }
   if ((blockIdx.x >> 3) & 1) {
     phase_u();
     phase_t();
diff --git a/ml_function_amd/csrc/cin_launch.h b/ml_function_amd/csrc/cin_launch.h
--- a/ml_function_amd/csrc/cin_launch.h
+++ b/ml_function_amd/csrc/cin_launch.h
@@ -24,6 +24,13 @@
 void cin_launch_last_bwd2(hipStream_t st, int JT, const float* xT, const float* xpT, int xps, const float* wsum, const float* wsn,
                           const float* dP, int ldp, const float* dPprev, float* GprevT, int HSp, float* dxT, int M, int F, int K, int Hp,
                           const float* Radd = nullptr, int HSr = 0, const float* dPadd = nullptr, float* colpart = nullptr);
+
+void cin_launch_last_bwd2_rsel(hipStream_t st, int JT, const float* xT, const float* xpT, int xps, const float* wsum, const float* wsn,
+                               const float* dP, int ldp, const float* dPprev, float* GprevT, int HSp, float* dxT, int M, int F, int K, int Hp,
+                               const float* Radd, int HSr, const float* dPadd, float* colpart, const float* gflag);
+void cin_launch_last_bwd2_gh(hipStream_t st, int JT, const float* xT, const float* xpT, int xps, const float* wsum, const float* wsn,
+                             const float* w_p, const float* w_1, const float* w_L, const float* gs, const float* gflag, float* GhatT, int HSp,
+                             float* dxT, int M, int F, int K, int Hp, const float* R, int HSr);
 
 void cin_launch_dz3_sym(hipStream_t st, int MB, int JT, int NHMAX, dim3 grid, const float* gT, int HS, const float* Wz, const float* xT,
                         float* gx0T, float* dxT, int accumulate, int M, int F, int H, int periods, int ks = 1);
diff --git a/ml_function_amd/csrc/cin_qmerge.h b/ml_function_amd/csrc/cin_qmerge.h
--- a/ml_function_amd/csrc/cin_qmerge.h
+++ b/ml_function_amd/csrc/cin_qmerge.h
@@ -54,14 +54,16 @@
   return p;
 }
 
-template <int DEPTH = kDwqDepth, int FOLD = 2>
+template <int DEPTH = kDwqDepth, int FOLD = 2, bool GH = false>
 __global__ __launch_bounds__(kDwqThreads, 2) void cin_dwq_kernel(const float* __restrict__ gT, const float* __restrict__ x1T, int HS, const float* __restrict__ xe,
                                                                 int XE, float* __restrict__ part, int M, int F, int symD, int rows_per_split, int splits,
-                                                                int ncol_full, int rem, int wgs_full, int wgs) {
+                                                                int ncol_full, int rem, int wgs_full, int wgs, const float* __restrict__ ghT = nullptr,
+                                                                const float* __restrict__ gflag = nullptr) {
   __shared__ float fold[4][128][64];
   const int tid = threadIdx.x, lane = tid & 63, wave = tid >> 6;
   const int r = lane & 31, half = lane >> 5;
-  const int Cp = F * symD, C = Cp + F;
+  const int Cp = F * symD, C = Cp + F, C1 = C + (GH ? 1 : 0);
+  if constexpr (GH) gT = *gflag != 0.f ? ghT : gT;
   const int item = (blockIdx.x & 7) * (gridDim.x >> 3) + (blockIdx.x >> 3);
   if (item >= wgs) return;
   const int wl = FOLD == 4 ? (wave & 1) : (wave & 3), up = FOLD == 4 ? (wave >> 1) : (wave >> 2);
@@ -106,9 +108,12 @@
   const __amdgpu_buffer_rsrc_t r1 = make_rsrc_uniform(x1T + mbase * HS, mrem * HS * 4);
   const __amdgpu_buffer_rsrc_t rx = make_rsrc_uniform(xe + mbase * XE, mrem * XE * 4);
   const int c = c0 + r;
-  const int cc = c < C ? c : C - 1;
+  const int cc = c < C1 ? c : C1 - 1;
   int hh, ff, sel;
-  if (cc < Cp) {
+  if (GH && cc == C) {
+    hh = ff = F;
+    sel = 1;
+  } else if (cc < Cp) {
     hh = cc / symD;
     ff = (hh + (cc - hh * symD)) % F;
     sel = 0;
@@ -119,6 +124,7 @@
   }
   const int ho = (half * XE + hh) * 4, fo = (half * XE + ff) * 4, so = (half * XE + F + 1 + sel) * 4;
   const int go = (half * HS + 4 * r) * 4;
+  const int qo = (half * XE + F + 3) * 4;
   const int steps = work ? (m_hi - m_lo + 1) >> 1 : 0;
   const int groups = (steps + DEPTH - 1) / DEPTH;
 
@@ -128,7 +134,7 @@
 #pragma unroll
     for (int i = 0; i < 16; ++i) acc[nb][i] = 0.f;
   f32x4s qg[DEPTH], q1[DEPTH];
-  float qh[DEPTH], qf[DEPTH], qs[DEPTH];
+  float qh[DEPTH], qf[DEPTH], qs[DEPTH], qgs[GH ? DEPTH : 1];
   auto fetch = [&](int s, int d) {
     const int row = 2 * s;
     qg[d] = __builtin_bit_cast(f32x4s, __builtin_amdgcn_raw_buffer_load_b128(rg, go, row * HS * 4, 0));
@@ -136,10 +142,12 @@
     qh[d] = __builtin_bit_cast(float, __builtin_amdgcn_raw_buffer_load_b32(rx, ho, row * XE * 4, 0));
     qf[d] = __builtin_bit_cast(float, __builtin_amdgcn_raw_buffer_load_b32(rx, fo, row * XE * 4, 0));
     qs[d] = __builtin_bit_cast(float, __builtin_amdgcn_raw_buffer_load_b32(rx, so, row * XE * 4, 0));
+    if constexpr (GH) qgs[d] = __builtin_bit_cast(float, __builtin_amdgcn_raw_buffer_load_b32(rx, qo, row * XE * 4, 0));
   };
 #pragma unroll
   for (int d = 0; d < DEPTH; ++d) fetch(d, d);
   float ac = qh[0] * qf[0], ac2 = ac * qs[0], an, an2;
+  if constexpr (GH) ac *= qgs[0];
 #pragma unroll 1
   for (int g = 0; g < groups; ++g) {
 #pragma unroll
@@ -147,6 +155,7 @@
       const f32x4s g4 = qg[d], x4 = q1[d];
       an = qh[(d + 1) % DEPTH] * qf[(d + 1) % DEPTH];
       an2 = an * qs[(d + 1) % DEPTH];
+      if constexpr (GH) an *= qgs[(d + 1) % DEPTH];
       __builtin_amdgcn_sched_barrier(0);
       acc[0] = mfma32(ac, g4[0], acc[0]);
       acc[1] = mfma32(ac, g4[1], acc[1]);
@@ -205,14 +214,14 @@
 #pragma unroll
       for (int i = 0; i < 16; ++i) acc[nb][i] += fold[wl][nb * 16 + i][lane];
   }
-  float* pout = part + (long)pair * C * 256;
+  float* pout = part + (long)pair * C1 * 256;
 #pragma unroll
   for (int reg = 0; reg < 16; ++reg) {
     const int cr = c0 + mfma32_row(reg, half);
-    if (cr < C) {
+    if (cr < C1) {
       float* dst = pout + (long)cr * 256 + 4 * r;
-      if (cr < Cp) *reinterpret_cast<float4*>(dst) = make_float4(acc[0][reg], acc[1][reg], acc[2][reg], acc[3][reg]);
-      *reinterpret_cast<float4*>(dst + 128) = make_float4(acc[4][reg], acc[5][reg], acc[6][reg], acc[7][reg]);
+      if (cr < Cp || cr == C) *reinterpret_cast<float4*>(dst) = make_float4(acc[0][reg], acc[1][reg], acc[2][reg], acc[3][reg]);
+      if (cr < C) *reinterpret_cast<float4*>(dst + 128) = make_float4(acc[4][reg], acc[5][reg], acc[6][reg], acc[7][reg]);
     }
   }
 }
@@ -221,9 +230,9 @@
                                                                           float* __restrict__ dW1, float* __restrict__ dT, float* __restrict__ vT,
                                                                           const float* __restrict__ bpart, int nbp, float* __restrict__ dbias1,
                                                                           int nb1, const float* __restrict__ hpart, int nhp, int LK,
-                                                                          float* __restrict__ ddw, float* __restrict__ ddb) {
-  const int Cp = F * D, C = Cp + F;
-  const int nbw = (C + 3) / 4;
+                                                                          float* __restrict__ ddw, float* __restrict__ ddb, int dbrow = 0) {
+  const int Cp = F * D, C = Cp + F, C1 = C + dbrow;
+  const int nbw = (C1 + 3) / 4;
   if ((int)blockIdx.x >= nbw + nb1) {
     cin_reduce_body(hpart, ddw, (long)LK + 1, nhp, ddb, (long)LK, (int)blockIdx.x - nbw - nb1);
     return;
@@ -234,8 +243,8 @@
   }
   const int lane = threadIdx.x & 63, wave = threadIdx.x >> 6;
   const int c = blockIdx.x * 4 + wave;
-  if (c >= C) return;
-  const long ps = (long)C * 256;
+  if (c >= C1) return;
+  const long ps = (long)C1 * 256;
   const float* p0 = part + (long)c * 256 + 4 * lane;
   f32x4 t[8];
 #pragma unroll
@@ -250,6 +259,14 @@
   const int col = 4 * lane, n0 = col & 127;
   const bool second = col >= 128;
   const int H = second ? H2 : H1;
+  if (c == C) {
+    if (!second) {
+#pragma unroll
+      for (int e = 0; e < 4; ++e)
+        if (n0 + e < H1) dbias1[n0 + e] = v[e];
+    }
+    return;
+  }
   if (c >= Cp) {
     if (second) {
 #pragma unroll
@@ -287,7 +304,7 @@
                                                                   int LK, int lL, int lp, const float* __restrict__ W0, float* __restrict__ Wz,
                                                                   int H0, int JTs, int HS0, int tiles0, int npz = -1,
                                                                   const float* __restrict__ Tq = nullptr, int HT = 0, u32x4* __restrict__ Wzb1 = nullptr,
-                                                                  u32x4* __restrict__ Wzb2 = nullptr) {
+                                                                  u32x4* __restrict__ Wzb2 = nullptr, int xg = 0) {
   extern __shared__ __attribute__((aligned(16))) float smem[];
   if ((int)blockIdx.x >= nscale) {
     if (threadIdx.x >= 256) return;
@@ -302,7 +319,7 @@
     return;
   }
   const int nl = g != nullptr ? LK / K : 0;
-  const int hl = nl + 1, XE = F + 3;
+  const int hl = nl + 1, XE = F + 3 + xg;
   const int tid = threadIdx.x;
   const long m0 = (long)blockIdx.x * 256;
   const int nrows = (int)min((long)256, (long)M - m0);
@@ -310,6 +327,7 @@
   float* dls = xs + 256 * F;
   float* dps = dls + 256;
   float* hd = dps + 256;
+  float* gs = hd + 256 * hl;
   {
     const float* src = xT + m0 * F;
     const int n = nrows * F;
@@ -331,12 +349,13 @@
   }
   if (tid < 256) {
     const long m = m0 + tid;
-    float dl = 0.f, dp = 0.f;
+    float dl = 0.f, dp = 0.f, gr = 0.f;
     if (m < M) {
       const long b = m / K;
       const int k = (int)(m - b * K);
       if (g != nullptr) {
         const float gb = g[b];
+        gr = gb;
         for (int l = 0; l < nl; ++l) {
           const float d = gb * dense_w[l * K + k];
           dP[b * LK + l * K + k] = d;
@@ -354,6 +373,7 @@
     }
     dls[tid] = dl;
     dps[tid] = dp;
+    if (xg) gs[tid] = gr;
   }
   __syncthreads();
   __shared__ float cs[4][64];
@@ -368,7 +388,7 @@
       float e[4];
 #pragma unroll
       for (int u = 0; u < 4; ++u) {
-        e[u] = c < F ? xs[rr * F + c] : c == F ? 1.f : c == F + 1 ? dls[rr] : dps[rr];
+        e[u] = c < F ? xs[rr * F + c] : c == F ? 1.f : c == F + 1 ? dls[rr] : c == F + 2 ? dps[rr] : gs[rr];
         if (++c == XE) {
           c = 0;
           ++rr;
@@ -378,7 +398,7 @@
     }
     for (int i = 4 * n4 + tid; i < nrows * XE; i += NT) {
       const int rr = i / XE, c = i - rr * XE;
-      dst[i] = c < F ? xs[rr * F + c] : c == F ? 1.f : c == F + 1 ? dls[rr] : dps[rr];
+      dst[i] = c < F ? xs[rr * F + c] : c == F ? 1.f : c == F + 1 ? dls[rr] : c == F + 2 ? dps[rr] : gs[rr];
     }
   } else {
     const int t2 = tid - (kXeThreads - 256);
@@ -466,7 +486,9 @@
                                                          const float* __restrict__ dsc, int ldp, int K, const float* __restrict__ Wz1,
                                                          const float* __restrict__ Wz2, const float* __restrict__ xT, float* __restrict__ dxT,
                                                          int accumulate, int M, int F, int H1, int H2, int periods, int FR,
-                                                         float* __restrict__ dx, const float* __restrict__ cvec) {
+                                                         float* __restrict__ dx, const float* __restrict__ cvec, const float* __restrict__ gs = nullptr,
+                                                         const float* __restrict__ ghT = nullptr, const float* __restrict__ gflag = nullptr) {
+  if (gs != nullptr && *gflag != 0.f) g1T = ghT;
   extern __shared__ __attribute__((aligned(16))) float smem[];
   constexpr int P = JT / gcd_c(16, JT);
   constexpr int HPP = 16 * P / JT;
@@ -499,10 +521,11 @@
       }
     }
   }
-  float dpl;
+  float dpl, grow = 1.f;
   {
     const long bb = mq / K;
     dpl = dsc[bb * ldp + (mq - bb * K)];
+    if (gs != nullptr) grow = gs[bb];
   }
   __builtin_amdgcn_wave_barrier();
   const long wbytes = ((long)periods * P + 1) * 32 * 128 * 4;
@@ -518,7 +541,7 @@
         greg[4 * s4 + e] = __builtin_bit_cast(float, __builtin_bit_cast(int, gv) & keep) * sc;
       }
   };
-  to_greg(gq, H1, 1.f);
+  to_greg(gq, H1, grow);
 
 #pragma unroll 1
   for (int pass = 0; pass < 2; ++pass) {
@@ -642,7 +665,7 @@
 
 bool cin_launch_dz2(hipStream_t st, int JT, const float* g1T, const float* g2T, int HS, const float* dsc, int ldp, int K, const float* Wz1,
                     const float* Wz2, const float* xT, float* dxT, int accumulate, int M, int F, int H1, int H2, int periods,
-                    float* dx = nullptr, const float* cvec = nullptr);
+                    float* dx = nullptr, const float* cvec = nullptr, const float* gs = nullptr, const float* ghT = nullptr, const float* gflag = nullptr);
 
 struct CinHeadFold {
   float* pooled;
@@ -653,12 +676,27 @@
 };
 
 template <int NW>
+__device__ __forceinline__ float (&cin_ghat_weights())[NW][3][32] {
+  __shared__ float w[NW][3][32];
+  return w;
+}
+template <int NW, bool GH = false>
 __device__ __forceinline__ void cin_fwdq_epilogue(f32x16 (&acc)[8], const __amdgpu_buffer_rsrc_t& rx, int vhalf, int wo, int r, int half, int wave, int wrow0,
                                                   const float* __restrict__ bias1, const float* __restrict__ wsn, int JTG, const float* __restrict__ cvec,
                                                   float* __restrict__ x1T, float* __restrict__ RT, int HS, float* __restrict__ pool1,
                                                   float* __restrict__ pool_p, float* __restrict__ pool_L, int M, int F, int H, const CinHeadFold& hf,
-                                                  float (&lin_s)[NW][32], float (&pv_s)[NW][3][32]) {
+                                                  float (&lin_s)[NW][32], float (&pv_s)[NW][3][32], float* __restrict__ GT = nullptr) {
   const int lane = half * 32 + r;
+  const bool ghat = GH && GT != nullptr && hf.out != nullptr;
+  if constexpr (GH) {
+    if (ghat && half == 0) {
+      float (&gw_s)[NW][3][32] = cin_ghat_weights<NW>();
+      const int k = (wrow0 + r) & ((1 << hf.kshift) - 1);
+      gw_s[wave][0][r] = hf.dense_w[k];
+      gw_s[wave][1][r] = hf.dense_w[hf.op + k];
+      gw_s[wave][2][r] = hf.dense_w[hf.oL + k];
+    }
+  }
   f32x16 t[4];
 #pragma unroll
   for (int nb = 0; nb < 4; ++nb)
@@ -722,7 +760,19 @@
     const float b0 = acc[4][reg], b1 = acc[5][reg], b2 = acc[6][reg], b3 = acc[7][reg];
     if (m < M) {
       *reinterpret_cast<float4*>(x1T + (long)m * HS + 4 * r) = make_float4(a0, a1, a2, a3);
-      *reinterpret_cast<float4*>(RT + (long)m * HS + 4 * r) = make_float4(b0, b1, b2, b3);
+      if (!ghat) *reinterpret_cast<float4*>(RT + (long)m * HS + 4 * r) = make_float4(b0, b1, b2, b3);
+      if constexpr (GH) {
+        if (ghat) {
+          float (&gw_s)[NW][3][32] = cin_ghat_weights<NW>();
+          const float w1 = gw_s[wave][0][row], wp = gw_s[wave][1][row], wL = gw_s[wave][2][row];
+          float gh[4] = {fmaf(wL, b0, fmaf(wp, t[0][reg], w1)), fmaf(wL, b1, fmaf(wp, t[1][reg], w1)), fmaf(wL, b2, fmaf(wp, t[2][reg], w1)),
+                         fmaf(wL, b3, fmaf(wp, t[3][reg], w1))};
+#pragma unroll
+          for (int nb = 0; nb < 4; ++nb)
+            if (4 * r + nb >= H) gh[nb] = 0.f;
+          *reinterpret_cast<float4*>(GT + (long)m * HS + 4 * r) = make_float4(gh[0], gh[1], gh[2], gh[3]);
+        }
+      }
     }
     float p1 = (a0 + a1) + (a2 + a3);
     float eL = a0 * b0, ep = a0 * t[0][reg];
@@ -775,7 +825,7 @@
                                                           const float* __restrict__ bias1, const float* __restrict__ wsn, int JTG,
                                                           const float* __restrict__ cvec, float* __restrict__ x1T, float* __restrict__ RT, int HS,
                                                           float* __restrict__ pool1, float* __restrict__ pool_p, float* __restrict__ pool_L, int M, int F,
-                                                          int H, CinHeadFold hf) {
+                                                          int H, CinHeadFold hf, float* __restrict__ GT, float* __restrict__ gflag) {
   constexpr int DEPTH = JT % 5 == 0 ? 5 : (JT % 4 == 0 ? 4 : (JT % 7 == 0 ? 7 : (JT % 3 == 0 ? 3 : 2)));
   static_assert(JT % DEPTH == 0, "queue depth must divide the steps per h");
   __shared__ float lin_s[4][32];
@@ -783,6 +833,7 @@
   const int tid = threadIdx.x, lane = tid & 63, wave = tid >> 6;
   const int r = lane & 31, half = lane >> 5;
   const int wrow0 = (blockIdx.x * 4 + wave) * 32;
+  if (blockIdx.x == 0 && tid == 0 && gflag != nullptr) *gflag = (GT != nullptr && hf.out != nullptr) ? 1.f : 0.f;
   if (wrow0 >= M) return;
   const int wrow_u = __builtin_amdgcn_readfirstlane(wrow0);
   const __amdgpu_buffer_rsrc_t rx = make_rsrc_uniform(x2T + (long)(wrow_u >> 6) * XL * 64, (long)XL * 256);
@@ -850,10 +901,11 @@
   }
   if (h < F) run_h(h, xa, pa, xb, pb);
 
-  cin_fwdq_epilogue<4>(acc, rx, vhalf, wo, r, half, wave, wrow0, bias1, wsn, JTG, cvec, x1T, RT, HS, pool1, pool_p, pool_L, M, F, H, hf, lin_s, pv_s);
+  cin_fwdq_epilogue<4, true>(acc, rx, vhalf, wo, r, half, wave, wrow0, bias1, wsn, JTG, cvec, x1T, RT, HS, pool1, pool_p, pool_L, M, F, H, hf, lin_s, pv_s, GT);
 }
 
 bool cin_launch_fwdq(hipStream_t st, int JT, const float* x2T, int XL, const float* W1f, const float* WTf, const float* bias1, const float* wsn, int JTG,
-                     const float* cvec, float* x1T, float* RT, int HS, float* pool1, float* pool_p, float* pool_L, int M, int F, int H, CinHeadFold hf);
-
-}
+                     const float* cvec, float* x1T, float* RT, int HS, float* pool1, float* pool_p, float* pool_L, int M, int F, int H, CinHeadFold hf,
+                     float* GT = nullptr, float* gflag = nullptr);
+
+}
diff --git a/ml_function_amd/csrc/cin_qmerge.hip b/ml_function_amd/csrc/cin_qmerge.hip
--- a/ml_function_amd/csrc/cin_qmerge.hip
+++ b/ml_function_amd/csrc/cin_qmerge.hip
@@ -4,36 +4,37 @@
 
 template <int JT, int G>
 static void dz2g(hipStream_t st, const float* g1T, const float* g2T, int HS, const float* dsc, int ldp, int K, const float* Wz1, const float* Wz2,
-                 const float* xT, float* dxT, int accumulate, int M, int F, int H1, int H2, int periods, float* dx, const float* cvec) {
+                 const float* xT, float* dxT, int accumulate, int M, int F, int H1, int H2, int periods, float* dx, const float* cvec, const float* gs, const float* ghT, const float* gflag) {
   const int FR = cin_dz2_rows(F, JT);
   const size_t sh = (size_t)FR * kDz2FieldStride * sizeof(float);
   if (sh > 48 * 1024)
     (void)hipFuncSetAttribute(reinterpret_cast<const void*>(cin_dz2_kernel<JT, G>), hipFuncAttributeMaxDynamicSharedMemorySize, (int)sh);
   hipLaunchKernelGGL((cin_dz2_kernel<JT, G>), dim3(cdiv(M, 128)), dim3(kCinThreads), sh, st, g1T, g2T, HS, dsc, ldp, K, Wz1, Wz2, xT, dxT, accumulate, M, F, H1,
-                     H2, periods, FR, dx, cvec);
+                     H2, periods, FR, dx, cvec, gs, ghT, gflag);
 }
 template <int JT>
 static void dz2(hipStream_t st, const float* g1T, const float* g2T, int HS, const float* dsc, int ldp, int K, const float* Wz1, const float* Wz2,
-                const float* xT, float* dxT, int accumulate, int M, int F, int H1, int H2, int periods, float* dx, const float* cvec) {
-  if (JT >= 4 && F >= cin_dz_h_per_period(JT) + 2 * JT) dz2g<JT, (JT >= 4 ? 4 : 1)>(st, g1T, g2T, HS, dsc, ldp, K, Wz1, Wz2, xT, dxT, accumulate, M, F, H1, H2, periods, dx, cvec);
-  else dz2g<JT, 1>(st, g1T, g2T, HS, dsc, ldp, K, Wz1, Wz2, xT, dxT, accumulate, M, F, H1, H2, periods, dx, cvec);
+                const float* xT, float* dxT, int accumulate, int M, int F, int H1, int H2, int periods, float* dx, const float* cvec, const float* gs, const float* ghT, const float* gflag) {
+  if (JT >= 4 && F >= cin_dz_h_per_period(JT) + 2 * JT) dz2g<JT, (JT >= 4 ? 4 : 1)>(st, g1T, g2T, HS, dsc, ldp, K, Wz1, Wz2, xT, dxT, accumulate, M, F, H1, H2, periods, dx, cvec, gs, ghT, gflag);
+  else dz2g<JT, 1>(st, g1T, g2T, HS, dsc, ldp, K, Wz1, Wz2, xT, dxT, accumulate, M, F, H1, H2, periods, dx, cvec, gs, ghT, gflag);
 }
 
 bool cin_launch_dz2(hipStream_t st, int JT, const float* g1T, const float* g2T, int HS, const float* dsc, int ldp, int K, const float* Wz1,
-                    const float* Wz2, const float* xT, float* dxT, int accumulate, int M, int F, int H1, int H2, int periods, float* dx, const float* cvec) {
+                    const float* Wz2, const float* xT, float* dxT, int accumulate, int M, int F, int H1, int H2, int periods, float* dx, const float* cvec, const float* gs, const float* ghT, const float* gflag) {
 #define FIL_Z2(JTV) \
-  case JTV: dz2<JTV>(st, g1T, g2T, HS, dsc, ldp, K, Wz1, Wz2, xT, dxT, accumulate, M, F, H1, H2, periods, dx, cvec); break;
+  case JTV: dz2<JTV>(st, g1T, g2T, HS, dsc, ldp, K, Wz1, Wz2, xT, dxT, accumulate, M, F, H1, H2, periods, dx, cvec, gs, ghT, gflag); break;
   switch (JT) { FIL_Z2(2) FIL_Z2(4) FIL_Z2(6) FIL_Z2(8) FIL_Z2(10) FIL_Z2(12) FIL_Z2(14) FIL_Z2(16) FIL_Z2(18) default: return false; }
 #undef FIL_Z2
   return true;
 }
 
 bool cin_launch_fwdq(hipStream_t st, int JT, const float* x2T, int XL, const float* W1f, const float* WTf, const float* bias1, const float* wsn, int JTG,
-                     const float* cvec, float* x1T, float* RT, int HS, float* pool1, float* pool_p, float* pool_L, int M, int F, int H, CinHeadFold hf) {
+                     const float* cvec, float* x1T, float* RT, int HS, float* pool1, float* pool_p, float* pool_L, int M, int F, int H, CinHeadFold hf,
+                     float* GT, float* gflag) {
 #define FIL_FQ(JTV)                                                                                                                             \
   case JTV:                                                                                                                                     \
     hipLaunchKernelGGL((cin_fwdq_kernel<JTV>), dim3(cdiv(M, 128)), dim3(kCinThreads), 0, st, x2T, XL, W1f, WTf, bias1, wsn, JTG, cvec, x1T, RT, HS, \
-                       pool1, pool_p, pool_L, M, F, H, hf);                                                                                       \
+                       pool1, pool_p, pool_L, M, F, H, hf, GT, gflag);                                                                                   \
     break;
   switch (JT) { FIL_FQ(2) FIL_FQ(4) FIL_FQ(6) FIL_FQ(8) FIL_FQ(10) FIL_FQ(12) FIL_FQ(14) FIL_FQ(16) FIL_FQ(18) default: return false; }
 #undef FIL_FQ
diff --git a/ml_function_amd/csrc/cin_qtail.h b/ml_function_amd/csrc/cin_qtail.h
--- a/ml_function_amd/csrc/cin_qtail.h
+++ b/ml_function_amd/csrc/cin_qtail.h
@@ -268,6 +268,34 @@
   }
 }
 
+constexpr int kQtRRows = 16;
+static __global__ __launch_bounds__(128) void cin_qtail_r_kernel(const float* __restrict__ xT, const float* __restrict__ T, float* __restrict__ Rout, int HS,
+                                                                 int M, int F, int H, const float* __restrict__ gflag) {
+  if (*gflag == 0.f) return;
+  __shared__ float xs[kQtRRows][64];
+  const int m0 = blockIdx.x * kQtRRows, h = threadIdx.x;
+  for (int i = threadIdx.x; i < kQtRRows * F; i += 128) {
+    const int rr = i / F, f = i - rr * F;
+    xs[rr][f] = m0 + rr < M ? xT[(long)(m0 + rr) * F + f] : 0.f;
+  }
+  __syncthreads();
+  float acc[kQtRRows];
+#pragma unroll
+  for (int rr = 0; rr < kQtRRows; ++rr) acc[rr] = 0.f;
+  if (h < H) {
+    for (int fp = 0; fp < F; ++fp)
+      for (int f = 0; f < F; ++f) {
+        const float t = T[(long)(fp * F + f) * H + h];
+#pragma unroll
+        for (int rr = 0; rr < kQtRRows; ++rr) acc[rr] = fmaf(xs[rr][fp] * xs[rr][f], t, acc[rr]);
+      }
+  }
+  for (int c = h; c < HS; c += 128)
+#pragma unroll
+    for (int rr = 0; rr < kQtRRows; ++rr)
+      if (m0 + rr < M) Rout[(long)(m0 + rr) * HS + c] = c < H ? acc[rr] : 0.f;
+}
+
 template <int JT>
 __global__ __launch_bounds__(256, 2) void cin_qtail_pool2_kernel(const float* __restrict__ xT, const float* __restrict__ xpT, int xps,
                                                                  const float* __restrict__ wsn, const float* __restrict__ R, int HSr,
```
